# jklebes/MetropolisEngine

Hardware: AMD Instinct MI355X
Metric: MC steps/sec (chains x sweeps) at 2^20 chains, 16 params (higher is better)
Workload: dtype f64

## Files before the change

include/metropolis_engine.h:

```cpp
#ifndef METROPOLIS_ENGINE_H
#define METROPOLIS_ENGINE_H

#include <stddef.h>
#include <stdint.h>

#ifdef __cplusplus
extern "C" {
#endif

#define ME_ABI_VERSION 1

typedef struct me_engine me_engine;

typedef enum me_status {
  ME_OK = 0,
  ME_ERR_INVALID = 1,
  ME_ERR_UNSUPPORTED = 2,
  ME_ERR_HIP = 3,
  ME_ERR_NUMERIC = 4,
  ME_ERR_STATE = 5
} me_status;

typedef enum me_dtype { ME_F32 = 0, ME_F64 = 1 } me_dtype;

// ... 206 lines not shown
int me_mbar_histogram_gram_samples(int32_t device_id, const double *energies, const int32_t *rungs, int64_t n_samples,
                                   const double *ladder_temps, int32_t n_rungs, const double *f, const double *temps, int32_t n,
                                   const double *values, const double *edges, int32_t n_bins, double *slot_gram,
                                   double *ladder_gram, double *column_counts, double *mass, int64_t *counts,
                                   double *neff_fraction, int64_t *n_used);
int me_mbar_histogram_joint(me_engine *engine, const double *f, const double *temps, int32_t n, int32_t column_x,
                        const double *edges_x, int32_t n_bins_x, int32_t column_y, const double *edges_y, int32_t n_bins_y,
                        double *mass, int64_t *counts, double *neff_fraction);
int me_mbar_histogram_joint_samples(int32_t device_id, const double *energies, const int32_t *rungs, int64_t n_samples,
                                const double *ladder_temps, int32_t n_rungs, const double *f, const double *temps, int32_t n,
                                const double *values_x, const double *values_y, const double *edges_x, int32_t n_bins_x,
                                const double *edges_y, int32_t n_bins_y, double *mass, int64_t *counts, double *neff_fraction);
int me_mbar_histogram_joint_gram(me_engine *engine, const double *f, const double *temps, int32_t n, int32_t column_x,
                                 const double *edges_x, int32_t n_bins_x, int32_t column_y, const double *edges_y,
                                 int32_t n_bins_y, double *cell_gram, double *ladder_gram, double *column_counts, double *mass,
                                 int64_t *counts, double *neff_fraction, int64_t *n_used);
int me_mbar_histogram_joint_gram_samples(int32_t device_id, const double *energies, const int32_t *rungs, int64_t n_samples,
                                         const double *ladder_temps, int32_t n_rungs, const double *f, const double *temps,
                                         int32_t n, const double *values_x, const double *values_y, const double *edges_x,
                                         int32_t n_bins_x, const double *edges_y, int32_t n_bins_y, double *cell_gram,
                                         double *ladder_gram, double *column_counts, double *mass, int64_t *counts,
                                         double *neff_fraction, int64_t *n_used);

int me_recorded_inefficiency(me_engine *engine, int32_t mintime, int32_t max_lag, double *g, double *mean, double *var,
                             int32_t *stop_lag, int64_t *chains_used, double *acf);
int me_series_inefficiency_samples(int32_t device_id, const double *series, int64_t n_records, int64_t n_series,
                                   int64_t group_chains, int32_t mintime, int32_t max_lag, double *g, double *mean, double *var,
                                   int32_t *stop_lag, int64_t *chains_used, double *acf);

int me_last_error(me_engine *engine, char *buf, size_t buf_bytes);

int me_supported(int32_t dtype, int32_t n_real, int32_t n_complex, int32_t energy_kind);

int me_detect_equilibration(int32_t device_id, const double *series, int64_t n_series, int64_t length, int32_t fast,
                            int32_t nskip, int64_t *t0, double *g, double *neff_max);

#ifdef __cplusplus
}
#endif
#endif
```

metropolisengine_amd/_capi.py:

```python
import ctypes
import os

PKG_DIR = os.path.dirname(os.path.abspath(__file__))
LIB_PATH = os.environ.get("METROPOLIS_HIP_LIB") or os.path.join(PKG_DIR, "lib", "libmetropolis_hip.so")
ABI_VERSION = 1

ME_OK, ME_ERR_INVALID, ME_ERR_UNSUPPORTED, ME_ERR_HIP, ME_ERR_NUMERIC, ME_ERR_STATE = range(6)
ME_F32, ME_F64 = 0, 1
(ENERGY_ISO_QUAD, ENERGY_DIAG_QUAD, ENERGY_DENSE_QUAD, ENERGY_LANDAU_TOY, ENERGY_CYLINDER, ENERGY_USER,
 ENERGY_USER_INDIRECT, ENERGY_LANDAU_TERMS) = range(8)
FLAG_TRACK_COVARIANCE = 1
FLAG_REFERENCE_ENERGY_LEDGERS = 2
REJECT_NONE, REJECT_ABS_REAL0_GE, REJECT_USER = 0, 1, 2
STEP_ALL, STEP_REAL_GROUP, STEP_COMPLEX_GROUP, STEP_COMPLEX_MAGNITUDE_PHASE = range(4)
COV_REFERENCE, COV_FIXED, COV_POOLED = 0, 1, 2
COMM_ID_BYTES = 128
(FIELD_PARAMS, FIELD_ENERGY, FIELD_WIDTH, FIELD_MEAN, FIELD_COV, FIELD_OBS_MEAN, FIELD_FACTOR, FIELD_ENERGY_TOTAL) = range(8)

_dp = ctypes.POINTER(ctypes.c_double)


def double_ptr(arr):
    return arr.ctypes.data_as(_dp)

# ... 44 lines not shown
                                               ctypes.POINTER(ctypes.c_double)]),
    "me_get": (ctypes.c_int, [_H, ctypes.c_int32, ctypes.c_int64, ctypes.c_int64, _dp]),
    "me_set": (ctypes.c_int, [_H, ctypes.c_int32, ctypes.c_int64, ctypes.c_int64, _dp]),
    "me_recompute_energy": (ctypes.c_int, [_H]),
    "me_constants": (ctypes.c_int, [_H, _dp, ctypes.POINTER(ctypes.c_int32), _dp]),
    "me_counters": (ctypes.c_int, [_H, ctypes.POINTER(ctypes.c_uint64), ctypes.POINTER(ctypes.c_uint64)]),
    "me_set_counters": (ctypes.c_int, [_H, ctypes.c_uint64, ctypes.c_uint64]),
    "me_accept_stats": (ctypes.c_int, [_H, ctypes.POINTER(ctypes.c_uint64), ctypes.POINTER(ctypes.c_uint64)]),
    "me_pooled_moments_size": (ctypes.c_int, [_H, ctypes.POINTER(ctypes.c_int64)]),
    "me_pooled_moments_geometry": (ctypes.c_int, [_H, ctypes.POINTER(ctypes.c_int32), ctypes.POINTER(ctypes.c_int32),
                                                  ctypes.POINTER(ctypes.c_int32)]),
    "me_pooled_moments": (ctypes.c_int, [_H, _dp, ctypes.c_int64]),
    "me_pooled_moments_device": (ctypes.c_int, [_H, ctypes.c_void_p, ctypes.c_int64]),
    "me_comm_unique_id": (ctypes.c_int, [ctypes.c_void_p, ctypes.c_size_t]),
    "me_comm_init_rank": (ctypes.c_int, [_H, ctypes.c_void_p, ctypes.c_size_t, ctypes.c_int32, ctypes.c_int32]),
    "me_comm_destroy": (ctypes.c_int, [_H]),
    "me_comm_info": (ctypes.c_int, [_H, ctypes.POINTER(ctypes.c_int32), ctypes.POINTER(ctypes.c_int32),
                                    ctypes.POINTER(ctypes.c_int32)]),
    "me_pooled_moments_allreduce": (ctypes.c_int, [_H, _dp, ctypes.c_int64]),
    "me_pooled_moments_allreduce_begin": (ctypes.c_int, [_H]),
    "me_set_shared_factor": (ctypes.c_int, [_H, _dp, ctypes.c_int64]),
    "me_get_shared_factor": (ctypes.c_int, [_H, _dp, ctypes.c_int64, ctypes.POINTER(ctypes.c_int32)]),
    "me_set_accept_stats": (ctypes.c_int, [_H, ctypes.c_uint64, ctypes.c_uint64]),
    "me_set_cache_budget": (ctypes.c_int, [ctypes.c_int64]),
    "me_trace_enable": (ctypes.c_int, [_H, ctypes.c_int64, ctypes.c_int64]),
    "me_trace_shape": (ctypes.c_int, [_H, ctypes.POINTER(ctypes.c_int64), ctypes.POINTER(ctypes.c_int64),
                                      ctypes.POINTER(ctypes.c_int64)]),
    "me_trace_get": (ctypes.c_int, [_H, _dp, ctypes.c_int64]),
    "me_sync": (ctypes.c_int, [_H]),
    "me_set_stream": (ctypes.c_int, [_H, ctypes.c_void_p]),
    "me_time_steps": (ctypes.c_int, [_H, ctypes.c_int32, ctypes.c_int32, ctypes.POINTER(ctypes.c_float)]),
    "me_last_error": (ctypes.c_int, [_H, ctypes.c_char_p, ctypes.c_size_t]),
    "me_supported": (ctypes.c_int, [ctypes.c_int32, ctypes.c_int32, ctypes.c_int32, ctypes.c_int32]),
    "me_set_temperature_ladder": (ctypes.c_int, [_H, _dp, ctypes.c_int32]),
    "me_temperature_ladder": (ctypes.c_int, [_H, _dp, ctypes.c_int32, ctypes.POINTER(ctypes.c_int32)]),
    "me_replica_exchange": (ctypes.c_int, [_H, ctypes.c_int32]),
    "me_replica_stats": (ctypes.c_int, [_H, ctypes.POINTER(ctypes.c_uint64), ctypes.POINTER(ctypes.c_uint64),
                                        ctypes.POINTER(ctypes.c_uint64), ctypes.c_int32]),
    "me_set_replica_stats": (ctypes.c_int, [_H, ctypes.c_uint64, ctypes.POINTER(ctypes.c_uint64),
                                            ctypes.POINTER(ctypes.c_uint64), ctypes.c_int32]),
    "me_pooled_moments_range": (ctypes.c_int, [_H, ctypes.c_int64, ctypes.c_int64, _dp, ctypes.c_int64]),
    "me_set_temperature": (ctypes.c_int, [_H, ctypes.c_double]),
    "me_population_resample": (ctypes.c_int, [_H, ctypes.c_double]),
    "me_population_stats": (ctypes.c_int, [_H, ctypes.POINTER(ctypes.c_uint64), _dp, _dp, _dp, ctypes.POINTER(ctypes.c_int64),
                                           ctypes.c_int64]),
    "me_set_population_stats": (ctypes.c_int, [_H, ctypes.c_uint64, _dp, _dp, _dp, ctypes.POINTER(ctypes.c_int64)]),
    "me_population_families": (ctypes.c_int, [_H, ctypes.c_int64, ctypes.c_int64, ctypes.POINTER(ctypes.c_int64)]),
    "me_set_population_families": (ctypes.c_int, [_H, ctypes.c_int64, ctypes.c_int64, ctypes.POINTER(ctypes.c_int64)]),
    "me_energy_samples_enable": (ctypes.c_int, [_H, ctypes.c_int64]),
    "me_energy_samples_record": (ctypes.c_int, [_H]),
    "me_energy_samples_count": (ctypes.c_int, [_H, ctypes.POINTER(ctypes.c_int64), ctypes.POINTER(ctypes.c_int64)]),
    "me_energy_samples_get": (ctypes.c_int, [_H, ctypes.c_int64, ctypes.c_int64, _dp]),
    "me_energy_samples_set": (ctypes.c_int, [_H, ctypes.c_int64, _dp]),
    "me_mbar_solve": (ctypes.c_int, [_H, ctypes.c_double, ctypes.c_int32, _dp, ctypes.POINTER(ctypes.c_int32), _dp,
                                     ctypes.POINTER(ctypes.c_int64)]),
    "me_mbar_solve_newton": (ctypes.c_int, [_H, ctypes.c_double, ctypes.c_int32, _dp, ctypes.POINTER(ctypes.c_int32), _dp, _dp,
                                            ctypes.POINTER(ctypes.c_int32), ctypes.POINTER(ctypes.c_int32),
                                            ctypes.POINTER(ctypes.c_int64)]),
    "me_mbar_solve_newton_samples": (ctypes.c_int, [ctypes.c_int32, _dp, ctypes.POINTER(ctypes.c_int32), ctypes.c_int64, _dp,
                                                    ctypes.c_int32, ctypes.c_double, ctypes.c_int32, _dp,
                                                    ctypes.POINTER(ctypes.c_int32), _dp, _dp, ctypes.POINTER(ctypes.c_int32),
                                                    ctypes.POINTER(ctypes.c_int32), ctypes.POINTER(ctypes.c_int64)]),
    "me_mbar_reweight": (ctypes.c_int, [_H, _dp, _dp, ctypes.c_int32, _dp, _dp, _dp, _dp]),
    "me_mbar_solve_samples": (ctypes.c_int, [ctypes.c_int32, _dp, ctypes.POINTER(ctypes.c_int32), ctypes.c_int64, _dp,
                                             ctypes.c_int32, ctypes.c_double, ctypes.c_int32, _dp,
                                             ctypes.POINTER(ctypes.c_int32), _dp, ctypes.POINTER(ctypes.c_int64)]),
# ... 107 lines not shown
```

metropolisengine_amd/csrc/me_api.hip:

```cpp
#include <algorithm>
#include <cmath>
#include <cstdlib>
#include <cstring>
#include <dlfcn.h>
#include <mutex>
#include <memory>
#include <string>
#include <atomic>
#include <chrono>
#include <vector>

#include "me_engine.h"

namespace me {

static std::vector<const KernelSet *> &registry() {
  static std::vector<const KernelSet *> sets;
  return sets;
}
static std::mutex &registry_mutex() {
  static std::mutex m;
  return m;
}
void register_kernel_set(const KernelSet *set) {
// ... 112 lines not shown
  to_device_type(src, count, dtype, bytes);
  const hipError_t err = dst.resize(bytes.size());
  return err != hipSuccess ? err : hipMemcpy(dst.get(), bytes.data(), bytes.size(), hipMemcpyHostToDevice);
}

int refuse_stale_total(me_engine *e, const char *subject) {
  if (!e->stale_total) return ME_OK;
  return fail(e, ME_ERR_UNSUPPORTED, std::string(subject) + " not available with ME_FLAG_REFERENCE_ENERGY_LEDGERS: its two ledgers "
                                                            "make the energy of a chain ambiguous");
}

static int report_status(me_engine *e, unsigned int bits) {
  if (!bits) return ME_OK;
  ME_HIP(e, hipMemsetAsync(e->status.get(), 0, sizeof(unsigned int), e->stream));
  std::string msg = "numeric failure in at least one chain:";
  if (bits & ST_NONFINITE_ENERGY) msg += " non-finite energy;";
  if (bits & ST_BAD_PIVOT) msg += " non-positive Cholesky pivot (proposal covariance not positive definite);";
  if (bits & ST_BAD_WIDTH) msg += " sampling width <= 0;";
  return fail(e, ME_ERR_NUMERIC, msg);
}
int check_status(me_engine *e) {
  unsigned long long *scratch = e->host_scratch.get<unsigned long long>();
  ME_HIP(e, hipMemcpyAsync(&scratch[0], e->status.get(), sizeof(unsigned int), hipMemcpyDeviceToHost, e->stream));
  ME_HIP(e, hipStreamSynchronize(e->stream));
  return report_status(e, (unsigned int)scratch[0]);
}

}

using namespace me;

namespace {

int broadcast(me_engine *e, DeviceBuffer &dst, const std::vector<double> &row, bool tiled = false) {
  std::vector<unsigned char> bytes;
  to_device_type(row.data(), row.size(), e->dtype, bytes);
  ME_HIP(e, hipMemcpyAsync(e->row_dev.get(), bytes.data(), bytes.size(), hipMemcpyHostToDevice, e->stream));
  if (tiled) ME_HIP(e, launch_broadcast_tiled(dst.get(), e->row_dev.get(), (int)row.size(), e->n, e->dtype, e->stream));
  else ME_HIP(e, launch_broadcast_rows(dst.get(), e->row_dev.get(), (int)row.size(), e->n, e->dtype, e->stream));
  ME_HIP(e, hipStreamSynchronize(e->stream));
  return ME_OK;
}

template <typename T>
void gather_rows(const T *t, int comps, int64_t n_chains, double *dst) {
  for (int r = 0; r < comps; ++r)
    for (int64_t c = 0; c < n_chains; ++c) dst[c * comps + r] = (double)t[(size_t)r * n_chains + c];
}
template <typename T>
void scatter_rows(T *t, int comps, int64_t n_chains, const double *src) {
  for (int r = 0; r < comps; ++r)
    for (int64_t c = 0; c < n_chains; ++c) t[(size_t)r * n_chains + c] = (T)src[c * comps + r];
}
template <typename T>
void transpose_tiled(T *t, int entries, int64_t tile0, int64_t chain_begin, int64_t n_chains, double *dst, const double *src) {
  const size_t tile_values = (size_t)entries * 64;
  auto at = [&](int64_t c, int k) { return (size_t)((c >> 6) - tile0) * tile_values + (size_t)k * 64 + (size_t)(c & 63); };
  for (int64_t i = 0; i < n_chains; ++i)
    for (int k = 0; k < entries; ++k) {
      if (dst) dst[i * entries + k] = (double)t[at(chain_begin + i, k)];
      else t[at(chain_begin + i, k)] = (T)src[i * entries + k];
    }
}

int copy_tiled(me_engine *e, void *field_ptr, int entries, int64_t chain_begin, int64_t n_chains, double *dst, const double *src) {
  const int64_t tile0 = chain_begin >> 6, tile1 = (chain_begin + n_chains - 1) >> 6;
  const size_t tile_values = (size_t)entries * 64, n_values = (size_t)(tile1 - tile0 + 1) * tile_values;
  unsigned char *dev = (unsigned char *)field_ptr + (size_t)tile0 * tile_values * e->esize;
  std::vector<unsigned char> tmp(n_values * e->esize);
  const bool whole = (chain_begin & 63) == 0 && (((chain_begin + n_chains) & 63) == 0 || chain_begin + n_chains == e->n);
  if (dst || !whole) {
    ME_HIP(e, hipMemcpyAsync(tmp.data(), dev, tmp.size(), hipMemcpyDeviceToHost, e->stream));
    ME_HIP(e, hipStreamSynchronize(e->stream));
  }
  if (e->dtype == ME_F32) transpose_tiled(reinterpret_cast<float *>(tmp.data()), entries, tile0, chain_begin, n_chains, dst, src);
  else transpose_tiled(reinterpret_cast<double *>(tmp.data()), entries, tile0, chain_begin, n_chains, dst, src);
  if (src) {
    ME_HIP(e, hipMemcpyAsync(dev, tmp.data(), tmp.size(), hipMemcpyHostToDevice, e->stream));
    ME_HIP(e, hipStreamSynchronize(e->stream));
  }
  return dst ? check_status(e) : ME_OK;
}

int field_info(me_engine *e, int field, void **ptr, int *comps) {
  switch (field) {
    case ME_FIELD_PARAMS: *ptr = e->x.get(); *comps = e->d; return ME_OK;
    case ME_FIELD_ENERGY: *ptr = e->energy.get(); *comps = e->n_terms; return ME_OK;
    case ME_FIELD_WIDTH: *ptr = e->width.get(); *comps = e->width_rows; return ME_OK;
    case ME_FIELD_MEAN: *ptr = e->mean.get(); *comps = e->d; return ME_OK;
    case ME_FIELD_OBS_MEAN: *ptr = e->obs_mean.get(); *comps = e->nobs; return ME_OK;
    case ME_FIELD_COV:
      if (!e->cov)
        return fail(e, ME_ERR_UNSUPPORTED, "this engine keeps no per-chain covariance: for large parameter spaces it is "
                                           "kept on request only (me_config.flags: ME_FLAG_TRACK_COVARIANCE), and not "
                                           "at all where the field would pass 4 GiB");
      *ptr = e->cov.get(); *comps = e->p; return ME_OK;
    case ME_FIELD_ENERGY_TOTAL:
      if (!e->stale_total)
        return fail(e, ME_ERR_UNSUPPORTED, "this engine keeps one coherent energy ledger (sum ME_FIELD_ENERGY); a separate "
                                           "energy_total exists with ME_FLAG_REFERENCE_ENERGY_LEDGERS only");
      *ptr = e->energy.get<unsigned char>() + (size_t)e->n_terms * (size_t)e->n * e->esize; *comps = 1; return ME_OK;
    case ME_FIELD_FACTOR:
      if (!e->factor) return fail(e, ME_ERR_UNSUPPORTED, "this engine keeps no per-chain proposal factors (dimensions "
                                                         "without per-chain kernels, or a field beyond 4 GiB)");
      *ptr = e->factor.get(); *comps = e->p; return ME_OK;
    default: return fail(e, ME_ERR_INVALID, "unknown field id");
  }
}

// ... 56 lines not shown
    return fail(e, ME_ERR_INVALID, "ME_REJECT_ABS_REAL0_GE needs a real parameter");
  return ME_OK;
}
int check_user_reject(me_engine *e, int reject_kind, const KernelSet *ks) {
  if (reject_kind == ME_REJECT_USER && !ks->has_user_reject)
    return fail(e, ME_ERR_UNSUPPORTED,
                "ME_REJECT_USER: this user-energy plugin defines no me_user_reject (#define ME_USER_HAS_REJECT in its source)");
  return ME_OK;
}

}

namespace me {
namespace {
std::atomic<long long> g_cache_budget{224ll << 20};
}
long long cache_budget_bytes() { return g_cache_budget.load(std::memory_order_relaxed); }
void set_cache_budget_bytes(long long bytes) { g_cache_budget.store(bytes, std::memory_order_relaxed); }
}


int me_set_cache_budget(int64_t bytes) {
  if (bytes < 0) return fail(nullptr, ME_ERR_INVALID, "cache budget must be >= 0");
  me::set_cache_budget_bytes(bytes);
  return ME_OK;
}

int me_abi_version(void) { return ME_ABI_VERSION; }

int me_supported(int32_t dtype, int32_t n_real, int32_t n_complex, int32_t energy_kind) {
  return find_kernel_set(dtype, n_real, n_complex, energy_kind, nullptr) ? 1 : 0;
}

namespace {

int validate_config(const me_config *c, const KernelSet **ks_out) {
  if (c->abi_version != ME_ABI_VERSION) return fail(nullptr, ME_ERR_INVALID, "me_config.abi_version mismatch");
  if (c->n_real < 0 || c->n_complex < 0 || c->n_real + c->n_complex == 0)
    return fail(nullptr, ME_ERR_INVALID,
                "must give at least one real or complex parameter (metropolis_engine.py:37-39)");
  if (c->n_chains <= 0) return fail(nullptr, ME_ERR_INVALID, "n_chains must be positive");
  if (!(c->temp >= 0)) return fail(nullptr, ME_ERR_INVALID, "temp must be >= 0 (metropolis_engine.py:92)");
  if (!(c->target_acceptance > 0 && c->target_acceptance < 1))
    return fail(nullptr, ME_ERR_INVALID, "target_acceptance must be in (0, 1)");
  if (!(c->sampling_width > 0)) return fail(nullptr, ME_ERR_INVALID, "sampling_width must be > 0");
  if (c->dtype != ME_F32 && c->dtype != ME_F64) return fail(nullptr, ME_ERR_INVALID, "unknown dtype");
  if (!c->initial_params) return fail(nullptr, ME_ERR_INVALID, "initial_params is required");
  if (c->n_energy_coeffs < 0 || (c->n_energy_coeffs > 0 && !c->energy_coeffs))
    return fail(nullptr, ME_ERR_INVALID, "energy coefficients missing");
  int rc = check_reject_kind(nullptr, c->reject_kind, c->energy_kind, c->n_real);
  if (rc != ME_OK) return rc;
  if (c->cov_mode < ME_COV_REFERENCE || c->cov_mode > ME_COV_POOLED)
    return fail(nullptr, ME_ERR_INVALID, "unknown cov_mode");
  const KernelSet *ks = *ks_out = find_kernel_set(c->dtype, c->n_real, c->n_complex, c->energy_kind, c->user_energy_name);
  if (!ks) {
    if (is_user_kind(c->energy_kind))
      return fail(nullptr, ME_ERR_UNSUPPORTED,
                  std::string("no user-energy plugin named '") + (c->user_energy_name ? c->user_energy_name : "") +
                      "' is loaded for these dimensions (build it with metropolisengine_amd.build.build_user_energy "
                      "and load it with me_load_plugin)");
    if (!has_dims(c->dtype, c->n_real, c->n_complex))
      return fail(nullptr, ME_ERR_UNSUPPORTED,
                  "no kernel set compiled for (dtype, n_real, n_complex) = (" + std::to_string(c->dtype) + ", " +
                      std::to_string(c->n_real) + ", " + std::to_string(c->n_complex) + ")");
    return fail(nullptr, ME_ERR_UNSUPPORTED, "energy kind " + std::to_string(c->energy_kind) +
                                                  " is not compiled for these dimensions");
// ... 8 lines not shown
    const bool starts_shared = !initial_shape_is_identity(c) && c->cov_mode != ME_COV_REFERENCE;
    if (starts_shared && c->n_complex > 0)
      return fail(nullptr, ME_ERR_UNSUPPORTED,
                  "parameter spaces beyond " + std::to_string(kMaxRegisterDof) + " real degrees of freedom with complex "
                  "parameters run with the identity proposal shape only: leave covariance_matrix_real / _complex unset");
    {
      const long long per_block = (long long)(c->n_real + 2 * c->n_complex) * 64 * (c->dtype == ME_F32 ? 4 : 8);
      const bool dense = c->energy_kind == ME_ENERGY_DENSE_QUAD, pooled = c->cov_mode == ME_COV_POOLED || starts_shared;
      const bool per_chain = c->cov_mode == ME_COV_REFERENCE || (c->flags & ME_FLAG_TRACK_COVARIANCE) != 0;
      if ((dense || pooled || per_chain) && per_block * (pooled ? 2 : 1) > 150 * 1024)
        return fail(nullptr, ME_ERR_UNSUPPORTED,
                    "a dense quadratic form, a shared proposal factor or per-chain shapes beyond " + std::to_string(kMaxRegisterDof) +
                        " degrees of freedom are staged in LDS: this many parameters do not fit (float64: about 290, 145 with "
                        "a shared factor or an initial covariance that ME_COV_FIXED keeps; float32 twice that)");
    }
    if (c->flags & ME_FLAG_REFERENCE_ENERGY_LEDGERS)
      return fail(nullptr, ME_ERR_UNSUPPORTED, "ME_FLAG_REFERENCE_ENERGY_LEDGERS is not available beyond " +
                                                   std::to_string(kMaxRegisterDof) + " real degrees of freedom");
    if (c->reject_kind == ME_REJECT_USER) return fail(nullptr, ME_ERR_UNSUPPORTED, "no user plugins at these dimensions");
  }
  if ((c->flags & ME_FLAG_REFERENCE_ENERGY_LEDGERS) && (c->n_real == 0 || c->n_complex == 0))
    return fail(nullptr, ME_ERR_INVALID,
                "ME_FLAG_REFERENCE_ENERGY_LEDGERS applies to mixed engines (real and complex parameters): only their "
                "step_all keeps a separate energy_total (metropolis_engine.py:241-259)");
  if (c->cov_mode == ME_COV_REFERENCE && !ks->per_chain_cov)
    return fail(nullptr, ME_ERR_UNSUPPORTED,
                "per-chain adaptive covariance is not compiled for these dimensions; use ME_COV_FIXED or ME_COV_POOLED");
  return ME_OK;
}

struct Layout {
  bool keep_per_chain;
  bool keep_cov;
  bool x_tiled;
  int width_rows;
};
int decide_layout(const me_config *c, const KernelSet *ks, Layout &l) {
  const long long esz = c->dtype == ME_F32 ? 4 : 8, limit = 1ll << 32, padded = padded_chains(c->n_chains);
  l.keep_per_chain = ks->per_chain_cov && (!ks->streams_packed || c->cov_mode == ME_COV_REFERENCE);
  if (l.keep_per_chain && !ks->streams_packed && (long long)packed_total(c->n_real, c->n_complex) * padded * esz >= limit) {
    if (c->cov_mode == ME_COV_REFERENCE)
      return fail(nullptr, ME_ERR_UNSUPPORTED,
                  "the per-chain covariance field would exceed 4 GiB on this engine; shard the chains over more "
                  "engines or use ME_COV_FIXED / ME_COV_POOLED");
    l.keep_per_chain = false;
  }
  const long long rows = std::max<long long>(c->n_real + 2 * c->n_complex, 2 * c->n_real + c->n_complex);
  if (rows * padded * esz >= limit)
    return fail(nullptr, ME_ERR_UNSUPPORTED,
                "a per-chain field would exceed 4 GiB on this engine; shard the chains over more engines");
  l.keep_cov = l.keep_per_chain ||
               ((!ks->per_chain_cov || ks->streams_packed) && ks->tracks_cov && (c->flags & ME_FLAG_TRACK_COVARIANCE));
  l.x_tiled = ks->tiled_state;
  l.width_rows = (c->n_real > 0 && c->n_complex > 0) ? 3 : 1;
  return ME_OK;
}

std::unique_ptr<me_engine> configure(const me_config *c, const KernelSet *ks, const Layout &l) {
  std::unique_ptr<me_engine> e(new me_engine);
  e->device = c->device_id;
  e->ks = ks;
  e->n_terms = ks->energy_terms(c->energy_kind);
  e->dtype = c->dtype;
  e->esize = c->dtype == ME_F32 ? 4 : 8;
  e->n = c->n_chains;
  e->nr = c->n_real;
  e->nc = c->n_complex;
  e->d = e->nr + 2 * e->nc;
  e->p = packed_total(e->nr, e->nc);
  e->nobs = n_observables(e->nr, e->nc);
  e->chain_offset = c->chain_offset;
  e->seed = c->seed;
  e->temp = c->temp;
  e->target_acceptance = c->target_acceptance;
  e->energy_kind = c->energy_kind;
  e->reject_kind = c->reject_kind;
  e->reject_bound = c->reject_bound;
  e->cov_mode = c->cov_mode;
  e->coef.assign(c->energy_coeffs, c->energy_coeffs + c->n_energy_coeffs);
  e->alpha = -norm_ppf(c->target_acceptance / 2.0);
  e->m = e->nr + e->nc;
  e->ratio = (1.0 - 1.0 / e->m) * std::sqrt(2.0 * M_PI) * std::exp(e->alpha * e->alpha / 2.0) / 2.0 * e->alpha +
             1.0 / (e->m * c->target_acceptance * (1.0 - c->target_acceptance));
  if (const char *g = std::getenv("ME_GRID_BLOCKS")) e->grid_blocks = std::atoi(g);
  e->x_tiled = l.x_tiled;
  e->stale_total = (c->flags & ME_FLAG_REFERENCE_ENERGY_LEDGERS) != 0;
  e->width_rows = l.width_rows;
  e->n_slots = (e->n + 31) / 32 + 8;
  return e;
}

int allocate(me_engine *e, const Layout &l) {
  const KernelSet *ks = e->ks;
  ME_HIP(e, hipSetDevice(e->device));
  ME_HIP(e, e->stream.create());
  const size_t n = (size_t)e->n, tiles = (size_t)padded_chains(e->n), es = e->esize;
  ME_HIP(e, e->x.resize((e->x_tiled ? tiles : n) * e->d * es));
  ME_HIP(e, e->energy.resize(n * (e->n_terms + (e->stale_total ? 1 : 0)) * es));
  ME_HIP(e, e->width.resize(n * e->width_rows * es));
  ME_HIP(e, e->mean.resize(n * e->d * es));
  ME_HIP(e, e->obs_mean.resize(n * e->nobs * es));
  if (l.keep_cov) ME_HIP(e, e->cov.resize(tiles * e->p * es));
  if (l.keep_per_chain) ME_HIP(e, e->factor.resize(tiles * e->p * es));
  ME_HIP(e, e->shared_factor.resize((size_t)e->p * es));
  if (e->nc == 0) ME_HIP(e, e->shared_full.resize((size_t)e->nr * e->nr * es));
  if (e->shared_full && ks->prepare_matrix) ME_HIP(e, e->shared_image.resize(ks->matrix_image_bytes));
  ME_HIP(e, e->row_dev.resize((size_t)std::max(std::max(e->d, e->p), e->nobs) * es));
  ME_HIP(e, e->accept_slots.resize((size_t)e->n_slots * sizeof(unsigned long long)));
  ME_HIP(e, e->accept_total.resize(sizeof(unsigned long long)));
  ME_HIP(e, e->status.resize(sizeof(unsigned int)));
  const size_t moments_bytes = sizeof(double) * (size_t)moments_size(e->nr, e->nc);
  ME_HIP(e, e->pool.dev.resize(moments_bytes));
  ME_HIP(e, e->host_scratch.allocate(64));
  e->host_scratch.get<unsigned long long>()[0] = e->host_scratch.get<unsigned long long>()[1] = 0;
  ME_HIP(e, e->pool.host.allocate(moments_bytes));
  if (pool_reduce_supported(e->nr, e->nc, e->dtype))
    ME_HIP(e, e->pool.partials.resize(sizeof(double) * (size_t)pool_reduce_blocks(e->n, e->nr, e->nc) *
                                      (size_t)(1 + e->d + e->nr + e->nc + e->d * (e->d + 1) / 2)));
  ME_HIP(e, hipMemsetAsync(e->accept_slots.get(), 0, e->accept_slots.bytes(), e->stream));
  ME_HIP(e, hipMemsetAsync(e->status.get(), 0, sizeof(unsigned int), e->stream));
  return ME_OK;
}

int upload_coefficients(me_engine *e) {
  const std::vector<double> &coef = e->coef;
  const bool runtime_dims = e->ks->n_real < 0;
  std::vector<double> form;
  if (runtime_dims && e->energy_kind == ME_ENERGY_DIAG_QUAD) {
    if ((int)coef.size() != e->nr + e->nc) return fail(e, ME_ERR_INVALID, "wrong number of energy coefficients for this energy kind");
    form.assign(coef.begin(), coef.end());
// ... 23 lines not shown
  for (int i = 0; i < e->nr; ++i) {
    obs[i] = std::fabs(init[i]);
    obs[e->nr + e->nc + i] = init[i] * init[i];
  }
  for (int j = 0; j < e->nc; ++j) obs[e->nr + j] = std::hypot(init[e->nr + j], init[e->nr + e->nc + j]);
  const int pr = packed_real(e->nr);
  std::vector<double> c0(e->p, 0.0);
  bool identity = true;
  for (int i = 0; i < e->nr; ++i)
    for (int j = 0; j <= i; ++j) {
      const double v = c->covariance_real ? c->covariance_real[i * e->nr + j] : (i == j ? 1.0 : 0.0);
      c0[i * (i + 1) / 2 + j] = v;
      identity = identity && v == (i == j ? 1.0 : 0.0);
    }
  for (int i = 0; i < e->nc; ++i) {
    for (int j = 0; j < i; ++j) {
      const double re = c->covariance_complex ? c->covariance_complex[2 * (i * e->nc + j)] : 0.0;
      const double im = c->covariance_complex ? c->covariance_complex[2 * (i * e->nc + j) + 1] : 0.0;
      c0[pr + i * i + 2 * j] = re;
      c0[pr + i * i + 2 * j + 1] = im;
      identity = identity && re == 0.0 && im == 0.0;
    }
    const double dg = c->covariance_complex ? c->covariance_complex[2 * (i * e->nc + i)] : 1.0;
    c0[pr + i * i + 2 * i] = dg;
    identity = identity && dg == 1.0;
  }
  std::vector<double> f0 = c0;
  for (int i = 0; i < e->nc; ++i)
    for (int j = 0; j < i; ++j) f0[pr + i * i + 2 * j + 1] = -f0[pr + i * i + 2 * j + 1];
  if (!host_factor(f0, e->nr, e->nc))
    return fail(e, ME_ERR_INVALID, "initial covariance matrix is not positive definite (metropolis_engine.py:270)");
  int rc = ME_OK;
  std::vector<double> width_row((size_t)e->width_rows, c->sampling_width);
  if ((rc = broadcast(e, e->x, init, e->x_tiled)) || (rc = broadcast(e, e->mean, init)) || (rc = broadcast(e, e->obs_mean, obs)) ||
      (rc = broadcast(e, e->width, width_row)) || (e->cov && (rc = broadcast(e, e->cov, c0, true))) ||
      (e->factor && (rc = broadcast(e, e->factor, f0, true))) || (rc = upload_shared_factor(e, f0.data())))
    return rc;
  e->cov_kind = identity ? CK_IDENTITY : (e->ks->n_real < 0 && e->factor) ? CK_PER_CHAIN : CK_SHARED;
  return ME_OK;
}

int initial_energy(me_engine *e) {
  const int rc = me_recompute_energy(e);
  if (rc != ME_OK) return rc;
  const hipError_t herr = hipStreamSynchronize(e->stream);
  if (herr != hipSuccess) return fail(e, ME_ERR_HIP, std::string("initial energy evaluation: ") + hipGetErrorString(herr));
  return ME_OK;
}

}

int me_create(const me_config *c, me_engine **out) {
  if (!c || !out) return fail(nullptr, ME_ERR_INVALID, "null config or output pointer");
  *out = nullptr;
  const KernelSet *ks = nullptr;
  Layout layout;
  int rc;
  if ((rc = validate_config(c, &ks)) || (rc = decide_layout(c, ks, layout))) return rc;
  int n_dev = 0;
  if (hipGetDeviceCount(&n_dev) != hipSuccess || n_dev <= 0)
    return fail(nullptr, ME_ERR_HIP, "no HIP device available (this library has no CPU fallback)");
  if (c->device_id < 0 || c->device_id >= n_dev) return fail(nullptr, ME_ERR_INVALID, "device_id out of range");

  std::unique_ptr<me_engine> e = configure(c, ks, layout);
  if ((rc = allocate(e.get(), layout)) || (rc = upload_coefficients(e.get())) || (rc = initial_state(e.get(), c)) ||
      (rc = initial_energy(e.get())))
    return fail(nullptr, rc, e->err);
  *out = e.release();
  return ME_OK;
}

int me_set_reject_condition(me_engine *e, int32_t reject_kind, double reject_bound) {
  if (!e) return ME_ERR_INVALID;
  int rc;
  if ((rc = check_reject_kind(e, reject_kind, e->energy_kind, e->nr)) || (rc = check_user_reject(e, reject_kind, e->ks))) return rc;
  e->reject_kind = reject_kind;
  e->reject_bound = reject_bound;
  return ME_OK;
}

int me_set_energy(me_engine *e, int32_t energy_kind, const double *coeffs, int32_t n_coeffs, const char *user_name) {
  if (!e) return ME_ERR_INVALID;
  if (n_coeffs < 0 || (n_coeffs > 0 && !coeffs)) return fail(e, ME_ERR_INVALID, "energy coefficients missing");
  if (e->ks->n_real < 0) return fail(e, ME_ERR_UNSUPPORTED, "me_set_energy: not available on the runtime-dimension kernel set");
  if (energy_kind == ME_ENERGY_DENSE_QUAD)
    return fail(e, ME_ERR_UNSUPPORTED, "me_set_energy: the dense quadratic form keeps device images of its matrix; create a new engine");
  const KernelSet *ks = find_kernel_set(e->dtype, e->nr, e->nc, energy_kind, user_name);
  if (!ks || ks->n_real < 0)
    return fail(e, ME_ERR_UNSUPPORTED, is_user_kind(energy_kind)
                    ? std::string("no user-energy plugin named '") + (user_name ? user_name : "") + "' is loaded for these dimensions"
                    : "energy kind " + std::to_string(energy_kind) + " is not compiled for these dimensions");
  if (ks->tiled_state != e->ks->tiled_state || ks->per_chain_cov != e->ks->per_chain_cov || ks->streams_packed != e->ks->streams_packed ||
      ks->tracks_cov != e->ks->tracks_cov)
    return fail(e, ME_ERR_UNSUPPORTED, "me_set_energy: the plugin was built with other per-chain covariance options than this engine's kernel set");
  if (e->reject_kind == ME_REJECT_USER && !ks->has_user_reject)
    return fail(e, ME_ERR_UNSUPPORTED, "me_set_energy: the engine's wall is the plugin's me_user_reject, which the new energy does not define");
  const int n_terms = ks->energy_terms(energy_kind);
  ME_HIP(e, hipSetDevice(e->device));
  ME_HIP(e, hipStreamSynchronize(e->stream));
  DeviceBuffer ledger, coef_dev;
  if (n_terms != e->n_terms)
    ME_HIP(e, ledger.resize((size_t)e->n * (size_t)(n_terms + (e->stale_total ? 1 : 0)) * e->esize));
  if (is_user_kind(energy_kind) && n_coeffs > 0) ME_HIP(e, upload(coef_dev, coeffs, (size_t)n_coeffs, e->dtype));
  if (n_terms != e->n_terms) {
    e->energy = std::move(ledger);
    e->n_terms = n_terms;
    if (e->trace.chains > 0) e->trace.restart();
  }
  e->coef.assign(coeffs, coeffs + n_coeffs);
  e->coef_dev = std::move(coef_dev);
  e->ks = ks;
  e->energy_kind = energy_kind;
  const int rc = me_recompute_energy(e);
  if (rc != ME_OK) return rc;
  ME_HIP(e, hipStreamSynchronize(e->stream));
  return check_status(e);
}

int me_load_plugin(const char *path) {
  if (!path) return fail(nullptr, ME_ERR_INVALID, "null plugin path");
  void *handle = dlopen(path, RTLD_NOW | RTLD_GLOBAL);
  if (!handle) return fail(nullptr, ME_ERR_INVALID, std::string("dlopen failed: ") + dlerror());
  return ME_OK;
}

// ... 128 lines not shown
  l.mean = e->mean.get();
  l.cov = e->cov.get();
  l.obs_mean = e->obs_mean.get();
  l.factor = e->factor.get();
  l.status = e->status.get<unsigned int>();
  l.n = e->n;
  l.measure_count = count;
  l.update_cov = (count > 50 && e->cov) ? 1 : 0;
  l.split_widths = (e->width_rows == 3 && !e->widths_synced) ? 1 : 0;
  l.write_factor = (l.update_cov && e->cov_mode == ME_COV_REFERENCE) ? 1 : 0;
  l.grid_blocks = e->grid_blocks;
}

int commit_measure(me_engine *e, const MeasureLaunch &l) {
  e->measure_count = l.measure_count;
  if (l.write_factor) e->cov_kind = CK_PER_CHAIN;
  if (e->trace.chains > 0) {
    const long long cols = e->d + e->n_terms + e->width_rows;
    if (e->trace.rows == e->trace.capacity) {
      const long long cap = e->trace.capacity ? 2 * e->trace.capacity : 1024;
      DeviceBuffer bigger;
      ME_HIP(e, bigger.resize(sizeof(double) * (size_t)(cap * cols * e->trace.chains)));
      if (e->trace.dev) {
        ME_HIP(e, hipMemcpyAsync(bigger.get(), e->trace.dev.get(), sizeof(double) * (size_t)(e->trace.rows * cols * e->trace.chains),
                                 hipMemcpyDeviceToDevice, e->stream));
        ME_HIP(e, hipStreamSynchronize(e->stream));
      }
      e->trace.dev = std::move(bigger);
      e->trace.capacity = cap;
    }
    const int rows_valid = (e->width_rows == 3 && e->widths_synced) ? 1 : e->width_rows;
    double *row = e->trace.dev.get<double>() + e->trace.rows * cols * e->trace.chains;
    ME_HIP(e, launch_trace(e->x.get(), e->energy.get(), e->width.get(), e->n, e->d, e->n_terms, rows_valid, e->dtype, e->trace.chains,
                           e->trace.stride, row, e->stream, e->x_tiled));
    if (rows_valid != e->width_rows) {
      double *widths = row + (size_t)(e->d + e->n_terms) * e->trace.chains;
      for (int r = 1; r < 3; ++r)
        ME_HIP(e, hipMemcpyAsync(widths + (size_t)r * e->trace.chains, widths, sizeof(double) * (size_t)e->trace.chains,
                                 hipMemcpyDeviceToDevice, e->stream));
    }
    e->trace.rows += 1;
  }
  return ME_OK;
}
}

int me_measure(me_engine *e) {
  if (!e) return ME_ERR_INVALID;
  ME_HIP(e, hipSetDevice(e->device));
  MeasureLaunch l;
  fill_measure_launch(e, l, e->measure_count + 1);
  ME_HIP(e, e->ks->measure(l, e->stream));
  return commit_measure(e, l);
}

int me_cycle(me_engine *e, int32_t n_sweeps) {
  if (!e) return ME_ERR_INVALID;
  if (n_sweeps <= 0) return fail(e, ME_ERR_INVALID, "n_sweeps must be positive");
  ME_HIP(e, hipSetDevice(e->device));
  if (e->ks->cycle) {
    StepLaunch sl;
    fill_step_launch(e, sl, n_sweeps);
    MeasureLaunch ml;
    fill_measure_launch(e, ml, e->measure_count + 1);
    ml.split_widths = 0;
    const hipError_t err = e->ks->cycle(sl, ml, e->stream);
    if (err == hipSuccess) {
// ... 39 lines not shown
  const long long want = e->trace.rows * (e->d + e->n_terms + e->width_rows) * e->trace.chains;
  if (n_doubles != want) return fail(e, ME_ERR_INVALID, "wrong trace buffer length");
  if (want == 0) return ME_OK;
  ME_HIP(e, hipSetDevice(e->device));
  ME_HIP(e, hipStreamSynchronize(e->stream));
  ME_HIP(e, hipMemcpy(dst, e->trace.dev.get(), sizeof(double) * (size_t)want, hipMemcpyDeviceToHost));
  return ME_OK;
}

int me_field_components(me_engine *e, int32_t field, int32_t *n_components) {
  if (!e || !n_components) return ME_ERR_INVALID;
  void *ptr;
  int comps;
  int rc = field_info(e, field, &ptr, &comps);
  if (rc == ME_OK) *n_components = comps;
  return rc;
}

int me_energy_terms(me_engine *e, int32_t *n_terms) {
  if (!e || !n_terms) return ME_ERR_INVALID;
  *n_terms = e->n_terms;
  return ME_OK;
}

int me_get(me_engine *e, int32_t field, int64_t chain_begin, int64_t n_chains, double *dst) {
  if (!e || !dst) return ME_ERR_INVALID;
  if (chain_begin < 0 || n_chains < 0 || chain_begin + n_chains > e->n) return fail(e, ME_ERR_INVALID, "chain range out of bounds");
  ME_HIP(e, hipSetDevice(e->device));
  void *ptr;
  int comps;
  int rc = field_info(e, field, &ptr, &comps);
  if (rc != ME_OK) return rc;
  if (n_chains == 0) return ME_OK;
  if (field == ME_FIELD_COV || field == ME_FIELD_FACTOR || (field == ME_FIELD_PARAMS && e->x_tiled))
    return copy_tiled(e, ptr, comps, chain_begin, n_chains, dst, nullptr);
  std::vector<unsigned char> tmp((size_t)comps * n_chains * e->esize);
  for (int r = 0; r < comps; ++r)
    ME_HIP(e, hipMemcpyAsync(tmp.data() + (size_t)r * n_chains * e->esize,
                             (const unsigned char *)ptr + ((size_t)r * e->n + chain_begin) * e->esize,
                             (size_t)n_chains * e->esize, hipMemcpyDeviceToHost, e->stream));
  ME_HIP(e, hipStreamSynchronize(e->stream));
  if (e->dtype == ME_F32) gather_rows(reinterpret_cast<const float *>(tmp.data()), comps, n_chains, dst);
  else gather_rows(reinterpret_cast<const double *>(tmp.data()), comps, n_chains, dst);
  if (field == ME_FIELD_WIDTH && e->width_rows == 3 && e->widths_synced)
    for (int64_t c = 0; c < n_chains; ++c) dst[c * 3 + 1] = dst[c * 3 + 2] = dst[c * 3];
  return check_status(e);
}

int me_set(me_engine *e, int32_t field, int64_t chain_begin, int64_t n_chains, const double *src) {
  if (!e || !src) return ME_ERR_INVALID;
  if (chain_begin < 0 || n_chains < 0 || chain_begin + n_chains > e->n) return fail(e, ME_ERR_INVALID, "chain range out of bounds");
  ME_HIP(e, hipSetDevice(e->device));
  void *ptr;
  int comps;
  int rc = field_info(e, field, &ptr, &comps);
  if (rc != ME_OK) return rc;
  if (field == ME_FIELD_WIDTH && e->width_rows == 3 && (chain_begin != 0 || n_chains != e->n))
    return fail(e, ME_ERR_INVALID, "widths of a mixed engine must be set for all chains at once");
  if (n_chains == 0) return ME_OK;
  if (field == ME_FIELD_COV || field == ME_FIELD_FACTOR || (field == ME_FIELD_PARAMS && e->x_tiled)) {
    rc = copy_tiled(e, ptr, comps, chain_begin, n_chains, nullptr, src);
    if (rc != ME_OK) return rc;
    if (field == ME_FIELD_FACTOR) e->cov_kind = CK_PER_CHAIN;
    return ME_OK;
  }
  std::vector<unsigned char> tmp((size_t)comps * n_chains * e->esize);
  if (e->dtype == ME_F32) scatter_rows(reinterpret_cast<float *>(tmp.data()), comps, n_chains, src);
  else scatter_rows(reinterpret_cast<double *>(tmp.data()), comps, n_chains, src);
  for (int r = 0; r < comps; ++r)
    ME_HIP(e, hipMemcpyAsync((unsigned char *)ptr + ((size_t)r * e->n + chain_begin) * e->esize,
                             tmp.data() + (size_t)r * n_chains * e->esize, (size_t)n_chains * e->esize,
                             hipMemcpyHostToDevice, e->stream));
  ME_HIP(e, hipStreamSynchronize(e->stream));
  if (field == ME_FIELD_FACTOR) e->cov_kind = CK_PER_CHAIN;
  if (field == ME_FIELD_WIDTH && e->width_rows == 3) e->widths_synced = false;
  return ME_OK;
}

int me_constants(me_engine *e, double *alpha, int32_t *m, double *ratio) {
  if (!e) return ME_ERR_INVALID;
  if (alpha) *alpha = e->alpha;
  if (m) *m = e->m;
  if (ratio) *ratio = e->ratio;
  return ME_OK;
}

int me_counters(me_engine *e, uint64_t *step_index, uint64_t *measure_step_counter) {
  if (!e) return ME_ERR_INVALID;
  if (step_index) *step_index = e->step_index;
  if (measure_step_counter) *measure_step_counter = e->measure_count;
  return ME_OK;
}

int me_set_counters(me_engine *e, uint64_t step_index, uint64_t measure_step_counter) {
// ... 41 lines not shown
  *matrix_core = e->ks->pool_stage1 ? 1 : 0;
  *tile_chains = e->ks->pool_stage1 ? 64 : pool_tile_chains(e->nr, e->nc, e->dtype);
  *partial_rows = pool_reduce_blocks(e->n, e->nr, e->nc);
  return ME_OK;
}

namespace {
hipError_t wait_polling(hipEvent_t ev) {
  const auto t0 = std::chrono::steady_clock::now();
  for (;;) {
    const hipError_t rc = hipEventQuery(ev);
    if (rc != hipErrorNotReady) return rc;
    if (std::chrono::steady_clock::now() - t0 > std::chrono::milliseconds(2)) return hipEventSynchronize(ev);
  }
}
hipError_t wait_polling(hipStream_t stream) {
  const auto t0 = std::chrono::steady_clock::now();
  for (;;) {
    const hipError_t rc = hipStreamQuery(stream);
    if (rc != hipErrorNotReady) return rc;
    if (std::chrono::steady_clock::now() - t0 > std::chrono::milliseconds(2)) return hipStreamSynchronize(stream);
  }
}

int check_pooled(me_engine *e, int64_t n_doubles) {
  if (n_doubles != moments_size(e->nr, e->nc)) return fail(e, ME_ERR_INVALID, "wrong pooled-moment buffer length");
  if (e->pool.pending) return fail(e, ME_ERR_STATE, "a pooled-moment reduction is in flight (me_pooled_moments_end first)");
  if (!e->pool.partials) return fail(e, ME_ERR_UNSUPPORTED, "pooled moments: dimension too large for the reduction kernel");
  ME_HIP(e, hipSetDevice(e->device));
  return ME_OK;
}
int enqueue_pool_reduce(me_engine *e, const void *x, long long n_chains, long long n_slots, double proposed, double *device_out) {
  hipError_t err = launch_pool_reduce(x, n_chains, e->nr, e->nc, e->dtype, e->accept_slots.get<unsigned long long>(), n_slots, proposed,
                                      e->pool.partials.get<double>(), device_out, e->stream, e->ks->pool_stage1, e->x_tiled);
  if (err == hipErrorInvalidValue) return fail(e, ME_ERR_UNSUPPORTED, "pooled moments: dimension too large for the reduction kernel");
  ME_HIP(e, err);
  return ME_OK;
}
int enqueue_pooled_moments(me_engine *e, double *device_out, int64_t n_doubles) {
  const int rc = check_pooled(e, n_doubles);
  return rc != ME_OK ? rc : enqueue_pool_reduce(e, e->x.get(), e->n, e->n_slots, (double)e->proposed, device_out);
}
int fetch_pooled_moments(me_engine *e, double *host_out, int64_t n_doubles) {
  const size_t bytes = sizeof(double) * (size_t)n_doubles;
  ME_HIP(e, hipMemcpyAsync(e->pool.host.get<double>(), e->pool.dev.get(), bytes, hipMemcpyDeviceToHost, e->stream));
  ME_HIP(e, wait_polling(e->stream));
  std::memcpy(host_out, e->pool.host.get<double>(), bytes);
  return ME_OK;
}
}

int me_pooled_moments_device(me_engine *e, void *device_out, int64_t n_doubles) {
  if (!e || !device_out) return ME_ERR_INVALID;
  int rc = enqueue_pooled_moments(e, (double *)device_out, n_doubles);
  if (rc != ME_OK) return rc;
  ME_HIP(e, wait_polling(e->stream));
  return ME_OK;
}

int me_pooled_moments(me_engine *e, double *host_out, int64_t n_doubles) {
  if (!e || !host_out) return ME_ERR_INVALID;
  const int rc = enqueue_pooled_moments(e, e->pool.dev.get<double>(), n_doubles);
  return rc != ME_OK ? rc : fetch_pooled_moments(e, host_out, n_doubles);
}

int me_pooled_moments_range(me_engine *e, int64_t chain_begin, int64_t n_chains, double *host_out, int64_t n_doubles) {
  if (!e || !host_out) return ME_ERR_INVALID;
  if (chain_begin < 0 || n_chains <= 0 || chain_begin + n_chains > e->n || chain_begin % 64 != 0 || n_chains % 64 != 0)
    return fail(e, ME_ERR_INVALID, "the chain range must be whole 64-chain tiles inside the engine");
  int rc = check_pooled(e, n_doubles);
  if (rc != ME_OK) return rc;
  const unsigned char *x = e->x.get<unsigned char>();
  if (e->x_tiled) {
    x += (size_t)chain_begin * e->d * e->esize;
  } else {
    const size_t row = (size_t)n_chains * e->esize;
    if (row * e->d > e->pool.range_x.bytes()) {
      ME_HIP(e, hipStreamSynchronize(e->stream));
      ME_HIP(e, e->pool.range_x.reserve(row * e->d));
    }
    ME_HIP(e, hipMemcpy2DAsync(e->pool.range_x.get(), row, x + (size_t)chain_begin * e->esize, (size_t)e->n * e->esize, row, (size_t)e->d,
                               hipMemcpyDeviceToDevice, e->stream));
    x = e->pool.range_x.get<unsigned char>();
  }
  if ((rc = enqueue_pool_reduce(e, x, n_chains, 0, 0.0, e->pool.dev.get<double>())) != ME_OK) return rc;
  return fetch_pooled_moments(e, host_out, n_doubles);
}

namespace {
int begin_pooled(me_engine *e, bool allreduce) {
  if (e->pool.pending) return fail(e, ME_ERR_STATE, "a pooled-moment reduction is already in flight: call me_pooled_moments_end first");
  if (allreduce && !e->comm)
    return fail(e, ME_ERR_STATE, "this engine has no communicator: call me_comm_init_rank first (single-GPU engines use me_pooled_moments)");
  ME_HIP(e, hipSetDevice(e->device));
  if (!e->pool.copy_stream) {
    ME_HIP(e, e->pool.copy_stream.create());
    ME_HIP(e, e->pool.reduced.create(hipEventDisableTiming));
    ME_HIP(e, e->pool.copied.create(hipEventDisableTiming));
  }
  const int64_t n_doubles = moments_size(e->nr, e->nc);
  int rc = enqueue_pooled_moments(e, e->pool.dev.get<double>(), n_doubles);
  if (rc != ME_OK) return rc;
  ME_HIP(e, hipEventRecord(e->pool.reduced, e->stream));
  ME_HIP(e, hipStreamWaitEvent(e->pool.copy_stream, e->pool.reduced, 0));
  if (allreduce) {
    const ncclResult_t nrc = e->rccl->all_reduce(e->pool.dev.get<double>(), e->pool.dev.get<double>(), (size_t)n_doubles, ncclDouble, ncclSum, e->comm, e->pool.copy_stream);
    if (nrc != ncclSuccess) return fail(e, ME_ERR_HIP, std::string("ncclAllReduce: ") + e->rccl->error_string(nrc));
// ... 167 lines not shown
```

metropolisengine_amd/csrc/me_device.h:

```cpp
#pragma once

#include <type_traits>
#include <utility>

#include <hip/hip_runtime.h>
#include <stdint.h>

#include "me_internal.h"
#include "me_math64.h"

namespace me {

struct U4 {
  uint32_t x, y, z, w;
};

__device__ __forceinline__ uint32_t xor3(uint32_t a, uint32_t b, uint32_t c) {
  return __builtin_amdgcn_bitop3_b32(a, b, c, 0x96);
}
__device__ __forceinline__ U4 philox4x32_10(U4 c, uint32_t k0, uint32_t k1) {
#pragma unroll
  for (int r = 0; r < 10; ++r) {
    const uint64_t p0 = (uint64_t)0xD2511F53u * c.x;
    const uint64_t p1 = (uint64_t)0xCD9E8D57u * c.z;
// ... 179 lines not shown
  __device__ __forceinline__ R load_nt(int k, unsigned int tile_off) const { return load_aux<ME_NT_AUX>(k, tile_off); }
  __device__ __forceinline__ void store(int k, unsigned int tile_off, R value) const { store_aux<0>(k, tile_off, value); }
  __device__ __forceinline__ void store_nt(int k, unsigned int tile_off, R value) const { store_aux<ME_NT_AUX>(k, tile_off, value); }
};

template <bool NT, class F>
__device__ __forceinline__ auto packed_load(const F &f, int row, unsigned int chain_off) {
  if constexpr (NT) return f.load_nt(row, chain_off);
  else return f.load(row, chain_off);
}
template <bool NT, class F, typename R>
__device__ __forceinline__ void packed_store(const F &f, int row, unsigned int chain_off, R value) {
  if constexpr (NT) f.store_nt(row, chain_off, value);
  else f.store(row, chain_off, value);
}

template <typename R, bool NTS>
struct StateField : Field<R> {
  using Field<R>::Field;
  __device__ __forceinline__ R load(int row, unsigned int chain_off) const {
    if constexpr (NTS) return Field<R>::load_nt(row, chain_off);
    else return Field<R>::load(row, chain_off);
  }
  __device__ __forceinline__ void store(int row, unsigned int chain_off, R value) const {
    if constexpr (NTS) Field<R>::store_nt(row, chain_off, value);
    else Field<R>::store(row, chain_off, value);
  }
};

#ifndef ME_TILED_STATE_DOF
#define ME_TILED_STATE_DOF 16
#endif
constexpr int kTiledStateDof = ME_TILED_STATE_DOF;
template <typename R, int D, bool NTS = false>
struct XField {
  static constexpr bool kTiled = D >= kTiledStateDof;
  std::conditional_t<kTiled, TiledField<R>, StateField<R, NTS>> f;
  __device__ __forceinline__ XField(const R *base, long long n) : f(base, n, D) {}
  static __device__ __forceinline__ unsigned int offset(long long c) {
    if constexpr (kTiled) return tiled_offset<R>(c, D);
    else return (unsigned int)c * (unsigned int)sizeof(R);
  }
  __device__ __forceinline__ R load(int row, unsigned int off) const {
    if constexpr (kTiled && NTS) return f.load_nt(row, off);
    else return f.load(row, off);
  }
  __device__ __forceinline__ void store(int row, unsigned int off, R value) const {
    if constexpr (kTiled && NTS) f.store_nt(row, off, value);
    else f.store(row, off, value);
  }
};
template <typename R, int D>
__device__ __forceinline__ long long state_index(long long c, int row, long long n) {
  if constexpr (D >= kTiledStateDof) return ((c >> 6) * (long long)D + row) * 64 + (c & 63);
  else return (long long)row * n + c;
}

constexpr int kMaxPackedInRegisters = 160;
#ifndef ME_STREAM_F64_ENTRIES
#define ME_STREAM_F64_ENTRIES 96
#endif
constexpr int kStreamF64Entries = ME_STREAM_F64_ENTRIES;

template <typename R, int NR, int NC>
struct EnergyIso {
  static constexpr int D = NR + 2 * NC;
  R a;
  __device__ __forceinline__ R operator()(const R (&x)[D]) const {
    R s0 = 0, s1 = 0;
#pragma unroll
    for (int d = 0; d + 1 < D; d += 2) {
      s0 += x[d] * x[d];
      s1 += x[d + 1] * x[d + 1];
    }
    if constexpr (D % 2 == 1) s0 += x[D - 1] * x[D - 1];
    return a * (s0 + s1);
  }
};

template <typename R, int NR, int NC>
struct EnergyDiag {
  static constexpr int D = NR + 2 * NC;
  R w[D];
  __device__ __forceinline__ R operator()(const R (&x)[D]) const {
    R s0 = 0, s1 = 0;
#pragma unroll
    for (int d = 0; d + 1 < D; d += 2) {
      s0 += w[d] * x[d] * x[d];
// ... 337 lines not shown
        R acc = 0;
#pragma unroll
        for (int j = 0; j <= i; ++j) acc += fac(tri(i, j)) * g[j];
        xp[i] = x[i] + w_r * acc;
      }
    }
    if constexpr (MOVE_COMPLEX) {
#pragma unroll
      for (int i = 0; i < NC; ++i) {
        R are = 0, aim = 0;
#pragma unroll
        for (int j = 0; j < i; ++j) {
          const R lre = fac(cre(PR, i, j));
          const R lim = fac(cim(PR, i, j));
          const R wre = g[NR + j] * R(0.70710678118654752440), wim = g[NR + NC + j] * R(0.70710678118654752440);
          are += lre * wre - lim * wim;
          aim += lre * wim + lim * wre;
        }
        const R ld = fac(cdiag(PR, i));
        are += ld * (g[NR + i] * R(0.70710678118654752440));
        aim += ld * (g[NR + NC + i] * R(0.70710678118654752440));
        xp[NR + i] = x[NR + i] + w_c * are;
        xp[NR + NC + i] = x[NR + NC + i] + w_c * aim;
      }
    }
  }

}

template <typename R, int NR, int NC, class Energy, int CK, int GROUP, bool LADDER, class Ledger>
__device__ __forceinline__ void decide_step(const StepArgs<R> &a, long long c, const Energy &en, bool stale_total, R u,
                                            const R (&g)[2 * ((NR + 2 * NC + 1) / 2)], R (&x)[NR + 2 * NC], const R (&xp)[NR + 2 * NC],
                                            Ledger &ledger, R &total_q5, R &w, R &w_r, R &w_c, unsigned int &wave_accepted,
                                            bool &bad_energy) {
  [[maybe_unused]] constexpr int D = NR + 2 * NC;
  constexpr bool MOVE_REAL = NR > 0 && GROUP != GROUP_COMPLEX;
  constexpr bool MOVE_COMPLEX = NC > 0 && GROUP != GROUP_REAL;
  using N_ = Num<R>;
  bool rejected = false;
  if (a.reject_kind == ME_REJECT_ABS_REAL0_GE) rejected = !(N_::abs_(xp[0]) < a.reject_bound);
  else if (a.reject_kind == ME_REJECT_USER) rejected = energy_reject(en, xp, 0);
  R terms_new[Ledger::T];
  const R e_new = ledger.propose(en, xp, terms_new);
  const R diff = e_new - (stale_total ? total_q5 : ledger.partial());
  bool accept = diff <= R(0);
  if constexpr (LADDER) accept = accept || uphill_at<true>(a, c, u, diff);
  else if (a.temp > R(0)) accept = accept || N_::uphill(u, diff, a.inv_temp, a.inv_temp_log2e);
  accept = accept && !rejected;
  bad_energy |= (!rejected && !N_::finite(e_new));
  if constexpr (CK == CK_IDENTITY) {
    const R wa_r = accept ? w_r : R(0), wa_c = accept ? w_c : R(0);
    if constexpr (MOVE_REAL) {
#pragma unroll
      for (int i = 0; i < NR; ++i) x[i] = x[i] + wa_r * g[i];
    }
    if constexpr (MOVE_COMPLEX) {
#pragma unroll
      for (int j = 0; j < NC; ++j) {
        x[NR + j] = x[NR + j] + wa_c * (g[NR + j] * R(0.70710678118654752440));
        x[NR + NC + j] = x[NR + NC + j] + wa_c * (g[NR + NC + j] * R(0.70710678118654752440));
      }
    }
  } else {
#pragma unroll
    for (int d = 0; d < D; ++d) x[d] = accept ? xp[d] : x[d];
  }
  if (stale_total) total_q5 = accept ? e_new : total_q5;
  else ledger.commit(accept, terms_new);
  w = N_::adapt(w, accept, a.ratio, a.p, a.damping, a.up, a.down);
  if constexpr (GROUP == GROUP_ALL) w_r = w_c = w;
  else if constexpr (GROUP == GROUP_REAL) w_r = w;
  else w_c = w;
  wave_accepted += (unsigned int)__popcll(__ballot(accept));
}

template <typename R, int NR, int NC, class Energy, int CK, bool INJECT, int GROUP, bool LADDER, class Ledger, class Fac>
__device__ __forceinline__ void run_sweeps(const StepArgs<R> &a, const Energy &en, long long c, unsigned long long gid,
                                           bool stale_total, R (&x)[NR + 2 * NC], Ledger &ledger, R &total_q5, R &w, R &w_r,
                                           R &w_c, Fac &&fac, unsigned int &wave_accepted, bool &bad_energy) {
  constexpr int D = NR + 2 * NC;
  constexpr int NW = 2 * ((D + 1) / 2);
  for (int s = 0; s < a.n_sweeps; ++s) {
    R g[NW], u, xp[D];
    draw_step<R, NR, NC, INJECT>(a, c, gid, s, g, u);
    propose_registers<R, NR, NC, CK, GROUP>(x, g, w_r, w_c, fac, xp);
    decide_step<R, NR, NC, Energy, CK, GROUP, LADDER>(a, c, en, stale_total, u, g, x, xp, ledger, total_q5, w, w_r, w_c, wave_accepted, bad_energy);
  }
}

#ifndef ME_STEP_WAVES_PER_EU
#define ME_STEP_WAVES_PER_EU 0
#endif
#if ME_STEP_WAVES_PER_EU > 0
#define ME_STEP_BOUNDS __launch_bounds__(kFusedStepThreads, ME_STEP_WAVES_PER_EU)
#else
#define ME_STEP_BOUNDS __launch_bounds__(kFusedStepThreads)
#endif

#ifndef ME_STEP_PRIO_SHIFT
#define ME_STEP_PRIO_SHIFT 8
#endif
__device__ __forceinline__ void stagger_priority() {
#if ME_STEP_PRIO_SHIFT >= 0
  switch ((blockIdx.x >> ME_STEP_PRIO_SHIFT) & 3u) {
    case 0: __builtin_amdgcn_s_setprio(3); break;
    case 1: __builtin_amdgcn_s_setprio(2); break;
    case 2: __builtin_amdgcn_s_setprio(1); break;
    default: break;
  }
#endif
}

template <typename R, int NR, int NC, class Energy, int CK, bool INJECT = false, int GROUP = GROUP_ALL, bool NTS = false,
          bool LADDER = false>
__global__ void ME_STEP_BOUNDS k_step(StepArgs<R> a, Energy en) {
  constexpr int D = NR + 2 * NC;
  constexpr bool MIXED = NR > 0 && NC > 0;
  static_assert(GROUP == GROUP_ALL || MIXED, "group-wise kernels exist for mixed engines only");
  using N_ = Num<R>;

  stagger_priority();
  if constexpr (!INJECT) N_::prepare();
  energy_prepare(en, 0);
  unsigned int wave_accepted = 0;
  bool bad_energy = false, bad_width = false;
  const long long stride = (long long)gridDim.x * blockDim.x;
  using Ledger = EnergyLedger<R, Energy, GROUP>;
  const XField<R, D, NTS> fx(a.x, a.n);
  const StateField<R, NTS> fe(a.energy, a.n, Ledger::T + (MIXED ? 1 : 0)), fw(a.width, a.n, MIXED ? 3 : 1);
  const bool stale_total = MIXED && GROUP == GROUP_ALL && a.stale_total != 0;
  constexpr bool PER_CHAIN = CK == CK_PER_CHAIN || CK == CK_PER_CHAIN_NT;
  constexpr int PF = PER_CHAIN ? NR * (NR + 1) / 2 + NC * NC : 0;
  constexpr bool STREAM_FACTOR = PER_CHAIN && (PF > kMaxPackedInRegisters ||
                                               (!INJECT && sizeof(R) == 8 && NC == 0 && PF > kStreamF64Entries));
  const TiledField<R> ffac(a.factor, a.n, STREAM_FACTOR ? 0 : PF);
  for (long long c = (long long)blockIdx.x * blockDim.x + threadIdx.x; c < a.n; c += stride) {
    const unsigned int coff = (unsigned int)c * (unsigned int)sizeof(R);
    const unsigned int xoff = fx.offset(c);
    R x[D];
#pragma unroll
    for (int d = 0; d < D; ++d) x[d] = fx.load(d, xoff);
    Ledger ledger;
    R total_q5 = R(0);
    if (stale_total) total_q5 = fe.load(Ledger::T, coff);
    else ledger.load(fe, coff);
    R w = fw.load(MIXED ? GROUP : 0, coff);
    R w_r = w, w_c = w;
    if constexpr (MIXED && GROUP == GROUP_ALL) {
      if (a.split_widths) {
        w_r = fw.load(GROUP_REAL, coff);
        w_c = fw.load(GROUP_COMPLEX, coff);
      }
    }
    const unsigned long long gid = a.chain_offset + (unsigned long long)c;
    [[maybe_unused]] const unsigned int toff = tiled_offset<R>(c, PF);
    auto fac = [&](int k) -> R {
      if constexpr (CK == CK_PER_CHAIN_NT) return ffac.load_nt(k, toff);
      else if constexpr (CK == CK_PER_CHAIN) return ffac.load(k, toff);
      else return a.factor[k];
    };

    if constexpr (STREAM_FACTOR) {
      constexpr int NW = 2 * ((D + 1) / 2);
      for (int s = 0; s < a.n_sweeps; ++s) {
        static_assert(!INJECT, "the streamed-factor form has no replay hook");
        constexpr int NBLK = (NW + 1 + 3) / 4;
        const unsigned long long step = a.step_index + (unsigned long long)s;
        R g[NW];
        R u_accept;
        {
          uint32_t words[4 * NBLK];
#pragma unroll
          for (int b = 0; b < NBLK; ++b) {
            const U4 o = philox_block(gid, step, b, a.seed_lo, a.seed_hi);
// ... 59 lines not shown
            const R lim = use(std::integral_constant<int, cim(NR * (NR + 1) / 2, i, j)>{});
            const R wre = g[NR + j] * R(0.70710678118654752440), wim = g[NR + NC + j] * R(0.70710678118654752440);
            are += lre * wre - lim * wim;
            aim += lre * wim + lim * wre;
          });
          const R ld = use(std::integral_constant<int, cdiag(NR * (NR + 1) / 2, i)>{});
          are += ld * (g[NR + i] * R(0.70710678118654752440));
          aim += ld * (g[NR + NC + i] * R(0.70710678118654752440));
          if constexpr (GROUP != GROUP_REAL) {
            xp[NR + i] = x[NR + i] + w_c * are;
            xp[NR + NC + i] = x[NR + NC + i] + w_c * aim;
          }
        });
        bool rejected = false;
        if (a.reject_kind == ME_REJECT_ABS_REAL0_GE) rejected = !(N_::abs_(xp[0]) < a.reject_bound);
        else if (a.reject_kind == ME_REJECT_USER) rejected = energy_reject(en, xp, 0);
        R terms_new[Ledger::T];
        const R e_new = ledger.propose(en, xp, terms_new);
        const R diff = e_new - (stale_total ? total_q5 : ledger.partial());
        bool accept = diff <= R(0);
        if constexpr (LADDER) accept = accept || uphill_at<true>(a, c, u_accept, diff);
        else if (a.temp > R(0)) accept = accept || N_::uphill(u_accept, diff, a.inv_temp, a.inv_temp_log2e);
        accept = accept && !rejected;
        bad_energy |= (!rejected && !N_::finite(e_new));
#pragma unroll
        for (int d = 0; d < D; ++d) x[d] = accept ? xp[d] : x[d];
        if (stale_total) total_q5 = accept ? e_new : total_q5;
        else ledger.commit(accept, terms_new);
        w = N_::adapt(w, accept, a.ratio, a.p, a.damping, a.up, a.down);
        if constexpr (GROUP == GROUP_ALL) w_r = w_c = w;
        else if constexpr (GROUP == GROUP_REAL) w_r = w;
        else w_c = w;
        wave_accepted += (unsigned int)__popcll(__ballot(accept));
      }
    } else {
      run_sweeps<R, NR, NC, Energy, CK, INJECT, GROUP, LADDER>(a, en, c, gid, stale_total, x, ledger, total_q5, w, w_r, w_c, fac, wave_accepted, bad_energy);
    }
    bad_width |= !(w > R(0));
#pragma unroll
    for (int d = 0; d < D; ++d) fx.store(d, xoff, x[d]);
    if (stale_total) fe.store(Ledger::T, coff, total_q5);
    else ledger.store(fe, coff);
    fw.store(MIXED ? GROUP : 0, coff, w);
  }
  publish_step(a, blockDim.x >> 6, wave_accepted, bad_energy, bad_width);
}

template <typename R, int NR, int NC, class Energy>
__global__ void __launch_bounds__(kStepThreads) k_init_energy(const R *xs, R *energy, long long n, unsigned int *status,
                                                                Energy en, int total_row) {
  constexpr int D = NR + 2 * NC;
  energy_prepare(en, 0);
  const long long stride = (long long)gridDim.x * kStepThreads;
  for (long long c = (long long)blockIdx.x * kStepThreads + threadIdx.x; c < n; c += stride) {
    R x[D];
#pragma unroll
    for (int d = 0; d < D; ++d) x[d] = xs[state_index<R, D>(c, d, n)];
    constexpr int T = term_count<Energy>::value;
    bool finite = true;
    R total = R(0);
#pragma unroll
    for (int t = 0; t < T; ++t) {
      R e;
      if constexpr (T == 1) e = en(x);
      else e = en.term(t, x);
      energy[(long long)t * n + c] = e;
      total = t == 0 ? e : total + e;
      finite = finite && Num<R>::finite(e);
    }
    if (total_row >= 0) energy[(long long)total_row * n + c] = total;
    if (!finite) atomicOr(status, (unsigned int)ST_NONFINITE_ENERGY);
  }
}

}
#include "me_packed_walk.h"
// ... 198 lines not shown
    R x[D];
#pragma unroll
    for (int d = 0; d < D; ++d) x[d] = fx.load(d, xoff);
    measure_chain<R, NR, NC, PER_CHAIN_COV, FUSED, NT, NTM>(a, c, x, fmean, fobs, fcov, ffac, s_delta, [&](R &w_real, R &w_cplx) {
      constexpr bool MIXED = NR > 0 && NC > 0;
      w_real = fw.load((MIXED && a.split_widths) ? 1 : 0, coff);
      w_cplx = fw.load((MIXED && a.split_widths) ? 2 : 0, coff);
    }, bad_pivot);
  }
  if (bad_pivot) atomicOr(a.status, (unsigned int)ST_BAD_PIVOT);
}

template <typename R, int NR, int NC, class Energy, int CK, bool NT, bool NTM, bool LADDER = false>
__global__ void ME_STEP_BOUNDS k_cycle(StepArgs<R> a, MeasureArgs<R> ma, Energy en) {
  constexpr int D = NR + 2 * NC;
  constexpr int P = NR * (NR + 1) / 2 + NC * NC;
  constexpr int NOBS = 2 * NR + NC;
  constexpr bool MIXED = NR > 0 && NC > 0;
  static_assert(P <= kMaxPackedInRegisters, "k_cycle keeps the packed matrix in registers");
  static_assert(CK == CK_IDENTITY || CK == CK_SHARED || CK == CK_PER_CHAIN, "NT selects the non-temporal factor read");
  constexpr int CKX = CK == CK_PER_CHAIN ? (NT ? CK_PER_CHAIN_NT : CK_PER_CHAIN) : CK;
  using N_ = Num<R>;
  N_::prepare();
  energy_prepare(en, 0);
  unsigned int wave_accepted = 0;
  bool bad_energy = false, bad_width = false, bad_pivot = false;
  const long long stride = (long long)gridDim.x * blockDim.x;
  using Ledger = EnergyLedger<R, Energy, GROUP_ALL>;
  const XField<R, D> fx(a.x, a.n);
  const Field<R> fe(a.energy, a.n, Ledger::T + (MIXED ? 1 : 0)), fw(a.width, a.n, MIXED ? 3 : 1);
  const Field<R> fmean(ma.mean, a.n, D), fobs(ma.obs_mean, a.n, NOBS);
  const TiledField<R> fcov(ma.cov, a.n, P), ffac(ma.factor, a.n, P);
  const bool stale_total = MIXED && a.stale_total != 0;
  for (long long c = (long long)blockIdx.x * blockDim.x + threadIdx.x; c < a.n; c += stride) {
    const unsigned int coff = (unsigned int)c * (unsigned int)sizeof(R);
    const unsigned int xoff = fx.offset(c);
    R x[D];
#pragma unroll
    for (int d = 0; d < D; ++d) x[d] = fx.load(d, xoff);
    Ledger ledger;
    R total_q5 = R(0);
    if (stale_total) total_q5 = fe.load(Ledger::T, coff);
    else ledger.load(fe, coff);
    R w = fw.load(0, coff);
    R w_r = w, w_c = w;
    if constexpr (MIXED) {
      if (a.split_widths) {
        w_r = fw.load(GROUP_REAL, coff);
        w_c = fw.load(GROUP_COMPLEX, coff);
      }
    }
    const unsigned long long gid = a.chain_offset + (unsigned long long)c;
    [[maybe_unused]] const unsigned int toff = tiled_offset<R>(c, P);
    auto fac = [&](int k) -> R {
      if constexpr (CK == CK_PER_CHAIN) return packed_load<NT>(ffac, k, toff);
      else return a.factor[k];
    };
    run_sweeps<R, NR, NC, Energy, CKX, false, GROUP_ALL, LADDER>(a, en, c, gid, stale_total, x, ledger, total_q5, w, w_r, w_c, fac,
                                                         wave_accepted, bad_energy);
    bad_width |= !(w > R(0));
#pragma unroll
    for (int d = 0; d < D; ++d) fx.store(d, xoff, x[d]);
    if (stale_total) fe.store(Ledger::T, coff, total_q5);
    else ledger.store(fe, coff);
    fw.store(0, coff, w);
    measure_chain<R, NR, NC, true, true, NT, NTM>(ma, c, x, fmean, fobs, fcov, ffac, nullptr,
                                                  [&](R &w_real, R &w_cplx) { w_real = w_cplx = w; }, bad_pivot);
  }
  publish_step(a, blockDim.x >> 6, wave_accepted, bad_energy, bad_width, bad_pivot);
}

template <typename R, int NR, bool NT>
__global__ void __launch_bounds__(kStepThreads) k_factor_stream(const R *cov, R *factor, unsigned int *status, long long n) {
  constexpr int P = NR * (NR + 1) / 2;
  constexpr int ROWS = sizeof(R) == 4 ? 4 : 2;
  __shared__ R rows[ROWS * NR][kStepThreads];
  bool bad_pivot = false;
  const long long stride = (long long)gridDim.x * kStepThreads;
  for (long long c = (long long)blockIdx.x * kStepThreads + threadIdx.x; c < n; c += stride) {
    const long long base = (c >> 6) * (long long)P * 64 + (c & 63);
    factor_real_rows<R, ROWS, NT>(cov + base, factor + base, NR, rows, (int)threadIdx.x, bad_pivot);
  }
  if (bad_pivot) atomicOr(status, (unsigned int)ST_BAD_PIVOT);
}

template <typename R, int NR, int NC, bool NT>
__global__ void __launch_bounds__(kStepThreads) k_factor_mixed(const R *cov, R *factor, unsigned int *status, long long n) {
  constexpr int PR = NR * (NR + 1) / 2, P = PR + NC * NC;
  using N_ = Num<R>;
  bool bad_pivot = false;
  const long long stride = (long long)gridDim.x * kStepThreads;
  for (long long c = (long long)blockIdx.x * kStepThreads + threadIdx.x; c < n; c += stride) {
    const long long base = (c >> 6) * (long long)P * 64 + (c & 63);
    const R *cv = cov + base;
    R *fc = factor + base;
    auto in = [&](int k) -> R { return NT ? __builtin_nontemporal_load(cv + (long long)k * 64) : cv[(long long)k * 64]; };
    for (int i = 0; i < NR; ++i)
      for (int j = 0; j <= i; ++j) {
        R s = in(tri(i, j));
        for (int k = 0; k < j; ++k) s = fma_(-fc[(long long)tri(i, k) * 64], fc[(long long)tri(j, k) * 64], s);
// ... 14 lines not shown
```

metropolisengine_amd/csrc/me_engine.h:

```cpp
#pragma once

#include <string>
#include <utility>
#include <vector>

#include "me_comm.h"
#include "me_internal.h"

#pragma GCC visibility push(hidden)

namespace me {


class DeviceBuffer {
 public:
  DeviceBuffer() = default;
  DeviceBuffer(DeviceBuffer &&o) noexcept : ptr_(std::exchange(o.ptr_, nullptr)), bytes_(std::exchange(o.bytes_, 0)) {}
  DeviceBuffer &operator=(DeviceBuffer &&o) noexcept {
    if (this != &o) {
      reset();
      ptr_ = std::exchange(o.ptr_, nullptr);
      bytes_ = std::exchange(o.bytes_, 0);
    }
    return *this;
// ... 86 lines not shown
  operator hipEvent_t() const { return event_; }

 private:
  hipEvent_t event_ = nullptr;
};

}

struct me_engine {
  int device = 0;
  me::Stream stream;
  const me::KernelSet *ks = nullptr;
  int dtype = ME_F32;
  size_t esize = 4;
  long long n = 0;
  int nr = 0, nc = 0, d = 0, p = 0, nobs = 0;
  unsigned long long chain_offset = 0, seed = 0;
  double temp = 0, target_acceptance = 0.3, alpha = 0, ratio = 0, reject_bound = 0;
  int m = 0, energy_kind = 0, reject_kind = 0, cov_mode = 0;
  bool stale_total = false;
  me::Event time_start, time_stop;
  std::vector<double> shared_host;
  int cov_kind = me::CK_IDENTITY;
  int grid_blocks = 0;
  int n_terms = 1;
  std::vector<double> coef;
  unsigned long long step_index = 0, measure_count = 1;
  unsigned long long fused_cycles = 0;
  me::DeviceBuffer x, energy, width, mean, cov, obs_mean;
  me::DeviceBuffer factor, shared_factor, shared_full, shared_image, energy_image, coef_dev, row_dev;
  me::DeviceBuffer accept_slots, accept_total;
  long long n_slots = 0;
  unsigned long long proposed = 0;
  bool x_tiled = false;
  int width_rows = 1;
  bool widths_synced = true;
  me::DeviceBuffer status;
  me::PinnedBuffer host_scratch;
  struct Pool {
    me::DeviceBuffer dev, partials;
    me::PinnedBuffer host;
    me::DeviceBuffer range_x;
    me::Stream copy_stream;
    me::Event reduced, copied;
    bool pending = false;
  } pool;
  const me::RcclApi *rccl = nullptr;
  ncclComm_t comm = nullptr;
  int comm_rank = 0, comm_world = 1;
  struct Trace {
    me::DeviceBuffer dev;
    long long chains = 0, stride = 1, rows = 0, capacity = 0;
    void restart() {
      dev.reset();
      rows = capacity = 0;
    }
  } trace;
  struct Ladder {
    int n_rungs = 0;
    std::vector<double> temps;
    me::DeviceBuffer table;
    me::DeviceBuffer pair_counts;
    unsigned long long round = 0;
  } ladder;
  struct Population {
    me::DeviceBuffer fam, fam_out;
    me::DeviceBuffer x, energy;
// ... 44 lines not shown
```

metropolisengine_amd/csrc/me_generic.hip:

```cpp
#include "me_internal.h"
#include "me_launch.h"

namespace me {
namespace {

template <typename R>
__global__ void __launch_bounds__(kBlockThreads) k_broadcast_rows(R *dst, const R *row_values, int rows, long long n) {
  const long long stride = (long long)gridDim.x * kBlockThreads;
  for (long long c = (long long)blockIdx.x * kBlockThreads + threadIdx.x; c < n; c += stride)
    for (int r = 0; r < rows; ++r) dst[(long long)r * n + c] = row_values[r];
}

template <typename R>
__global__ void __launch_bounds__(kBlockThreads) k_broadcast_tiled(R *dst, const R *entry_values, int entries, long long n_padded) {
  const long long total = n_padded * entries, stride = (long long)gridDim.x * kBlockThreads;
  for (long long i = (long long)blockIdx.x * kBlockThreads + threadIdx.x; i < total; i += stride)
    dst[i] = entry_values[(i >> 6) % entries];
}

__device__ __forceinline__ void pair_of(int p, int &i, int &j) {
  i = (int)((sqrtf(8.0f * (float)p + 1.0f) - 1.0f) * 0.5f);
  while (i * (i + 1) / 2 > p) --i;
  while ((i + 1) * (i + 2) / 2 <= p) ++i;
  j = p - i * (i + 1) / 2;
}

constexpr int kMaxEntries = 12;

template <typename R, int TILE>
__global__ void __launch_bounds__(kBlockThreads) k_pool_reduce(const R *x, long long n, int nr, int nc, int entry_base, int tiled, double *partials) {
  extern __shared__ __attribute__((aligned(16))) unsigned char smem_raw[];
  R *tile = reinterpret_cast<R *>(smem_raw);
  constexpr int kTilePitch = TILE + 1;
  const int d = nr + 2 * nc;
  const int n_aug = d + nr + nc;
  const int n_pair = d * (d + 1) / 2;
  const int n_entries = 1 + n_aug + n_pair;
  const int tid = threadIdx.x;
  auto at = [&](int r, long long c) -> long long { return tiled ? ((c >> 6) * (long long)d + r) * 64 + (c & 63) : (long long)r * n + c; };

  int row_i[kMaxEntries], row_j[kMaxEntries];
  bool active[kMaxEntries];
  double acc[kMaxEntries];
#pragma unroll
  for (int k = 0; k < kMaxEntries; ++k) {
    const int e = entry_base + tid + k * kBlockThreads;
    acc[k] = 0.0;
    row_i[k] = row_j[k] = -1;
    active[k] = e < n_entries;
    if (!active[k] || e == 0) continue;
    if (e <= n_aug) {
      row_i[k] = e - 1;
    } else {
      pair_of(e - 1 - n_aug, row_i[k], row_j[k]);
    }
  }

  const long long n_tiles = (n + TILE - 1) / TILE;
  for (long long t = blockIdx.x; t < n_tiles; t += gridDim.x) {
    const long long base = t * TILE;
    const int valid = (int)((n - base) < TILE ? (n - base) : TILE);
    for (int r = tid / TILE; r < n_aug; r += kBlockThreads / TILE) {
      const int col = tid % TILE;
      R v = 0;
      if (col < valid) {
        const long long c = base + col;
        if (r < d) v = x[at(r, c)];
        else if (r < d + nr) {
          const R xv = x[at(r - d, c)];
          v = xv < 0 ? -xv : xv;
        } else {
          const int j = r - d - nr;
// ... 78 lines not shown
#pragma unroll
  for (int w = 0; w < kFinishSlices; ++w) s += part[w][lane];
  if (e == 0) {
    out[0] = s;
  } else if (e <= n_aug) {
    const int r = e - 1;
    out[r < d ? 1 + r : 1 + d + n_pair + (r - d)] = s;
  } else if (e < n_entries) {
    const int p = e - 1 - n_aug;
    int i, j;
    pair_of(p, i, j);
    out[1 + d + p] = s;
    if (i == j && i < nr) out[1 + d + n_pair + nr + nc + i] = s;
  }
}

}

hipError_t launch_broadcast_rows(void *dst, const void *row_values, int rows, long long n, int dtype,
                                 hipStream_t stream) {
  long long blocks = (n + kBlockThreads - 1) / kBlockThreads;
  if (blocks > 4096) blocks = 4096;
  if (blocks < 1) blocks = 1;
  if (dtype == ME_F32)
    hipLaunchKernelGGL(k_broadcast_rows<float>, dim3((unsigned)blocks), dim3(kBlockThreads), 0, stream, (float *)dst,
                       (const float *)row_values, rows, n);
  else
    hipLaunchKernelGGL(k_broadcast_rows<double>, dim3((unsigned)blocks), dim3(kBlockThreads), 0, stream, (double *)dst,
                       (const double *)row_values, rows, n);
  return hipGetLastError();
}

hipError_t launch_broadcast_tiled(void *dst, const void *entry_values, int entries, long long n, int dtype,
                                  hipStream_t stream) {
  const long long n_padded = (n + 63) / 64 * 64;
  long long blocks = (n_padded * entries + kBlockThreads - 1) / kBlockThreads;
  if (blocks > 8192) blocks = 8192;
  if (blocks < 1) blocks = 1;
  if (dtype == ME_F32)
    hipLaunchKernelGGL(k_broadcast_tiled<float>, dim3((unsigned)blocks), dim3(kBlockThreads), 0, stream, (float *)dst,
                       (const float *)entry_values, entries, n_padded);
  else
    hipLaunchKernelGGL(k_broadcast_tiled<double>, dim3((unsigned)blocks), dim3(kBlockThreads), 0, stream, (double *)dst,
                       (const double *)entry_values, entries, n_padded);
  return hipGetLastError();
}

constexpr int kSumThreads = 1024;
__global__ void __launch_bounds__(kSumThreads) k_sum_slots(const unsigned long long *slots, long long n_slots,
                                                           unsigned long long *total) {
  __shared__ unsigned long long part[kSumThreads / 64];
  unsigned long long s = 0;
  long long i = threadIdx.x;
  for (; i + 7 * kSumThreads < n_slots; i += 8 * kSumThreads) {
    unsigned long long v[8];
#pragma unroll
    for (int u = 0; u < 8; ++u) v[u] = slots[i + u * kSumThreads];
#pragma unroll
    for (int u = 0; u < 8; ++u) s += v[u];
  }
  for (; i < n_slots; i += kSumThreads) s += slots[i];
#pragma unroll
  for (int w = 32; w > 0; w >>= 1) s += __shfl_xor(s, w, 64);
  if ((threadIdx.x & 63) == 0) part[threadIdx.x >> 6] = s;
  __syncthreads();
  if (threadIdx.x == 0) {
    unsigned long long t = 0;
#pragma unroll
    for (int w = 0; w < kSumThreads / 64; ++w) t += part[w];
    total[0] = t;
  }
}

template <typename R>
__global__ void __launch_bounds__(kBlockThreads) k_trace(const R *x, const R *energy, const R *width, long long n, int d,
                                                         int n_terms, int width_rows, long long n_traced, long long stride,
                                                         int tiled, double *out) {
  const long long t = (long long)blockIdx.x * kBlockThreads + threadIdx.x;
  if (t >= n_traced) return;
  const long long c = t * stride;
  for (int k = 0; k < d; ++k)
    out[(long long)k * n_traced + t] = (double)x[tiled ? ((c >> 6) * (long long)d + k) * 64 + (c & 63) : (long long)k * n + c];
  for (int k = 0; k < n_terms; ++k) out[(long long)(d + k) * n_traced + t] = (double)energy[(long long)k * n + c];
  for (int r = 0; r < width_rows; ++r)
    out[(long long)(d + n_terms + r) * n_traced + t] = (double)width[(long long)r * n + c];
}

hipError_t launch_trace(const void *x, const void *energy, const void *width, long long n, int d, int n_terms,
                        int width_rows, int dtype, long long n_traced, long long stride, double *out, hipStream_t stream,
                        bool tiled_state) {
  const dim3 grid((unsigned)((n_traced + kBlockThreads - 1) / kBlockThreads)), block(kBlockThreads);
  if (dtype == ME_F32)
    hipLaunchKernelGGL(k_trace<float>, grid, block, 0, stream, (const float *)x, (const float *)energy, (const float *)width,
                       n, d, n_terms, width_rows, n_traced, stride, tiled_state ? 1 : 0, out);
  else
    hipLaunchKernelGGL(k_trace<double>, grid, block, 0, stream, (const double *)x, (const double *)energy,
                       (const double *)width, n, d, n_terms, width_rows, n_traced, stride, tiled_state ? 1 : 0, out);
  return hipGetLastError();
}

hipError_t launch_sum_slots(const unsigned long long *slots, long long n_slots, unsigned long long *total,
                            hipStream_t stream) {
  hipLaunchKernelGGL(k_sum_slots, dim3(1), dim3(kSumThreads), 0, stream, slots, n_slots, total);
  return hipGetLastError();
}

constexpr size_t kPoolLdsLimit = 160 * 1024;
int pool_tile_chains(int nr, int nc, int dtype) {
  const int n_aug = nr + 2 * nc + nr + nc;
  const size_t elem = dtype == ME_F32 ? sizeof(float) : sizeof(double);
  for (int tile : {64, 32, 16})
    if ((size_t)n_aug * (size_t)(tile + 1) * elem <= kPoolLdsLimit) return tile;
  return 0;
}

bool pool_reduce_supported(int nr, int nc, int dtype) { return pool_tile_chains(nr, nc, dtype) != 0; }

int pool_reduce_blocks(long long n, int nr, int nc) {
  const int d = nr + 2 * nc;
  const long long n_entries = 1 + d + nr + nc + (long long)d * (d + 1) / 2;
  long long cap = (32ll << 20) / (8 * n_entries);
  if (cap > 1024) cap = 1024;
  if (cap < 64) cap = 64;
  if (d + nr + nc <= 32) cap = 256;
  const long long tiles = (n + 63) / 64;
  return (int)(tiles < cap ? (tiles < 1 ? 1 : tiles) : cap);
}

namespace {
template <typename R, int TILE>
hipError_t launch_pool_stage1(const void *x, long long n, int nr, int nc, int n_entries, int blocks, double *partials, hipStream_t stream, bool tiled) {
  const size_t lds = (size_t)(nr + 2 * nc + nr + nc) * (size_t)(TILE + 1) * sizeof(R);
  if (lds > 64 * 1024)
    if (hipError_t rc = raise_lds_limit<k_pool_reduce<R, TILE>>(kPoolLdsLimit); rc != hipSuccess) return rc;
  for (int base = 0; base < n_entries; base += kMaxEntries * kBlockThreads)
    hipLaunchKernelGGL((k_pool_reduce<R, TILE>), dim3((unsigned)blocks), dim3(kBlockThreads), lds, stream, (const R *)x, n, nr, nc, base,
                       tiled ? 1 : 0, partials);
  return hipGetLastError();
}
template <typename R>
hipError_t launch_pool_stage1_tile(int tile, const void *x, long long n, int nr, int nc, int n_entries, int blocks, double *partials, hipStream_t stream, bool tiled) {
  switch (tile) {
    case 64: return launch_pool_stage1<R, 64>(x, n, nr, nc, n_entries, blocks, partials, stream, tiled);
    case 32: return launch_pool_stage1<R, 32>(x, n, nr, nc, n_entries, blocks, partials, stream, tiled);
    case 16: return launch_pool_stage1<R, 16>(x, n, nr, nc, n_entries, blocks, partials, stream, tiled);
    default: return hipErrorInvalidValue;
  }
}
}

hipError_t launch_pool_reduce(const void *x, long long n, int nr, int nc, int dtype, const unsigned long long *slots,
                              long long n_slots, double proposed, double *partials, double *out_device,
                              hipStream_t stream,
                              hipError_t (*stage1)(const void *, long long, double *, int, hipStream_t), bool tiled_state) {
  const int d = nr + 2 * nc;
  const int n_aug = d + nr + nc;
  const int n_entries = 1 + n_aug + d * (d + 1) / 2;
  const int tile = pool_tile_chains(nr, nc, dtype);
  if (!stage1 && tile == 0) return hipErrorInvalidValue;
  const int blocks = pool_reduce_blocks(n, nr, nc);
  hipError_t err;
  if (stage1) err = stage1(x, n, partials, blocks, stream);
  else if (dtype == ME_F32) err = launch_pool_stage1_tile<float>(tile, x, n, nr, nc, n_entries, blocks, partials, stream, tiled_state);
  else err = launch_pool_stage1_tile<double>(tile, x, n, nr, nc, n_entries, blocks, partials, stream, tiled_state);
  if (err != hipSuccess) return err;
  hipLaunchKernelGGL(k_pool_finish, dim3((unsigned)((n_entries + 63) / 64 + 1)), dim3(kFinishThreads), 0, stream,
                     (const double *)partials, blocks, nr, nc, slots, n_slots, proposed, out_device);
  return hipGetLastError();
}

}
```

metropolisengine_amd/csrc/me_internal.h:

```cpp
#pragma once

#include <hip/hip_runtime.h>
#include <stdint.h>

#include "../../include/metropolis_engine.h"

namespace me {

enum CovKind { CK_IDENTITY = 0, CK_SHARED = 1, CK_PER_CHAIN = 2, CK_PER_CHAIN_NT = 3 };

enum StepGroup { GROUP_ALL = 0, GROUP_REAL = 1, GROUP_COMPLEX = 2 };

enum StatusBits : uint32_t {
  ST_NONFINITE_ENERGY = 1u,
  ST_BAD_PIVOT = 2u,
  ST_BAD_WIDTH = 4u
};

long long cache_budget_bytes();
void set_cache_budget_bytes(long long bytes);

constexpr int kBlockThreads = 256;
#ifndef ME_STEP_THREADS
#define ME_STEP_THREADS 64
// ... 24 lines not shown
  int stale_total;
  const void *cov;
  double reject_bound, temp, ratio, target_acceptance, damping;
  const void *ladder;
  int tiles_per_rung;
};

struct MeasureLaunch {
  int n_real, n_complex;
  void *x, *width, *mean, *cov, *obs_mean, *factor;
  unsigned int *status;
  long long n;
  unsigned long long measure_count;
  int update_cov;
  int split_widths;
  int write_factor;
  int grid_blocks;
};

struct EnergyLaunch {
  int n_real, n_complex;
  int total_row;
  void *x, *energy;
  const void *coef_device;
  const double *coef_host;
  int n_coef;
  unsigned int *status;
  long long n;
  int energy_kind, grid_blocks;
};

constexpr int kMaxRegisterDof = 96;

struct KernelSet {
  const char *user_name;
  int dtype, n_real, n_complex;
  bool per_chain_cov;
  bool tracks_cov;
  bool (*has_energy)(int energy_kind);
  int (*energy_terms)(int energy_kind);
  hipError_t (*step)(const StepLaunch &, hipStream_t);
  hipError_t (*magphase)(const StepLaunch &, hipStream_t);
  hipError_t (*measure)(const MeasureLaunch &, hipStream_t);
  hipError_t (*init_energy)(const EnergyLaunch &, hipStream_t);
  size_t matrix_image_bytes;
  hipError_t (*prepare_matrix)(const void *matrix, void *image, hipStream_t);
  hipError_t (*pool_stage1)(const void *x, long long n, double *partials, int n_rows, hipStream_t);
  bool has_user_reject;
  bool streams_packed;
  hipError_t (*cycle)(const StepLaunch &, const MeasureLaunch &, hipStream_t);
  bool tiled_state;
};

void register_kernel_set(const KernelSet *set);
const KernelSet *find_kernel_set(int dtype, int n_real, int n_complex, int energy_kind, const char *user_name);
bool has_dims(int dtype, int n_real, int n_complex);

hipError_t launch_broadcast_rows(void *dst, const void *row_values, int rows, long long n, int dtype,
                                 hipStream_t stream);
hipError_t launch_broadcast_tiled(void *dst, const void *entry_values, int entries, long long n, int dtype,
                                  hipStream_t stream);
hipError_t launch_pool_reduce(const void *x, long long n, int n_real, int n_complex, int dtype,
                              const unsigned long long *slots, long long n_slots, double proposed, double *partials,
                              double *out_device, hipStream_t stream,
                              hipError_t (*stage1)(const void *, long long, double *, int, hipStream_t) = nullptr,
                              bool tiled_state = false);
int pool_reduce_blocks(long long n, int n_real, int n_complex);
bool pool_reduce_supported(int n_real, int n_complex, int dtype);
int pool_tile_chains(int n_real, int n_complex, int dtype);
hipError_t launch_trace(const void *x, const void *energy, const void *width, long long n, int d, int n_terms,
                        int width_rows, int dtype, long long n_traced, long long stride, double *out, hipStream_t stream,
                        bool tiled_state = false);
hipError_t launch_sum_slots(const unsigned long long *slots, long long n_slots, unsigned long long *total,
                            hipStream_t stream);

inline int grid_for(long long n, int requested, int threads = kStepThreads) {
  long long blocks = (n + threads - 1) / threads;
  if (requested > 0 && blocks > requested) blocks = requested;
  if (blocks < 1) blocks = 1;
  return (int)blocks;
}

__host__ __device__ inline int packed_real(int nr) { return nr * (nr + 1) / 2; }
__host__ __device__ inline int packed_total(int nr, int nc) { return nr * (nr + 1) / 2 + nc * nc; }
__host__ __device__ inline int n_observables(int nr, int nc) { return 2 * nr + nc; }
__host__ __device__ inline long long moments_size(int nr, int nc) {
  const int d = nr + 2 * nc;
  return 1 + d + (long long)d * (d + 1) / 2 + n_observables(nr, nc) + 2;
}

}
```

metropolisengine_amd/csrc/me_kernels.hip:

```cpp
#include <type_traits>

#include "me_device.h"
#include "me_dense_mfma.h"
#include "me_dense_bf16x3.h"
#include "me_dense_f64.h"
#include "me_factor_tile.h"
#include "me_per_device.h"
#include "me_pool_gram.h"
#include "me_magphase.h"

#ifdef ME_USER_SOURCE
#include ME_USER_SOURCE
#endif

#ifndef ME_NR
#error "compile with -DME_NR=<n_real> -DME_NC=<n_complex>"
#endif
#ifndef ME_DENSE
#define ME_DENSE 0
#endif
#ifndef ME_PER_CHAIN
#define ME_PER_CHAIN 1
#endif
#ifndef ME_TRACK_COV
// ... 61 lines not shown
  return fn;
}
#endif

int energy_terms(int kind) {
#ifdef ME_USER_SOURCE
#ifdef ME_USER_N_TERMS
  if (kind == ME_ENERGY_USER) return ME_USER_N_TERMS;
#else
  if (kind == ME_ENERGY_USER) return 1;
#endif
  return kind == ME_ENERGY_USER_INDIRECT ? 1 : 0;
#endif
  switch (kind) {
    case ME_ENERGY_ISO_QUAD:
    case ME_ENERGY_DIAG_QUAD: return 1;
    case ME_ENERGY_DENSE_QUAD: return ME_DENSE != 0 ? 1 : 0;
    case ME_ENERGY_LANDAU_TOY: return kLandau ? 1 : 0;
    case ME_ENERGY_LANDAU_TERMS: return kLandau ? 2 : 0;
    case ME_ENERGY_CYLINDER: return kCylinder ? 1 : 0;
    default: return 0;
  }
}
bool has_energy(int kind) { return energy_terms(kind) > 0; }

template <typename R, class Energy, bool INJECT, int GROUP, bool LADDER>
hipError_t launch_step_cov(const StepLaunch &l, const StepArgs<R> &a, const Energy &en, dim3 grid, dim3 block,
                           hipStream_t stream) {
  switch (l.cov_kind) {
    case CK_IDENTITY: {
      constexpr long long state_bytes = (long long)sizeof(R) * (D + 2);
      if constexpr (!INJECT && GROUP == GROUP_ALL && !LADDER) {
        if (state_bytes * l.n > 2 * cache_budget_bytes()) {
          hipLaunchKernelGGL((k_step<R, NR, NC, Energy, CK_IDENTITY, INJECT, GROUP, true>), grid, block, 0, stream, a, en);
          break;
        }
      }
      hipLaunchKernelGGL((k_step<R, NR, NC, Energy, CK_IDENTITY, INJECT, GROUP, false, LADDER>), grid, block, 0, stream, a, en);
      break;
    }
    case CK_SHARED: hipLaunchKernelGGL((k_step<R, NR, NC, Energy, CK_SHARED, INJECT, GROUP, false, LADDER>), grid, block, 0, stream, a, en); break;
#if ME_PER_CHAIN == 2
    case CK_PER_CHAIN: {
      if constexpr (INJECT) return hipErrorInvalidValue;
      else hipLaunchKernelGGL((k_step<R, NR, NC, Energy, CK_PER_CHAIN_NT, INJECT, GROUP, false, LADDER>), grid, block, 0, stream, a, en);
      break;
    }
#elif ME_PER_CHAIN
    case CK_PER_CHAIN: {
      constexpr long long per_chain_bytes = (long long)sizeof(R) * (D + 2 + NR * (NR + 1) / 2 + NC * NC);
      if constexpr (!INJECT) {
        if (per_chain_bytes * l.n > cache_budget_bytes()) {
          hipLaunchKernelGGL((k_step<R, NR, NC, Energy, CK_PER_CHAIN_NT, INJECT, GROUP, false, LADDER>), grid, block, 0, stream, a, en);
          break;
        }
      }
      hipLaunchKernelGGL((k_step<R, NR, NC, Energy, CK_PER_CHAIN, INJECT, GROUP, false, LADDER>), grid, block, 0, stream, a, en);
      break;
    }
#endif
    default: return hipErrorInvalidValue;
  }
  return hipGetLastError();
}

template <typename R, class Energy, bool INJECT, bool LADDER = false>
hipError_t launch_step_group(const StepLaunch &l, const StepArgs<R> &a, const Energy &en, dim3 grid, dim3 block,
                             hipStream_t stream) {
  if (l.group == GROUP_ALL) return launch_step_cov<R, Energy, INJECT, GROUP_ALL, LADDER>(l, a, en, grid, block, stream);
  if constexpr (NR > 0 && NC > 0) {
    if (l.group == GROUP_REAL) return launch_step_cov<R, Energy, INJECT, GROUP_REAL, LADDER>(l, a, en, grid, block, stream);
    if (l.group == GROUP_COMPLEX) return launch_step_cov<R, Energy, INJECT, GROUP_COMPLEX, LADDER>(l, a, en, grid, block, stream);
  }
  return hipErrorInvalidValue;
}

template <typename R, class Energy>
hipError_t step_with(const StepLaunch &l, const Energy &en, hipStream_t stream) {
  const StepArgs<R> a = typed<R>(l);
  const bool per_chain = l.cov_kind == CK_PER_CHAIN;
  const int threads = (l.n_sweeps >= kFusedSweepsThreshold || (ME_PER_CHAIN == 2 && per_chain)) ? kFusedStepThreads : kStepThreads;
  const dim3 grid(grid_for(l.n, l.grid_blocks, threads)), block(threads);
  if (l.ladder) {
    if (l.inj_normals) {
      if constexpr (std::is_same<R, double>::value) {
        if (l.group != GROUP_ALL || l.cov_kind != CK_IDENTITY) return hipErrorNotSupported;
        hipLaunchKernelGGL((k_step<R, NR, NC, Energy, CK_IDENTITY, true, GROUP_ALL, false, true>), grid, block, 0, stream, a, en);
        return hipGetLastError();
      } else return hipErrorNotSupported;
    }
#if ME_DENSE && !defined(ME_USER_SOURCE)
    if constexpr (NR == 64 && NC == 0 && std::is_same<Energy, EnergyDense<R, 64, 0>>::value) return hipErrorNotSupported;
    else
#endif
      return launch_step_group<R, Energy, false, true>(l, a, en, grid, block, stream);
  }
  if (l.inj_normals) {
    if constexpr (std::is_same<R, double>::value) return launch_step_group<R, Energy, true>(l, a, en, grid, block, stream);
    else return hipErrorNotSupported;
  }
#if ME_DENSE && !defined(ME_USER_SOURCE)
  if constexpr (std::is_same<R, float>::value && NR == 64 && NC == 0 &&
                std::is_same<Energy, EnergyDense<float, 64, 0>>::value) {
    if (per_chain) return launch_step_group<R, Energy, false>(l, a, en, grid, block, stream);
    if (dense64_exact_fp32_mfma()) {
      if (l.cov_kind == CK_IDENTITY)
        return launch_step_dense64_mfma<CK_IDENTITY>(a, en.a, nullptr, l.grid_blocks, stream);
      if (l.cov_kind == CK_SHARED && l.factor_full)
        return launch_step_dense64_mfma<CK_SHARED>(a, en.a, (const float *)l.factor_full, l.grid_blocks, stream);
      return hipErrorInvalidValue;
    }
    if (!l.energy_image) return hipErrorInvalidValue;
    if (l.cov_kind == CK_IDENTITY)
      return launch_step_dense64_bf16x3<CK_IDENTITY>(a, (const unsigned int *)l.energy_image, nullptr, l.grid_blocks, stream);
    if (l.cov_kind == CK_SHARED && l.factor_image)
      return launch_step_dense64_bf16x3<CK_SHARED>(a, (const unsigned int *)l.energy_image,
                                                   (const unsigned int *)l.factor_image, l.grid_blocks, stream);
    return hipErrorInvalidValue;
  } else if constexpr (std::is_same<R, double>::value && NR == 64 && NC == 0 &&
                       std::is_same<Energy, EnergyDense<double, 64, 0>>::value) {
// ... 120 lines not shown
    hipLaunchKernelGGL((k_init_energy<R, NR, NC, Energy>), dim3(grid_for(l.n, l.grid_blocks)), dim3(kStepThreads), 0,
                       stream, (const R *)l.x, (R *)l.energy, l.n, l.status, en, l.total_row);
    return hipGetLastError();
  });
}

#ifndef ME_FACTOR_TILE
#define ME_FACTOR_TILE 1
#endif
#ifndef ME_CYCLE
#define ME_CYCLE (ME_PER_CHAIN == 1)
#endif
template <typename R>
hipError_t cycle(const StepLaunch &l, const MeasureLaunch &ml, hipStream_t stream) {
#if ME_CYCLE
  constexpr int P = NR * (NR + 1) / 2 + NC * NC;
  if constexpr (P <= kMaxPackedInRegisters) {
    if (l.group != GROUP_ALL || l.inj_normals || !ml.cov || !ml.factor) return hipErrorNotSupported;
    if (l.cov_kind != CK_IDENTITY && l.cov_kind != CK_PER_CHAIN) return hipErrorNotSupported;
    return with_energy<R>(l.energy_kind, l.coef_host, l.n_coef, l.coef_device, [&](const auto &en) -> hipError_t {
      using Energy = std::decay_t<decltype(en)>;
#if ME_DENSE && !defined(ME_USER_SOURCE)
      if constexpr (NR == 64 && NC == 0 && std::is_same<Energy, EnergyDense<R, 64, 0>>::value) return hipErrorNotSupported;
#endif
      const StepArgs<R> a = typed<R>(l);
      const MeasureArgs<R> ma = typed_measure<R>(ml);
      constexpr long long mean_bytes = (long long)sizeof(R) * (2 * D + (2 * NR + NC));
      constexpr long long all_bytes = mean_bytes + (long long)sizeof(R) * (2 + 2 * P);
      const bool nt = all_bytes * l.n > cache_budget_bytes(), ntm = mean_bytes * l.n > cache_budget_bytes();
      const int threads = l.n_sweeps >= kFusedSweepsThreshold ? kFusedStepThreads : kStepThreads;
      const dim3 grid(grid_for(l.n, l.grid_blocks, threads)), block(threads);
      auto launch = [&](auto ck) {
        constexpr int CK = decltype(ck)::value;
        if (l.ladder && nt) hipLaunchKernelGGL((k_cycle<R, NR, NC, Energy, CK, true, true, true>), grid, block, 0, stream, a, ma, en);
        else if (l.ladder) hipLaunchKernelGGL((k_cycle<R, NR, NC, Energy, CK, false, false, true>), grid, block, 0, stream, a, ma, en);
        else if (ntm) hipLaunchKernelGGL((k_cycle<R, NR, NC, Energy, CK, true, true>), grid, block, 0, stream, a, ma, en);
        else if (nt) hipLaunchKernelGGL((k_cycle<R, NR, NC, Energy, CK, true, false>), grid, block, 0, stream, a, ma, en);
        else hipLaunchKernelGGL((k_cycle<R, NR, NC, Energy, CK, false, false>), grid, block, 0, stream, a, ma, en);
      };
      if (l.cov_kind == CK_PER_CHAIN) launch(std::integral_constant<int, CK_PER_CHAIN>{});
      else launch(std::integral_constant<int, CK_IDENTITY>{});
      return hipGetLastError();
    });
  }
#endif
  return hipErrorNotSupported;
}

template <typename R>
hipError_t measure(const MeasureLaunch &l, hipStream_t stream) {
  const MeasureArgs<R> a = typed_measure<R>(l);
  constexpr int P = NR * (NR + 1) / 2 + NC * NC;
  constexpr bool kFused = ME_PER_CHAIN == 1;
  static_assert(ME_PER_CHAIN != 1 || P <= kMaxPackedInRegisters, "ME_PER_CHAIN=1 keeps the packed matrix in registers");
  const dim3 grid(grid_for(l.n, l.grid_blocks)), block(kStepThreads);
  constexpr long long mean_bytes = (long long)sizeof(R) * (2 * D + (2 * NR + NC));
  constexpr long long all_bytes = mean_bytes + (long long)sizeof(R) * 2 * P;
  const bool nt = all_bytes * l.n > cache_budget_bytes(), ntm = mean_bytes * l.n > cache_budget_bytes();
  constexpr bool kCov = (ME_PER_CHAIN != 0 || ME_TRACK_COV != 0);
  if (l.cov) {
    if (ntm) hipLaunchKernelGGL((k_measure<R, NR, NC, kCov, kFused, true, true>), grid, block, 0, stream, a);
    else if (nt) hipLaunchKernelGGL((k_measure<R, NR, NC, kCov, kFused, true, false>), grid, block, 0, stream, a);
    else hipLaunchKernelGGL((k_measure<R, NR, NC, kCov, kFused, false, false>), grid, block, 0, stream, a);
  } else {
    if (ntm) hipLaunchKernelGGL((k_measure<R, NR, NC, false, false, false, true>), grid, block, 0, stream, a);
    else hipLaunchKernelGGL((k_measure<R, NR, NC, false, false, false, false>), grid, block, 0, stream, a);
  }
#if ME_PER_CHAIN == 2
  static_assert(P > kMaxPackedInRegisters, "ME_PER_CHAIN=2 is for spaces with more than 160 packed entries");
  if (l.cov && l.update_cov && l.write_factor) {
    if constexpr (NC > 0) {
// ... 32 lines not shown
  if constexpr (NR == 64 && NC == 0) {
    hipLaunchKernelGGL(k_dense64_bf16_fragments<0>, dim3(1), dim3(256), 0, stream, (const float *)factor_full,
                       (unsigned int *)image);
    return hipGetLastError();
  }
  return hipSuccess;
}
[[maybe_unused]] constexpr size_t kMatrixImageBytes = (NR == 64 && NC == 0) ? sizeof(unsigned int) * kBf16FragWords : 0;
#define ME_PREPARE_MATRIX_F32 kMatrixImageBytes, (kMatrixImageBytes ? prepare_matrix_f32 : nullptr), pool_stage1_f32()
hipError_t prepare_matrix_f64(const void *matrix, void *image, hipStream_t stream) {
  if constexpr (NR == 64 && NC == 0) {
    hipLaunchKernelGGL(k_dense64_f64_fragments<0>, dim3(1), dim3(256), 0, stream, (const double *)matrix, (double *)image);
    return hipGetLastError();
  }
  return hipSuccess;
}
[[maybe_unused]] constexpr size_t kMatrixImageBytesF64 = (NR == 64 && NC == 0) ? sizeof(double) * kDense64F64ImageDoubles : 0;
#define ME_PREPARE_MATRIX_F64 kMatrixImageBytesF64, (kMatrixImageBytesF64 ? prepare_matrix_f64 : nullptr), pool_stage1_f64()
#else
#define ME_PREPARE_MATRIX_F32 0, nullptr, pool_stage1_f32()
#define ME_PREPARE_MATRIX_F64 0, nullptr, pool_stage1_f64()
#endif
#ifdef ME_USER_HAS_REJECT
constexpr bool kHasUserReject = true;
#else
constexpr bool kHasUserReject = false;
#endif
#ifndef ME_ONLY_DTYPE
#define ME_ONLY_DTYPE 0
#endif
#if ME_ONLY_DTYPE != 64
const KernelSet kSetF32 = {ME_SET_NAME, ME_F32, NR, NC, ME_PER_CHAIN != 0, (ME_PER_CHAIN != 0 || ME_TRACK_COV != 0), has_energy, energy_terms, step<float>,
                           (NC > 0 && ME_PER_CHAIN == 1) ? magphase<float> : nullptr, measure<float>, init_energy<float>,
                           ME_PREPARE_MATRIX_F32, kHasUserReject, ME_PER_CHAIN == 2, cycle<float>, D >= kTiledStateDof};
#endif
#if ME_ONLY_DTYPE != 32
const KernelSet kSetF64 = {ME_SET_NAME, ME_F64, NR, NC, ME_PER_CHAIN != 0, (ME_PER_CHAIN != 0 || ME_TRACK_COV != 0), has_energy, energy_terms, step<double>,
                           (NC > 0 && ME_PER_CHAIN == 1) ? magphase<double> : nullptr, measure<double>, init_energy<double>,
                           ME_PREPARE_MATRIX_F64, kHasUserReject, ME_PER_CHAIN == 2, cycle<double>, D >= kTiledStateDof};
#endif

struct Registrar {
  Registrar() {
#if ME_ONLY_DTYPE != 64
    register_kernel_set(&kSetF32);
#endif
#if ME_ONLY_DTYPE != 32
    register_kernel_set(&kSetF64);
#endif
  }
} registrar;

}
}
```

metropolisengine_amd/csrc/me_mbar_obs.hip:

```cpp
#include "me_mbar.h"

#pragma clang fp contract(off)

namespace me {
namespace mbar {
namespace {

constexpr int kObsTargets = 4;
constexpr int kObsCols = 4;

struct ObsSelection {
  int q[ME_MAX_RECORDED_OBSERVABLES];
};

template <typename R>
__global__ void __launch_bounds__(kThreads) k_observable_record(const R *__restrict__ x, const R *__restrict__ energy, long long n,
                                                                 int nr, int nc, int n_terms, int tiled, ObsSelection sel,
                                                                 int n_sel, double *dst) {
  const long long c = (long long)blockIdx.x * kThreads + threadIdx.x;
  if (c >= n) return;
  const int d = nr + 2 * nc, nobs = 2 * nr + nc;
  const long long x0 = tiled ? (c >> 6) * (long long)d * 64 + (c & 63) : c;
  const long long xs = tiled ? 64 : n;
  for (int j = 0; j < n_sel; ++j) {
    const int q = sel.q[j];
    double v;
    if (q < d) {
      v = (double)x[x0 + (long long)q * xs];
    } else if (q < d + nobs) {
      const int o = q - d;
      if (o < nr) {
        v = fabs((double)x[x0 + (long long)o * xs]);
      } else if (o < nr + nc) {
        const double re = (double)x[x0 + (long long)o * xs], im = (double)x[x0 + (long long)(o + nc) * xs];
        v = __builtin_sqrt(__builtin_fma(re, re, im * im));
      } else {
        const double xr = (double)x[x0 + (long long)(o - nr - nc) * xs];
        v = xr * xr;
      }
    } else {
      v = (double)energy[(long long)(q - d - nobs) * n + c];
    }
    dst[(long long)j * n + c] = v;
  }
}

struct TargetState {
  double M, W, Q2, mean_e;
  double mean[kObsCols], M2[kObsCols], C[kObsCols];
};
static_assert(sizeof(TargetState) == 16 * sizeof(double), "partials are addressed as 16 doubles per state");

__device__ __forceinline__ void clear(TargetState &s) {
  s.M = -INFINITY;
  s.W = s.Q2 = s.mean_e = 0.0;
#pragma unroll
// ... 223 lines not shown

hipError_t reweight_observables_enqueue(Problem &p, const MbarSamples &sm, const ObsColumns &oc, const double *inv_temps, int n_temps,
                                        ObsScratch &scratch, double *out) {
  hipStream_t stream = p.stream;
  const int n_blocks = blocks_of(sm.n_samples), nq_all = oc.n_columns;
  const long long n_tiles = tiles_of(sm.n_samples);
  const size_t cells = (size_t)n_temps * nq_all;
  ME_MBAR_HIP(log_denominator_enqueue(p, sm, scratch.d));
  ME_MBAR_HIP(scratch.partials.resize((size_t)n_blocks * kObsTargets * sizeof(TargetState)));
  double *o_mean = out, *o_var = o_mean + cells, *o_cov = o_var + cells, *o_neff = o_cov + cells;
  for (int t0 = 0; t0 < n_temps; t0 += kObsTargets) {
    const int nt = std::min(kObsTargets, n_temps - t0);
    for (int q0 = 0; q0 < nq_all; q0 += kObsCols) {
      const int nq = std::min(kObsCols, nq_all - q0);
      const size_t cell = (size_t)t0 * nq_all + q0;
      hipLaunchKernelGGL(k_mbar_reweight_obs, dim3(n_blocks), dim3(kThreads), 0, stream, sm.energies, scratch.d.get<const double>(),
                         oc.data + (size_t)q0 * oc.column_stride, sm.n_samples, oc.n_chains, oc.record_stride, oc.column_stride, nq,
                         inv_temps + t0, nt, n_tiles, scratch.partials.get<TargetState>());
      hipLaunchKernelGGL(k_mbar_reweight_obs_finish, dim3(nt), dim3(kThreads), 0, stream, scratch.partials.get<const TargetState>(),
                         n_blocks, nq, nq_all, p.n_used, q0 == 0 ? 1 : 0, o_mean + cell, o_var + cell, o_cov + cell, o_neff + t0);
    }
  }
  return hipGetLastError();
}

hipError_t observable_record_enqueue(me_engine *e, long long row) {
  me_engine::Samples &s = e->samples;
  ObsSelection sel;
  for (int j = 0; j < ME_MAX_RECORDED_OBSERVABLES; ++j) sel.q[j] = j < s.n_obs ? s.obs_index[j] : 0;
  double *dst = s.obs.get<double>() + (size_t)row * (size_t)s.n_obs * (size_t)e->n;
  const dim3 grid((unsigned)((e->n + kThreads - 1) / kThreads));
  if (e->dtype == ME_F32)
    hipLaunchKernelGGL(k_observable_record<float>, grid, dim3(kThreads), 0, e->stream, e->x.get<const float>(), e->energy.get<const float>(),
                       e->n, e->nr, e->nc, e->n_terms, e->x_tiled ? 1 : 0, sel, s.n_obs, dst);
  else
    hipLaunchKernelGGL(k_observable_record<double>, grid, dim3(kThreads), 0, e->stream, e->x.get<const double>(),
                       e->energy.get<const double>(), e->n, e->nr, e->nc, e->n_terms, e->x_tiled ? 1 : 0, sel, s.n_obs, dst);
  return hipGetLastError();
}

}
}

using namespace me;
using namespace me::mbar;

extern "C" {

int me_observable_samples_enable(me_engine *e, const int32_t *indices, int32_t n_observables) {
  if (!e) return ME_ERR_INVALID;
  const int rc = refuse_stale_total(e, "observable samples are");
  if (rc != ME_OK) return rc;
  if (n_observables < 0 || n_observables > ME_MAX_RECORDED_OBSERVABLES)
    return fail(e, ME_ERR_INVALID, "n_observables must lie in [0, " + std::to_string(ME_MAX_RECORDED_OBSERVABLES) + "]");
  me_engine::Samples &s = e->samples;
  ME_HIP(e, hipSetDevice(e->device));
  if (n_observables == 0) {
    ME_HIP(e, hipStreamSynchronize(e->stream));
    s.obs.reset();
    s.n_obs = 0;
    return ME_OK;
  }
  if (!s.data) return fail(e, ME_ERR_STATE, "observable samples need the energy store: call me_energy_samples_enable first");
  if (!indices) return fail(e, ME_ERR_INVALID, "indices missing");
  for (int j = 0; j < n_observables; ++j)
    if (indices[j] < 0 || indices[j] >= catalogue_size(e))
      return fail(e, ME_ERR_INVALID, "observable index " + std::to_string(indices[j]) + " outside the catalogue of " +
                                         std::to_string(catalogue_size(e)) + " quantities");
  ME_HIP(e, hipStreamSynchronize(e->stream));
  s.obs.reset();
// ... 72 lines not shown
```

metropolisengine_amd/csrc/me_population.hip:

```cpp
#include <algorithm>
#include <cmath>
#include <vector>

#include "me_device.h"
#include "me_engine.h"

namespace me {
namespace {

constexpr int kPopThreads = 256;
constexpr int kPopWaves = kPopThreads / 64;
constexpr int kPopItems = 8;
constexpr int kPopChunk = kPopThreads * kPopItems;
constexpr int kFinalThreads = 256;
constexpr long long kSerialSlots = 8;

struct PopParams {
  double M, W, u;
  long long hi;
  long long n_finite;
};

template <typename R>
__device__ __forceinline__ double chain_log_weight(const Field<R> &fe, long long c, long long n, int n_terms, double neg_dbeta,
// ... 224 lines not shown
      up = slot_bound(o + f * q, N, p.W, p.u, p.hi);
    }
    const bool long_run = up - lo > kSerialSlots;
    if (!long_run)
      for (long long j = lo; j < up; ++j) ancestors[j] = (unsigned int)c;
    unsigned long long runs = __ballot(long_run);
    while (runs) {
      const int src = __ffsll((long long)runs) - 1;
      runs &= runs - 1;
      const long long run_lo = __shfl(lo, src), run_up = __shfl(up, src);
      const unsigned int run_c = (unsigned int)__shfl(c, src);
      for (long long j = run_lo + (threadIdx.x & 63); j < run_up; j += 64) ancestors[j] = run_c;
    }
  }
}

template <class F>
__device__ __forceinline__ void copy_rows(const F &src, const F &dst, unsigned int src_off, unsigned int dst_off, int rows) {
  constexpr int B = 8;
  for (int r0 = 0; r0 < rows; r0 += B) {
    decltype(src.load(0, 0u)) v[B];
#pragma unroll
    for (int k = 0; k < B; ++k)
      if (r0 + k < rows) v[k] = src.load(r0 + k, src_off);
#pragma unroll
    for (int k = 0; k < B; ++k)
      if (r0 + k < rows) dst.store(r0 + k, dst_off, v[k]);
  }
}

template <typename R>
__global__ void __launch_bounds__(kPopThreads) k_pop_gather(const R *x, const R *energy, const long long *fam, R *x_out,
                                                           R *energy_out, long long *fam_out, long long n, int d, int n_terms,
                                                           int tiled, const unsigned int *ancestors, const PopParams *params) {
  const long long j = (long long)blockIdx.x * kPopThreads + threadIdx.x;
  if (j >= n) return;
  const long long hi = params->hi;
  const long long a = (long long)ancestors[j < hi ? j : hi - 1];
  const unsigned int a_off = (unsigned int)a * (unsigned int)sizeof(R), j_off = (unsigned int)j * (unsigned int)sizeof(R);
  if (tiled) copy_rows(TiledField<R>(x, n, d), TiledField<R>(x_out, n, d), tiled_offset<R>(a, d), tiled_offset<R>(j, d), d);
  else copy_rows(Field<R>(x, n, d), Field<R>(x_out, n, d), a_off, j_off, d);
  copy_rows(Field<R>(energy, n, n_terms), Field<R>(energy_out, n, n_terms), a_off, j_off, n_terms);
  fam_out[j] = fam[a];
}

__global__ void __launch_bounds__(kPopThreads) k_pop_init_families(long long *fam, long long n, unsigned long long chain_offset) {
  const long long j = (long long)blockIdx.x * kPopThreads + threadIdx.x;
  if (j < n) fam[j] = (long long)(chain_offset + (unsigned long long)j);
}

template <typename R>
hipError_t launch(me_engine *e, double neg_dbeta) {
  me_engine::Population &pop = e->population;
  const long long n = e->n;
  hipStream_t stream = e->stream;
  const int n_blocks = (int)((n + kPopChunk - 1) / kPopChunk);
  const unsigned slot_blocks = (unsigned)((n + kPopThreads - 1) / kPopThreads);
  double *partials = pop.scratch.get<double>(), *factors = partials + 4 * (size_t)n_blocks, *offsets = factors + n_blocks;
  PopParams *params = (PopParams *)(offsets + n_blocks + 1);
  double *record = pop.records.get<double>() + 3 * (size_t)pop.stages;
  hipLaunchKernelGGL(k_pop_weights<R>, dim3(n_blocks), dim3(kPopThreads), 0, stream, e->energy.get<const R>(), n, e->n_terms,
                     neg_dbeta, partials);
  hipLaunchKernelGGL(k_pop_finalize, dim3(1), dim3(kFinalThreads), 0, stream, (const double *)partials, n_blocks, n,
                     e->chain_offset, pop.stages, (uint32_t)e->seed, (uint32_t)(e->seed >> 32), factors, offsets, params, record);
  hipLaunchKernelGGL(k_pop_scan_ancestors<R>, dim3(n_blocks), dim3(kPopThreads), 0, stream, e->energy.get<const R>(), n,
                     e->n_terms, neg_dbeta, (const double *)partials, (const double *)factors, (const double *)offsets,
                     (const PopParams *)params, pop.anc.get<unsigned int>());
  hipLaunchKernelGGL(k_pop_gather<R>, dim3(slot_blocks), dim3(kPopThreads), 0, stream, e->x.get<const R>(), e->energy.get<const R>(),
                     pop.fam.get<const long long>(), pop.x.get<R>(), pop.energy.get<R>(), pop.fam_out.get<long long>(), n, e->d,
                     e->n_terms, e->x_tiled ? 1 : 0, pop.anc.get<const unsigned int>(), (const PopParams *)params);
  return hipGetLastError();
}

size_t population_scratch_doubles(long long n) {
  const long long n_blocks = (n + kPopChunk - 1) / kPopChunk;
  return (size_t)(4 * n_blocks + n_blocks + n_blocks + 1) + (sizeof(PopParams) + sizeof(double) - 1) / sizeof(double);
}

int ensure_families(me_engine *e) {
  me_engine::Population &pop = e->population;
  if (pop.fam) return ME_OK;
  ME_HIP(e, pop.fam.resize((size_t)e->n * sizeof(long long)));
  hipLaunchKernelGGL(k_pop_init_families, dim3((unsigned)((e->n + kPopThreads - 1) / kPopThreads)), dim3(kPopThreads), 0, e->stream,
                     pop.fam.get<long long>(), e->n, e->chain_offset);
  ME_HIP(e, hipGetLastError());
  return ME_OK;
}
int ensure_population_scratch(me_engine *e) {
  me_engine::Population &pop = e->population;
  const size_t energy_bytes = (size_t)e->n * (size_t)e->n_terms * e->esize;
  if (pop.energy.bytes() < energy_bytes) {
    if (pop.energy) ME_HIP(e, hipStreamSynchronize(e->stream));
    ME_HIP(e, pop.energy.reserve(energy_bytes));
  }
  if (!pop.x) {
    ME_HIP(e, pop.x.resize(e->x.bytes()));
    ME_HIP(e, hipMemcpyAsync(pop.x.get(), e->x.get(), pop.x.bytes(), hipMemcpyDeviceToDevice, e->stream));
  }
  ME_HIP(e, pop.fam_out.resize((size_t)e->n * sizeof(long long)));
  ME_HIP(e, pop.anc.resize((size_t)e->n * sizeof(unsigned int)));
  ME_HIP(e, pop.scratch.resize(population_scratch_doubles(e->n) * sizeof(double)));
  return ME_OK;
}
// ... 129 lines not shown
```

metropolisengine_amd/csrc/me_replica.hip:

```cpp
#include <algorithm>
#include <cmath>
#include <string>
#include <vector>

#include "me_device.h"
#include "me_engine.h"

namespace me {
namespace {

constexpr int kSwapThreads = 256;
constexpr int kSwapBlocks = 2048;

template <typename R>
struct SwapArgs {
  R *x, *energy;
  const R *ladder;
  unsigned long long *pair_counts;
  long long n, rung_chains;
  unsigned long long chain_offset, round;
  uint32_t seed_lo, seed_hi;
  int d, n_terms, first_rung, tiled;
};

template <class F>
__device__ __forceinline__ void swap_rows(const F &f, unsigned int off_a, unsigned int off_b, int rows) {
  constexpr int B = 8;
  for (int r0 = 0; r0 < rows; r0 += B) {
    decltype(f.load(0, 0u)) va[B], vb[B];
#pragma unroll
    for (int u = 0; u < B; ++u)
      if (r0 + u < rows) {
        va[u] = f.load(r0 + u, off_a);
        vb[u] = f.load(r0 + u, off_b);
      }
#pragma unroll
    for (int u = 0; u < B; ++u)
      if (r0 + u < rows) {
        f.store(r0 + u, off_a, vb[u]);
        f.store(r0 + u, off_b, va[u]);
      }
  }
}

template <typename R>
__device__ __forceinline__ bool swap_pair(const SwapArgs<R> &s, const Field<R> &fe, int k, long long j, R dbeta, R dbeta_log2e) {
  using N_ = Num<R>;
  const long long a = (long long)k * s.rung_chains + j, b = a + s.rung_chains;
  const unsigned int ea_off = (unsigned int)a * (unsigned int)sizeof(R), eb_off = (unsigned int)b * (unsigned int)sizeof(R);
  const R ea = chain_energy(fe, ea_off, s.n_terms), eb = chain_energy(fe, eb_off, s.n_terms);
  const unsigned long long gid = s.chain_offset + (unsigned long long)a;
  U4 ctr;
  ctr.x = (uint32_t)gid;
  ctr.y = (uint32_t)(gid >> 32);
  ctr.z = (uint32_t)s.round;
  ctr.w = ((uint32_t)(s.round >> 32) << 16) | 0xffffu;
  const R u = N_::unit(philox4x32_10(ctr, s.seed_lo, s.seed_hi).x);
  const R delta = dbeta * (ea - eb);
  const bool accept = N_::finite(ea) && N_::finite(eb) && (delta >= R(0) || N_::uphill(u, eb - ea, dbeta, dbeta_log2e));
  if (accept) {
    if (s.tiled) swap_rows(TiledField<R>(s.x, s.n, s.d), tiled_offset<R>(a, s.d), tiled_offset<R>(b, s.d), s.d);
    else swap_rows(Field<R>(s.x, s.n, s.d), ea_off, eb_off, s.d);
    swap_rows(fe, ea_off, eb_off, s.n_terms);
  }
  return accept;
}

template <typename R>
__global__ void __launch_bounds__(kSwapThreads) k_replica_swap(SwapArgs<R> s) {
  const int k = s.first_rung + 2 * (int)blockIdx.y;
  const Field<R> fe(s.energy, s.n, s.n_terms);
  const R dbeta = s.ladder[2 * k] - s.ladder[2 * k + 2], dbeta_log2e = s.ladder[2 * k + 1] - s.ladder[2 * k + 3];
  unsigned int attempted = 0, accepted = 0;
  for (long long j = (long long)blockIdx.x * kSwapThreads + threadIdx.x; j < s.rung_chains; j += (long long)gridDim.x * kSwapThreads) {
    const bool acc = swap_pair(s, fe, k, j, dbeta, dbeta_log2e);
    attempted += (unsigned int)__popcll(__ballot(true));
    accepted += (unsigned int)__popcll(__ballot(acc));
  }
  __shared__ unsigned int wave_counts[kSwapThreads / 64][2];
  if ((threadIdx.x & 63) == 0) {
    wave_counts[threadIdx.x >> 6][0] = attempted;
    wave_counts[threadIdx.x >> 6][1] = accepted;
  }
  __syncthreads();
  if (threadIdx.x < 2) {
    unsigned long long total = 0;
#pragma unroll
    for (int w = 0; w < kSwapThreads / 64; ++w) total += wave_counts[w][threadIdx.x];
    if (total) atomicAdd(&s.pair_counts[2 * k + threadIdx.x], total);
  }
}

template <typename R>
hipError_t launch(void *x, void *energy, long long n, int d, int n_terms, bool tiled_state, const void *ladder, int n_rungs,
                  unsigned long long round, unsigned long long chain_offset, unsigned long long seed,
                  unsigned long long *pair_counts, hipStream_t stream) {
  SwapArgs<R> s;
  s.x = (R *)x;
  s.energy = (R *)energy;
  s.ladder = (const R *)ladder;
  s.pair_counts = pair_counts;
  s.n = n;
  s.rung_chains = n / n_rungs;
  s.first_rung = (int)(round & 1ull);
  const int n_pairs = (n_rungs - s.first_rung) / 2;
  s.chain_offset = chain_offset;
  s.round = round;
  s.seed_lo = (uint32_t)seed;
  s.seed_hi = (uint32_t)(seed >> 32);
  s.d = d;
  s.n_terms = n_terms;
  s.tiled = tiled_state ? 1 : 0;
  if (n_pairs == 0) return hipSuccess;
  const long long per_pair = std::min<long long>((s.rung_chains + kSwapThreads - 1) / kSwapThreads, std::max(kSwapBlocks / n_pairs, 1));
  hipLaunchKernelGGL(k_replica_swap<R>, dim3((unsigned)per_pair, (unsigned)n_pairs), dim3(kSwapThreads), 0, stream, s);
  return hipGetLastError();
}

int check_ladder_capable(me_engine *e) {
  if (e->ks->n_real < 0)
    return fail(e, ME_ERR_UNSUPPORTED, "temperature ladders are not available on the runtime-dimension kernel set (beyond " +
                                           std::to_string(kMaxRegisterDof) + " real degrees of freedom)");
  if (e->energy_kind == ME_ENERGY_DENSE_QUAD && e->nr == 64 && e->nc == 0)
    return fail(e, ME_ERR_UNSUPPORTED, "temperature ladders are not available on the matrix-core kernels of the dense 64-parameter form");
  return refuse_stale_total(e, "temperature ladders are");
}
int free_ladder(me_engine *e) {
  ME_HIP(e, hipStreamSynchronize(e->stream));
  e->ladder = me_engine::Ladder();
  e->samples.rows = 0;
  return ME_OK;
}
}
}

using namespace me;

extern "C" {

int me_set_temperature_ladder(me_engine *e, const double *temps, int32_t n_rungs) {
  if (!e) return ME_ERR_INVALID;
  if (n_rungs < 0 || (n_rungs > 0 && !temps)) return fail(e, ME_ERR_INVALID, "n_rungs must be >= 0 and temps given");
  ME_HIP(e, hipSetDevice(e->device));
  if (n_rungs == 0) return free_ladder(e);
  int rc = check_ladder_capable(e);
// ... 6 lines not shown
  }
  if (e->n % (64ll * n_rungs) != 0)
    return fail(e, ME_ERR_INVALID, "n_chains must be a multiple of 64 * n_rungs: every rung is a run of whole 64-chain tiles");
  std::vector<double> table(2 * (size_t)n_rungs);
  for (int k = 0; k < n_rungs; ++k) {
    table[2 * k] = 1.0 / temps[k];
    table[2 * k + 1] = 1.4426950408889634 / temps[k];
  }
  if ((rc = free_ladder(e)) != ME_OK) return rc;
  ME_HIP(e, upload(e->ladder.table, table.data(), table.size(), e->dtype));
  ME_HIP(e, e->ladder.pair_counts.resize(2 * (size_t)std::max(n_rungs - 1, 1) * sizeof(unsigned long long)));
  ME_HIP(e, hipMemset(e->ladder.pair_counts.get(), 0, e->ladder.pair_counts.bytes()));
  e->ladder.temps.assign(temps, temps + n_rungs);
  e->ladder.n_rungs = n_rungs;
  return ME_OK;
}

int me_temperature_ladder(me_engine *e, double *temps, int32_t capacity, int32_t *n_rungs) {
  if (!e || !n_rungs) return ME_ERR_INVALID;
  *n_rungs = e->ladder.n_rungs;
  if (e->ladder.n_rungs == 0 || !temps) return ME_OK;
  if (capacity < e->ladder.n_rungs) return fail(e, ME_ERR_INVALID, "temps must hold n_rungs doubles");
  std::copy(e->ladder.temps.begin(), e->ladder.temps.end(), temps);
  return ME_OK;
}

int me_replica_exchange(me_engine *e, int32_t n_rounds) {
  if (!e) return ME_ERR_INVALID;
  if (n_rounds < 0) return fail(e, ME_ERR_INVALID, "n_rounds must be >= 0");
  if (e->ladder.n_rungs == 0) return fail(e, ME_ERR_STATE, "no temperature ladder: call me_set_temperature_ladder first");
  ME_HIP(e, hipSetDevice(e->device));
  const auto swap = e->dtype == ME_F32 ? launch<float> : launch<double>;
  for (int i = 0; i < n_rounds; ++i) {
    ME_HIP(e, swap(e->x.get(), e->energy.get(), e->n, e->d, e->n_terms, e->x_tiled, e->ladder.table.get(), e->ladder.n_rungs, e->ladder.round,
                   e->chain_offset, e->seed, e->ladder.pair_counts.get<unsigned long long>(), e->stream));
    e->ladder.round += 1;
  }
  return ME_OK;
}

int me_replica_stats(me_engine *e, uint64_t *round, uint64_t *attempted, uint64_t *accepted, int32_t n_pairs) {
  if (!e) return ME_ERR_INVALID;
  if (e->ladder.n_rungs == 0) return fail(e, ME_ERR_STATE, "no temperature ladder");
  if (n_pairs != e->ladder.n_rungs - 1) return fail(e, ME_ERR_INVALID, "n_pairs must be n_rungs - 1");
  if (round) *round = e->ladder.round;
  if (n_pairs == 0) return ME_OK;
  ME_HIP(e, hipSetDevice(e->device));
  std::vector<unsigned long long> counts(2 * (size_t)n_pairs);
  ME_HIP(e, hipMemcpyAsync(counts.data(), e->ladder.pair_counts.get(), counts.size() * sizeof(unsigned long long), hipMemcpyDeviceToHost,
                           e->stream));
  ME_HIP(e, hipStreamSynchronize(e->stream));
  for (int k = 0; k < n_pairs; ++k) {
    if (attempted) attempted[k] = counts[2 * k];
    if (accepted) accepted[k] = counts[2 * k + 1];
  }
  return ME_OK;
}

int me_set_replica_stats(me_engine *e, uint64_t round, const uint64_t *attempted, const uint64_t *accepted, int32_t n_pairs) {
  if (!e) return ME_ERR_INVALID;
  if (e->ladder.n_rungs == 0) return fail(e, ME_ERR_STATE, "no temperature ladder");
  if (n_pairs != e->ladder.n_rungs - 1) return fail(e, ME_ERR_INVALID, "n_pairs must be n_rungs - 1");
  if (n_pairs > 0 && (!attempted || !accepted)) return fail(e, ME_ERR_INVALID, "attempted / accepted missing");
  std::vector<unsigned long long> counts(2 * (size_t)n_pairs);
  for (int k = 0; k < n_pairs; ++k) {
    if (accepted[k] > attempted[k]) return fail(e, ME_ERR_INVALID, "accepted swaps exceed attempted ones");
    counts[2 * k] = attempted[k];
// ... 14 lines not shown
```

Before: 18.71 billion.

## Add per-chain line state layout and generalize tiled state indexing

Adds a third state layout (per-chain contiguous "line" rows) alongside the component-major and 64-chain tiled layouts, selected per dtype and dimension through state_layout_of. Device loads and stores, host copies, replica swaps, population gather, observable recording and pooled reductions all now go through a generic state_index or layout field. The aim is to make each chain's parameters contiguous for some dtype/dimension combinations, such as f64 at 16 parameters, which may improve cache-line use in the step kernel. In exchange, per-thread accesses stop being coalesced across chains, and runtime layout dispatch is added to the auxiliary kernels.

```diff
diff --git a/include/metropolis_engine.h b/include/metropolis_engine.h
--- a/include/metropolis_engine.h
+++ b/include/metropolis_engine.h
@@ -262,6 +262,9 @@
 
 int me_supported(int32_t dtype, int32_t n_real, int32_t n_complex, int32_t energy_kind);
 
+int me_state_layout(int32_t dtype, int32_t n_real, int32_t n_complex, int32_t *layout);
+int me_state_index(int32_t layout, int64_t chain, int32_t row, int32_t d, int64_t n, int64_t *index);
+
 int me_detect_equilibration(int32_t device_id, const double *series, int64_t n_series, int64_t length, int32_t fast,
                             int32_t nskip, int64_t *t0, double *g, double *neff_max);
 
diff --git a/metropolisengine_amd/_capi.py b/metropolisengine_amd/_capi.py
--- a/metropolisengine_amd/_capi.py
+++ b/metropolisengine_amd/_capi.py
@@ -100,6 +100,9 @@
     "me_time_steps": (ctypes.c_int, [_H, ctypes.c_int32, ctypes.c_int32, ctypes.POINTER(ctypes.c_float)]),
     "me_last_error": (ctypes.c_int, [_H, ctypes.c_char_p, ctypes.c_size_t]),
     "me_supported": (ctypes.c_int, [ctypes.c_int32, ctypes.c_int32, ctypes.c_int32, ctypes.c_int32]),
+    "me_state_layout": (ctypes.c_int, [ctypes.c_int32, ctypes.c_int32, ctypes.c_int32, ctypes.POINTER(ctypes.c_int32)]),
+    "me_state_index": (ctypes.c_int, [ctypes.c_int32, ctypes.c_int64, ctypes.c_int32, ctypes.c_int32, ctypes.c_int64,
+                                      ctypes.POINTER(ctypes.c_int64)]),
     "me_set_temperature_ladder": (ctypes.c_int, [_H, _dp, ctypes.c_int32]),
     "me_temperature_ladder": (ctypes.c_int, [_H, _dp, ctypes.c_int32, ctypes.POINTER(ctypes.c_int32)]),
     "me_replica_exchange": (ctypes.c_int, [_H, ctypes.c_int32]),
diff --git a/metropolisengine_amd/csrc/me_api.hip b/metropolisengine_amd/csrc/me_api.hip
--- a/metropolisengine_amd/csrc/me_api.hip
+++ b/metropolisengine_amd/csrc/me_api.hip
@@ -168,11 +168,12 @@
 
 namespace {
 
-int broadcast(me_engine *e, DeviceBuffer &dst, const std::vector<double> &row, bool tiled = false) {
+int broadcast(me_engine *e, DeviceBuffer &dst, const std::vector<double> &row, int layout = ME_STATE_COMPONENT_MAJOR) {
   std::vector<unsigned char> bytes;
   to_device_type(row.data(), row.size(), e->dtype, bytes);
   ME_HIP(e, hipMemcpyAsync(e->row_dev.get(), bytes.data(), bytes.size(), hipMemcpyHostToDevice, e->stream));
-  if (tiled) ME_HIP(e, launch_broadcast_tiled(dst.get(), e->row_dev.get(), (int)row.size(), e->n, e->dtype, e->stream));
+  if (layout != ME_STATE_COMPONENT_MAJOR)
+    ME_HIP(e, launch_broadcast_tiled(dst.get(), e->row_dev.get(), (int)row.size(), e->n, e->dtype, e->stream, layout));
   else ME_HIP(e, launch_broadcast_rows(dst.get(), e->row_dev.get(), (int)row.size(), e->n, e->dtype, e->stream));
   ME_HIP(e, hipStreamSynchronize(e->stream));
   return ME_OK;
@@ -189,9 +190,8 @@
     for (int64_t c = 0; c < n_chains; ++c) t[(size_t)r * n_chains + c] = (T)src[c * comps + r];
 }
 template <typename T>
-void transpose_tiled(T *t, int entries, int64_t tile0, int64_t chain_begin, int64_t n_chains, double *dst, const double *src) {
-  const size_t tile_values = (size_t)entries * 64;
-  auto at = [&](int64_t c, int k) { return (size_t)((c >> 6) - tile0) * tile_values + (size_t)k * 64 + (size_t)(c & 63); };
+void transpose_tiled(T *t, int layout, int entries, int64_t chain0, int64_t chain_begin, int64_t n_chains, double *dst, const double *src) {
+  auto at = [&](int64_t c, int k) { return (size_t)state_index(layout, c - chain0, k, entries, 0); };
   for (int64_t i = 0; i < n_chains; ++i)
     for (int k = 0; k < entries; ++k) {
       if (dst) dst[i * entries + k] = (double)t[at(chain_begin + i, k)];
@@ -199,18 +199,20 @@
     }
 }
 
-int copy_tiled(me_engine *e, void *field_ptr, int entries, int64_t chain_begin, int64_t n_chains, double *dst, const double *src) {
-  const int64_t tile0 = chain_begin >> 6, tile1 = (chain_begin + n_chains - 1) >> 6;
-  const size_t tile_values = (size_t)entries * 64, n_values = (size_t)(tile1 - tile0 + 1) * tile_values;
-  unsigned char *dev = (unsigned char *)field_ptr + (size_t)tile0 * tile_values * e->esize;
+int copy_tiled(me_engine *e, void *field_ptr, int entries, int64_t chain_begin, int64_t n_chains, double *dst, const double *src,
+               int layout = ME_STATE_TILE_MAJOR) {
+  const bool line = layout == ME_STATE_LINE;
+  const int64_t tile0 = chain_begin >> 6, tile1 = (chain_begin + n_chains - 1) >> 6, chain0 = line ? chain_begin : tile0 * 64;
+  const size_t n_values = (size_t)(line ? n_chains : (tile1 - tile0 + 1) * 64) * (size_t)entries;
+  unsigned char *dev = (unsigned char *)field_ptr + (size_t)state_index(layout, chain0, 0, entries, 0) * e->esize;
   std::vector<unsigned char> tmp(n_values * e->esize);
-  const bool whole = (chain_begin & 63) == 0 && (((chain_begin + n_chains) & 63) == 0 || chain_begin + n_chains == e->n);
+  const bool whole = line || ((chain_begin & 63) == 0 && (((chain_begin + n_chains) & 63) == 0 || chain_begin + n_chains == e->n));
   if (dst || !whole) {
     ME_HIP(e, hipMemcpyAsync(tmp.data(), dev, tmp.size(), hipMemcpyDeviceToHost, e->stream));
     ME_HIP(e, hipStreamSynchronize(e->stream));
   }
-  if (e->dtype == ME_F32) transpose_tiled(reinterpret_cast<float *>(tmp.data()), entries, tile0, chain_begin, n_chains, dst, src);
-  else transpose_tiled(reinterpret_cast<double *>(tmp.data()), entries, tile0, chain_begin, n_chains, dst, src);
+  if (e->dtype == ME_F32) transpose_tiled(reinterpret_cast<float *>(tmp.data()), layout, entries, chain0, chain_begin, n_chains, dst, src);
+  else transpose_tiled(reinterpret_cast<double *>(tmp.data()), layout, entries, chain0, chain_begin, n_chains, dst, src);
   if (src) {
     ME_HIP(e, hipMemcpyAsync(dev, tmp.data(), tmp.size(), hipMemcpyHostToDevice, e->stream));
     ME_HIP(e, hipStreamSynchronize(e->stream));
@@ -333,6 +335,21 @@
   return find_kernel_set(dtype, n_real, n_complex, energy_kind, nullptr) ? 1 : 0;
 }
 
+int me_state_layout(int32_t dtype, int32_t n_real, int32_t n_complex, int32_t *layout) {
+  if (!layout) return ME_ERR_INVALID;
+  const KernelSet *ks = find_kernel_set(dtype, n_real, n_complex, ME_ENERGY_ISO_QUAD, nullptr);
+  if (!ks) return ME_ERR_UNSUPPORTED;
+  *layout = ks->state_layout;
+  return ME_OK;
+}
+
+int me_state_index(int32_t layout, int64_t chain, int32_t row, int32_t d, int64_t n, int64_t *index) {
+  if (!index || layout < ME_STATE_COMPONENT_MAJOR || layout > ME_STATE_LINE || chain < 0 || chain >= n || row < 0 || row >= d)
+    return ME_ERR_INVALID;
+  *index = state_index(layout, chain, row, d, n);
+  return ME_OK;
+}
+
 namespace {
 
 int validate_config(const me_config *c, const KernelSet **ks_out) {
@@ -407,7 +424,7 @@
 struct Layout {
   bool keep_per_chain;
   bool keep_cov;
-  bool x_tiled;
+  int x_layout;
   int width_rows;
 };
 int decide_layout(const me_config *c, const KernelSet *ks, Layout &l) {
@@ -426,7 +443,7 @@
                 "a per-chain field would exceed 4 GiB on this engine; shard the chains over more engines");
   l.keep_cov = l.keep_per_chain ||
                ((!ks->per_chain_cov || ks->streams_packed) && ks->tracks_cov && (c->flags & ME_FLAG_TRACK_COVARIANCE));
-  l.x_tiled = ks->tiled_state;
+  l.x_layout = ks->state_layout;
   l.width_rows = (c->n_real > 0 && c->n_complex > 0) ? 3 : 1;
   return ME_OK;
 }
@@ -458,7 +475,7 @@
   e->ratio = (1.0 - 1.0 / e->m) * std::sqrt(2.0 * M_PI) * std::exp(e->alpha * e->alpha / 2.0) / 2.0 * e->alpha +
              1.0 / (e->m * c->target_acceptance * (1.0 - c->target_acceptance));
   if (const char *g = std::getenv("ME_GRID_BLOCKS")) e->grid_blocks = std::atoi(g);
-  e->x_tiled = l.x_tiled;
+  e->x_layout = l.x_layout;
   e->stale_total = (c->flags & ME_FLAG_REFERENCE_ENERGY_LEDGERS) != 0;
   e->width_rows = l.width_rows;
   e->n_slots = (e->n + 31) / 32 + 8;
@@ -470,7 +487,7 @@
   ME_HIP(e, hipSetDevice(e->device));
   ME_HIP(e, e->stream.create());
   const size_t n = (size_t)e->n, tiles = (size_t)padded_chains(e->n), es = e->esize;
-  ME_HIP(e, e->x.resize((e->x_tiled ? tiles : n) * e->d * es));
+  ME_HIP(e, e->x.resize((size_t)state_field_values(e->x_layout, e->d, e->n) * es));
   ME_HIP(e, e->energy.resize(n * (e->n_terms + (e->stale_total ? 1 : 0)) * es));
   ME_HIP(e, e->width.resize(n * e->width_rows * es));
   ME_HIP(e, e->mean.resize(n * e->d * es));
@@ -560,9 +577,9 @@
     return fail(e, ME_ERR_INVALID, "initial covariance matrix is not positive definite (metropolis_engine.py:270)");
   int rc = ME_OK;
   std::vector<double> width_row((size_t)e->width_rows, c->sampling_width);
-  if ((rc = broadcast(e, e->x, init, e->x_tiled)) || (rc = broadcast(e, e->mean, init)) || (rc = broadcast(e, e->obs_mean, obs)) ||
-      (rc = broadcast(e, e->width, width_row)) || (e->cov && (rc = broadcast(e, e->cov, c0, true))) ||
-      (e->factor && (rc = broadcast(e, e->factor, f0, true))) || (rc = upload_shared_factor(e, f0.data())))
+  if ((rc = broadcast(e, e->x, init, e->x_layout)) || (rc = broadcast(e, e->mean, init)) || (rc = broadcast(e, e->obs_mean, obs)) ||
+      (rc = broadcast(e, e->width, width_row)) || (e->cov && (rc = broadcast(e, e->cov, c0, ME_STATE_TILE_MAJOR))) ||
+      (e->factor && (rc = broadcast(e, e->factor, f0, ME_STATE_TILE_MAJOR))) || (rc = upload_shared_factor(e, f0.data())))
     return rc;
   e->cov_kind = identity ? CK_IDENTITY : (e->ks->n_real < 0 && e->factor) ? CK_PER_CHAIN : CK_SHARED;
   return ME_OK;
@@ -618,7 +635,7 @@
     return fail(e, ME_ERR_UNSUPPORTED, is_user_kind(energy_kind)
                     ? std::string("no user-energy plugin named '") + (user_name ? user_name : "") + "' is loaded for these dimensions"
                     : "energy kind " + std::to_string(energy_kind) + " is not compiled for these dimensions");
-  if (ks->tiled_state != e->ks->tiled_state || ks->per_chain_cov != e->ks->per_chain_cov || ks->streams_packed != e->ks->streams_packed ||
+  if (ks->state_layout != e->ks->state_layout || ks->per_chain_cov != e->ks->per_chain_cov || ks->streams_packed != e->ks->streams_packed ||
       ks->tracks_cov != e->ks->tracks_cov)
     return fail(e, ME_ERR_UNSUPPORTED, "me_set_energy: the plugin was built with other per-chain covariance options than this engine's kernel set");
   if (e->reject_kind == ME_REJECT_USER && !ks->has_user_reject)
@@ -813,7 +830,7 @@
     const int rows_valid = (e->width_rows == 3 && e->widths_synced) ? 1 : e->width_rows;
     double *row = e->trace.dev.get<double>() + e->trace.rows * cols * e->trace.chains;
     ME_HIP(e, launch_trace(e->x.get(), e->energy.get(), e->width.get(), e->n, e->d, e->n_terms, rows_valid, e->dtype, e->trace.chains,
-                           e->trace.stride, row, e->stream, e->x_tiled));
+                           e->trace.stride, row, e->stream, e->x_layout));
     if (rows_valid != e->width_rows) {
       double *widths = row + (size_t)(e->d + e->n_terms) * e->trace.chains;
       for (int r = 1; r < 3; ++r)
@@ -919,8 +936,8 @@
   int rc = field_info(e, field, &ptr, &comps);
   if (rc != ME_OK) return rc;
   if (n_chains == 0) return ME_OK;
-  if (field == ME_FIELD_COV || field == ME_FIELD_FACTOR || (field == ME_FIELD_PARAMS && e->x_tiled))
-    return copy_tiled(e, ptr, comps, chain_begin, n_chains, dst, nullptr);
+  if (field == ME_FIELD_COV || field == ME_FIELD_FACTOR || (field == ME_FIELD_PARAMS && e->x_layout != ME_STATE_COMPONENT_MAJOR))
+    return copy_tiled(e, ptr, comps, chain_begin, n_chains, dst, nullptr, field == ME_FIELD_PARAMS ? e->x_layout : ME_STATE_TILE_MAJOR);
   std::vector<unsigned char> tmp((size_t)comps * n_chains * e->esize);
   for (int r = 0; r < comps; ++r)
     ME_HIP(e, hipMemcpyAsync(tmp.data() + (size_t)r * n_chains * e->esize,
@@ -945,8 +962,8 @@
   if (field == ME_FIELD_WIDTH && e->width_rows == 3 && (chain_begin != 0 || n_chains != e->n))
     return fail(e, ME_ERR_INVALID, "widths of a mixed engine must be set for all chains at once");
   if (n_chains == 0) return ME_OK;
-  if (field == ME_FIELD_COV || field == ME_FIELD_FACTOR || (field == ME_FIELD_PARAMS && e->x_tiled)) {
-    rc = copy_tiled(e, ptr, comps, chain_begin, n_chains, nullptr, src);
+  if (field == ME_FIELD_COV || field == ME_FIELD_FACTOR || (field == ME_FIELD_PARAMS && e->x_layout != ME_STATE_COMPONENT_MAJOR)) {
+    rc = copy_tiled(e, ptr, comps, chain_begin, n_chains, nullptr, src, field == ME_FIELD_PARAMS ? e->x_layout : ME_STATE_TILE_MAJOR);
     if (rc != ME_OK) return rc;
     if (field == ME_FIELD_FACTOR) e->cov_kind = CK_PER_CHAIN;
     return ME_OK;
@@ -1054,7 +1071,7 @@
 }
 int enqueue_pool_reduce(me_engine *e, const void *x, long long n_chains, long long n_slots, double proposed, double *device_out) {
   hipError_t err = launch_pool_reduce(x, n_chains, e->nr, e->nc, e->dtype, e->accept_slots.get<unsigned long long>(), n_slots, proposed,
-                                      e->pool.partials.get<double>(), device_out, e->stream, e->ks->pool_stage1, e->x_tiled);
+                                      e->pool.partials.get<double>(), device_out, e->stream, e->ks->pool_stage1, e->x_layout);
   if (err == hipErrorInvalidValue) return fail(e, ME_ERR_UNSUPPORTED, "pooled moments: dimension too large for the reduction kernel");
   ME_HIP(e, err);
   return ME_OK;
@@ -1093,8 +1110,8 @@
   int rc = check_pooled(e, n_doubles);
   if (rc != ME_OK) return rc;
   const unsigned char *x = e->x.get<unsigned char>();
-  if (e->x_tiled) {
-    x += (size_t)chain_begin * e->d * e->esize;
+  if (e->x_layout != ME_STATE_COMPONENT_MAJOR) {
+    x += (size_t)state_index(e->x_layout, chain_begin, 0, e->d, e->n) * e->esize;
   } else {
     const size_t row = (size_t)n_chains * e->esize;
     if (row * e->d > e->pool.range_x.bytes()) {
diff --git a/metropolisengine_amd/csrc/me_device.h b/metropolisengine_amd/csrc/me_device.h
--- a/metropolisengine_amd/csrc/me_device.h
+++ b/metropolisengine_amd/csrc/me_device.h
@@ -235,28 +235,134 @@
 #define ME_TILED_STATE_DOF 16
 #endif
 constexpr int kTiledStateDof = ME_TILED_STATE_DOF;
+template <typename R, int D>
+constexpr int kStateLayout = state_layout_of((int)sizeof(R), D, kTiledStateDof);
 template <typename R, int D, bool NTS = false>
 struct XField {
-  static constexpr bool kTiled = D >= kTiledStateDof;
+  static constexpr int kLayout = kStateLayout<R, D>;
+  static constexpr bool kLine = kLayout == ME_STATE_LINE;
+  static constexpr bool kTiled = kLayout != ME_STATE_COMPONENT_MAJOR;
   std::conditional_t<kTiled, TiledField<R>, StateField<R, NTS>> f;
   __device__ __forceinline__ XField(const R *base, long long n) : f(base, n, D) {}
   static __device__ __forceinline__ unsigned int offset(long long c) {
-    if constexpr (kTiled) return tiled_offset<R>(c, D);
-    else return (unsigned int)c * (unsigned int)sizeof(R);
-  }
+    return (unsigned int)(state_index(kLayout, c, 0, D, 0) * (long long)sizeof(R));
+  }
+  static constexpr unsigned int kRowBytes = (unsigned int)((state_index(kLayout, 0, 1, D, 0) - state_index(kLayout, 0, 0, D, 0)) * (long long)sizeof(R));
   __device__ __forceinline__ R load(int row, unsigned int off) const {
-    if constexpr (kTiled && NTS) return f.load_nt(row, off);
+    if constexpr (kLine) return bit_load<NTS ? ME_NT_AUX : 0>(f.rsrc, off, (unsigned int)row * kRowBytes);
+    else if constexpr (kTiled && NTS) return f.load_nt(row, off);
     else return f.load(row, off);
   }
   __device__ __forceinline__ void store(int row, unsigned int off, R value) const {
-    if constexpr (kTiled && NTS) f.store_nt(row, off, value);
+    if constexpr (kLine) bit_store<NTS ? ME_NT_AUX : 0>(f.rsrc, off, (unsigned int)row * kRowBytes, value);
+    else if constexpr (kTiled && NTS) f.store_nt(row, off, value);
     else f.store(row, off, value);
+  }
+  template <int AUX>
+  static __device__ __forceinline__ R bit_load(__amdgpu_buffer_rsrc_t rsrc, unsigned int voff, unsigned int soff) {
+    if constexpr (sizeof(R) == 4) return __builtin_bit_cast(R, __builtin_amdgcn_raw_buffer_load_b32(rsrc, voff, soff, AUX));
+    else return __builtin_bit_cast(R, __builtin_amdgcn_raw_buffer_load_b64(rsrc, voff, soff, AUX));
+  }
+  template <int AUX>
+  static __device__ __forceinline__ void bit_store(__amdgpu_buffer_rsrc_t rsrc, unsigned int voff, unsigned int soff, R value) {
+    if constexpr (sizeof(R) == 4) {
+      __builtin_amdgcn_raw_buffer_store_b32(__builtin_bit_cast(unsigned int, value), rsrc, voff, soff, AUX);
+    } else {
+      using v2 = decltype(__builtin_amdgcn_raw_buffer_load_b64(rsrc, 0u, 0u, 0));
+      __builtin_amdgcn_raw_buffer_store_b64(__builtin_bit_cast(v2, value), rsrc, voff, soff, AUX);
+    }
   }
 };
 template <typename R, int D>
 __device__ __forceinline__ long long state_index(long long c, int row, long long n) {
-  if constexpr (D >= kTiledStateDof) return ((c >> 6) * (long long)D + row) * 64 + (c & 63);
-  else return (long long)row * n + c;
+  return state_index(kStateLayout<R, D>, c, row, D, n);
+}
+
+template <typename R>
+struct LayoutField : Field<R> {
+  int layout, d;
+  long long n;
+  __device__ __forceinline__ LayoutField(const R *base, long long n_, int d_, int layout_) : Field<R>(base, n_, d_), layout(layout_), d(d_), n(n_) {
+    this->rsrc = __builtin_amdgcn_make_buffer_rsrc(const_cast<R *>(base), 0,
+                                                   (unsigned int)(state_field_values(layout, d, n) * (long long)sizeof(R)), 0x00020000);
+    this->row_bytes = (unsigned int)((state_index(layout, 0, 1, d, n) - state_index(layout, 0, 0, d, n)) * (long long)sizeof(R));
+  }
+  __device__ __forceinline__ unsigned int offset(long long c) const {
+    return (unsigned int)(state_index(layout, c, 0, d, n) * (long long)sizeof(R));
+  }
+};
+
+constexpr int kLineSlabBytes = 8192;
+template <typename R, int D, int AUX>
+struct LineTile {
+  static_assert(sizeof(R) * D == 128, "a chain is one 128-byte line");
+  static constexpr int VPP = 16 / (int)sizeof(R);
+  typedef unsigned int Piece __attribute__((ext_vector_type(4)));
+  struct Values { R v[VPP]; };
+  static __device__ __forceinline__ int swizzle(int c) { return ((c >> 1) & 3) | ((((c >> 3) ^ c) & 1) << 2); }
+  static __device__ __forceinline__ Piece *slab() {
+    extern __shared__ __attribute__((aligned(16))) unsigned char line_slabs[];
+    return reinterpret_cast<Piece *>(line_slabs + (threadIdx.x >> 6) * kLineSlabBytes);
+  }
+  static __device__ __forceinline__ int lane() {
+    int l = (int)(threadIdx.x & 63u);
+    asm volatile("" : "+v"(l));
+    return l;
+  }
+  static __device__ __forceinline__ void wave_sync() {
+    __builtin_amdgcn_fence(__ATOMIC_RELEASE, "wavefront");
+    __builtin_amdgcn_wave_barrier();
+    __builtin_amdgcn_fence(__ATOMIC_ACQUIRE, "wavefront");
+  }
+  static __device__ __forceinline__ void load(__amdgpu_buffer_rsrc_t rsrc, unsigned int tile_bytes, R (&x)[D]) {
+    Piece *s = slab();
+    const int l = lane();
+    const unsigned int voff = tile_bytes + (unsigned int)l * 16u;
+    Piece in[8];
+#pragma unroll
+    for (int i = 0; i < 8; ++i) in[i] = __builtin_amdgcn_raw_buffer_load_b128(rsrc, voff, i * 1024, AUX);
+    wave_sync();
+#pragma unroll
+    for (int i = 0; i < 8; ++i) {
+      const int chain = 8 * i + (l >> 3);
+      s[chain * 8 + ((l & 7) ^ swizzle(chain))] = in[i];
+    }
+    wave_sync();
+#pragma unroll
+    for (int p = 0; p < 8; ++p) {
+      const Values v = __builtin_bit_cast(Values, s[l * 8 + (p ^ swizzle(l))]);
+#pragma unroll
+      for (int k = 0; k < VPP; ++k) x[p * VPP + k] = v.v[k];
+    }
+  }
+  static __device__ __forceinline__ void store(__amdgpu_buffer_rsrc_t rsrc, unsigned int tile_bytes, const R (&x)[D], unsigned long long moved) {
+    if (moved == 0ull) return;
+    Piece *s = slab();
+    const int l = lane();
+    const unsigned int voff = tile_bytes + (unsigned int)l * 16u;
+    wave_sync();
+#pragma unroll
+    for (int p = 0; p < 8; ++p) {
+      Values v;
+#pragma unroll
+      for (int k = 0; k < VPP; ++k) v.v[k] = x[p * VPP + k];
+      s[l * 8 + (p ^ swizzle(l))] = __builtin_bit_cast(Piece, v);
+    }
+    wave_sync();
+    Piece out[8];
+#pragma unroll
+    for (int i = 0; i < 8; ++i) {
+      const int chain = 8 * i + (l >> 3);
+      out[i] = s[chain * 8 + ((l & 7) ^ swizzle(chain))];
+    }
+#pragma unroll
+    for (int i = 0; i < 8; ++i)
+      if ((moved >> (8 * i + (l >> 3))) & 1ull) __builtin_amdgcn_raw_buffer_store_b128(out[i], rsrc, voff, i * 1024, AUX);
+  }
+};
+template <typename R, int D>
+constexpr unsigned int step_lds_bytes(int threads) {
+  return kStateLayout<R, D> == ME_STATE_LINE ? (unsigned int)(threads / 64 * kLineSlabBytes) : 0u;
 }
 
 constexpr int kMaxPackedInRegisters = 160;
@@ -660,7 +766,7 @@
 __device__ __forceinline__ void decide_step(const StepArgs<R> &a, long long c, const Energy &en, bool stale_total, R u,
                                             const R (&g)[2 * ((NR + 2 * NC + 1) / 2)], R (&x)[NR + 2 * NC], const R (&xp)[NR + 2 * NC],
                                             Ledger &ledger, R &total_q5, R &w, R &w_r, R &w_c, unsigned int &wave_accepted,
-                                            bool &bad_energy) {
+                                            bool &moved, bool &bad_energy) {
   [[maybe_unused]] constexpr int D = NR + 2 * NC;
   constexpr bool MOVE_REAL = NR > 0 && GROUP != GROUP_COMPLEX;
   constexpr bool MOVE_COMPLEX = NC > 0 && GROUP != GROUP_REAL;
@@ -700,19 +806,20 @@
   else if constexpr (GROUP == GROUP_REAL) w_r = w;
   else w_c = w;
   wave_accepted += (unsigned int)__popcll(__ballot(accept));
+  moved |= accept;
 }
 
 template <typename R, int NR, int NC, class Energy, int CK, bool INJECT, int GROUP, bool LADDER, class Ledger, class Fac>
 __device__ __forceinline__ void run_sweeps(const StepArgs<R> &a, const Energy &en, long long c, unsigned long long gid,
                                            bool stale_total, R (&x)[NR + 2 * NC], Ledger &ledger, R &total_q5, R &w, R &w_r,
-                                           R &w_c, Fac &&fac, unsigned int &wave_accepted, bool &bad_energy) {
+                                           R &w_c, Fac &&fac, unsigned int &wave_accepted, bool &moved, bool &bad_energy) {
   constexpr int D = NR + 2 * NC;
   constexpr int NW = 2 * ((D + 1) / 2);
   for (int s = 0; s < a.n_sweeps; ++s) {
     R g[NW], u, xp[D];
     draw_step<R, NR, NC, INJECT>(a, c, gid, s, g, u);
     propose_registers<R, NR, NC, CK, GROUP>(x, g, w_r, w_c, fac, xp);
-    decide_step<R, NR, NC, Energy, CK, GROUP, LADDER>(a, c, en, stale_total, u, g, x, xp, ledger, total_q5, w, w_r, w_c, wave_accepted, bad_energy);
+    decide_step<R, NR, NC, Energy, CK, GROUP, LADDER>(a, c, en, stale_total, u, g, x, xp, ledger, total_q5, w, w_r, w_c, wave_accepted, moved, bad_energy);
   }
 }
 
@@ -762,12 +869,19 @@
   constexpr bool STREAM_FACTOR = PER_CHAIN && (PF > kMaxPackedInRegisters ||
                                                (!INJECT && sizeof(R) == 8 && NC == 0 && PF > kStreamF64Entries));
   const TiledField<R> ffac(a.factor, a.n, STREAM_FACTOR ? 0 : PF);
-  for (long long c = (long long)blockIdx.x * blockDim.x + threadIdx.x; c < a.n; c += stride) {
+  constexpr bool LINE = XField<R, D, NTS>::kLine;
+  for (long long c = (long long)blockIdx.x * blockDim.x + threadIdx.x; (LINE ? (c & ~63ll) : c) < a.n; c += stride) {
     const unsigned int coff = (unsigned int)c * (unsigned int)sizeof(R);
     const unsigned int xoff = fx.offset(c);
     R x[D];
-#pragma unroll
-    for (int d = 0; d < D; ++d) x[d] = fx.load(d, xoff);
+    if constexpr (LINE) {
+      LineTile<R, D, NTS ? ME_NT_AUX : 0>::load(fx.f.rsrc, fx.offset(c & ~63ll), x);
+    } else {
+#pragma unroll
+      for (int d = 0; d < D; ++d) x[d] = fx.load(d, xoff);
+    }
+    bool moved = false;
+    if (!LINE || c < a.n) {
     Ledger ledger;
     R total_q5 = R(0);
     if (stale_total) total_q5 = fe.load(Ledger::T, coff);
@@ -893,16 +1007,21 @@
         else if constexpr (GROUP == GROUP_REAL) w_r = w;
         else w_c = w;
         wave_accepted += (unsigned int)__popcll(__ballot(accept));
+        moved |= accept;
       }
     } else {
-      run_sweeps<R, NR, NC, Energy, CK, INJECT, GROUP, LADDER>(a, en, c, gid, stale_total, x, ledger, total_q5, w, w_r, w_c, fac, wave_accepted, bad_energy);
+      run_sweeps<R, NR, NC, Energy, CK, INJECT, GROUP, LADDER>(a, en, c, gid, stale_total, x, ledger, total_q5, w, w_r, w_c, fac, wave_accepted, moved, bad_energy);
     }
     bad_width |= !(w > R(0));
-#pragma unroll
-    for (int d = 0; d < D; ++d) fx.store(d, xoff, x[d]);
+    if constexpr (!LINE) {
+#pragma unroll
+      for (int d = 0; d < D; ++d) fx.store(d, xoff, x[d]);
+    }
     if (stale_total) fe.store(Ledger::T, coff, total_q5);
     else ledger.store(fe, coff);
     fw.store(MIXED ? GROUP : 0, coff, w);
+    }
+    if constexpr (LINE) LineTile<R, D, NTS ? ME_NT_AUX : 0>::store(fx.f.rsrc, fx.offset(c & ~63ll), x, __ballot(moved));
   }
   publish_step(a, blockDim.x >> 6, wave_accepted, bad_energy, bad_width);
 }
@@ -1167,17 +1286,26 @@
   const Field<R> fmean(ma.mean, a.n, D), fobs(ma.obs_mean, a.n, NOBS);
   const TiledField<R> fcov(ma.cov, a.n, P), ffac(ma.factor, a.n, P);
   const bool stale_total = MIXED && a.stale_total != 0;
-  for (long long c = (long long)blockIdx.x * blockDim.x + threadIdx.x; c < a.n; c += stride) {
+  constexpr bool LINE = XField<R, D>::kLine;
+  for (long long c = (long long)blockIdx.x * blockDim.x + threadIdx.x; (LINE ? (c & ~63ll) : c) < a.n; c += stride) {
     const unsigned int coff = (unsigned int)c * (unsigned int)sizeof(R);
     const unsigned int xoff = fx.offset(c);
     R x[D];
-#pragma unroll
-    for (int d = 0; d < D; ++d) x[d] = fx.load(d, xoff);
+    if constexpr (LINE) {
+      LineTile<R, D, 0>::load(fx.f.rsrc, fx.offset(c & ~63ll), x);
+    } else {
+#pragma unroll
+      for (int d = 0; d < D; ++d) x[d] = fx.load(d, xoff);
+    }
+    bool moved = false;
+    const bool live = !LINE || c < a.n;
+    R w = R(0);
+    if (live) {
     Ledger ledger;
     R total_q5 = R(0);
     if (stale_total) total_q5 = fe.load(Ledger::T, coff);
     else ledger.load(fe, coff);
-    R w = fw.load(0, coff);
+    w = fw.load(0, coff);
     R w_r = w, w_c = w;
     if constexpr (MIXED) {
       if (a.split_widths) {
@@ -1192,15 +1320,20 @@
       else return a.factor[k];
     };
     run_sweeps<R, NR, NC, Energy, CKX, false, GROUP_ALL, LADDER>(a, en, c, gid, stale_total, x, ledger, total_q5, w, w_r, w_c, fac,
-                                                         wave_accepted, bad_energy);
+                                                         wave_accepted, moved, bad_energy);
     bad_width |= !(w > R(0));
-#pragma unroll
-    for (int d = 0; d < D; ++d) fx.store(d, xoff, x[d]);
+    if constexpr (!LINE) {
+#pragma unroll
+      for (int d = 0; d < D; ++d) fx.store(d, xoff, x[d]);
+    }
     if (stale_total) fe.store(Ledger::T, coff, total_q5);
     else ledger.store(fe, coff);
     fw.store(0, coff, w);
-    measure_chain<R, NR, NC, true, true, NT, NTM>(ma, c, x, fmean, fobs, fcov, ffac, nullptr,
-                                                  [&](R &w_real, R &w_cplx) { w_real = w_cplx = w; }, bad_pivot);
+    }
+    if constexpr (LINE) LineTile<R, D, 0>::store(fx.f.rsrc, fx.offset(c & ~63ll), x, __ballot(moved));
+    if (live)
+      measure_chain<R, NR, NC, true, true, NT, NTM>(ma, c, x, fmean, fobs, fcov, ffac, nullptr,
+                                                    [&](R &w_real, R &w_cplx) { w_real = w_cplx = w; }, bad_pivot);
   }
   publish_step(a, blockDim.x >> 6, wave_accepted, bad_energy, bad_width, bad_pivot);
 }
diff --git a/metropolisengine_amd/csrc/me_engine.h b/metropolisengine_amd/csrc/me_engine.h
--- a/metropolisengine_amd/csrc/me_engine.h
+++ b/metropolisengine_amd/csrc/me_engine.h
@@ -142,7 +142,7 @@
   me::DeviceBuffer accept_slots, accept_total;
   long long n_slots = 0;
   unsigned long long proposed = 0;
-  bool x_tiled = false;
+  int x_layout = me::ME_STATE_COMPONENT_MAJOR;
   int width_rows = 1;
   bool widths_synced = true;
   me::DeviceBuffer status;
diff --git a/metropolisengine_amd/csrc/me_generic.hip b/metropolisengine_amd/csrc/me_generic.hip
--- a/metropolisengine_amd/csrc/me_generic.hip
+++ b/metropolisengine_amd/csrc/me_generic.hip
@@ -12,10 +12,13 @@
 }
 
 template <typename R>
-__global__ void __launch_bounds__(kBlockThreads) k_broadcast_tiled(R *dst, const R *entry_values, int entries, long long n_padded) {
+__global__ void __launch_bounds__(kBlockThreads) k_broadcast_tiled(R *dst, const R *entry_values, int entries, long long n_padded, int layout) {
   const long long total = n_padded * entries, stride = (long long)gridDim.x * kBlockThreads;
-  for (long long i = (long long)blockIdx.x * kBlockThreads + threadIdx.x; i < total; i += stride)
-    dst[i] = entry_values[(i >> 6) % entries];
+  for (long long i = (long long)blockIdx.x * kBlockThreads + threadIdx.x; i < total; i += stride) {
+    const long long row_of_tile = i >> 6;
+    const int k = (int)(row_of_tile % entries);
+    dst[state_index(layout, row_of_tile / entries * 64 + (i & 63), k, entries, n_padded)] = entry_values[k];
+  }
 }
 
 __device__ __forceinline__ void pair_of(int p, int &i, int &j) {
@@ -28,7 +31,7 @@
 constexpr int kMaxEntries = 12;
 
 template <typename R, int TILE>
-__global__ void __launch_bounds__(kBlockThreads) k_pool_reduce(const R *x, long long n, int nr, int nc, int entry_base, int tiled, double *partials) {
+__global__ void __launch_bounds__(kBlockThreads) k_pool_reduce(const R *x, long long n, int nr, int nc, int entry_base, int layout, double *partials) {
   extern __shared__ __attribute__((aligned(16))) unsigned char smem_raw[];
   R *tile = reinterpret_cast<R *>(smem_raw);
   constexpr int kTilePitch = TILE + 1;
@@ -37,7 +40,7 @@
   const int n_pair = d * (d + 1) / 2;
   const int n_entries = 1 + n_aug + n_pair;
   const int tid = threadIdx.x;
-  auto at = [&](int r, long long c) -> long long { return tiled ? ((c >> 6) * (long long)d + r) * 64 + (c & 63) : (long long)r * n + c; };
+  auto at = [&](int r, long long c) -> long long { return state_index(layout, c, r, d, n); };
 
   int row_i[kMaxEntries], row_j[kMaxEntries];
   bool active[kMaxEntries];
@@ -182,17 +185,17 @@
 }
 
 hipError_t launch_broadcast_tiled(void *dst, const void *entry_values, int entries, long long n, int dtype,
-                                  hipStream_t stream) {
+                                  hipStream_t stream, int layout) {
   const long long n_padded = (n + 63) / 64 * 64;
   long long blocks = (n_padded * entries + kBlockThreads - 1) / kBlockThreads;
   if (blocks > 8192) blocks = 8192;
   if (blocks < 1) blocks = 1;
   if (dtype == ME_F32)
     hipLaunchKernelGGL(k_broadcast_tiled<float>, dim3((unsigned)blocks), dim3(kBlockThreads), 0, stream, (float *)dst,
-                       (const float *)entry_values, entries, n_padded);
+                       (const float *)entry_values, entries, n_padded, layout);
   else
     hipLaunchKernelGGL(k_broadcast_tiled<double>, dim3((unsigned)blocks), dim3(kBlockThreads), 0, stream, (double *)dst,
-                       (const double *)entry_values, entries, n_padded);
+                       (const double *)entry_values, entries, n_padded, layout);
   return hipGetLastError();
 }
 
@@ -225,12 +228,12 @@
 template <typename R>
 __global__ void __launch_bounds__(kBlockThreads) k_trace(const R *x, const R *energy, const R *width, long long n, int d,
                                                          int n_terms, int width_rows, long long n_traced, long long stride,
-                                                         int tiled, double *out) {
+                                                         int layout, double *out) {
   const long long t = (long long)blockIdx.x * kBlockThreads + threadIdx.x;
   if (t >= n_traced) return;
   const long long c = t * stride;
   for (int k = 0; k < d; ++k)
-    out[(long long)k * n_traced + t] = (double)x[tiled ? ((c >> 6) * (long long)d + k) * 64 + (c & 63) : (long long)k * n + c];
+    out[(long long)k * n_traced + t] = (double)x[state_index(layout, c, k, d, n)];
   for (int k = 0; k < n_terms; ++k) out[(long long)(d + k) * n_traced + t] = (double)energy[(long long)k * n + c];
   for (int r = 0; r < width_rows; ++r)
     out[(long long)(d + n_terms + r) * n_traced + t] = (double)width[(long long)r * n + c];
@@ -238,14 +241,14 @@
 
 hipError_t launch_trace(const void *x, const void *energy, const void *width, long long n, int d, int n_terms,
                         int width_rows, int dtype, long long n_traced, long long stride, double *out, hipStream_t stream,
-                        bool tiled_state) {
+                        int state_layout) {
   const dim3 grid((unsigned)((n_traced + kBlockThreads - 1) / kBlockThreads)), block(kBlockThreads);
   if (dtype == ME_F32)
     hipLaunchKernelGGL(k_trace<float>, grid, block, 0, stream, (const float *)x, (const float *)energy, (const float *)width,
-                       n, d, n_terms, width_rows, n_traced, stride, tiled_state ? 1 : 0, out);
+                       n, d, n_terms, width_rows, n_traced, stride, state_layout, out);
   else
     hipLaunchKernelGGL(k_trace<double>, grid, block, 0, stream, (const double *)x, (const double *)energy,
-                       (const double *)width, n, d, n_terms, width_rows, n_traced, stride, tiled_state ? 1 : 0, out);
+                       (const double *)width, n, d, n_terms, width_rows, n_traced, stride, state_layout, out);
   return hipGetLastError();
 }
 
@@ -279,21 +282,21 @@
 
 namespace {
 template <typename R, int TILE>
-hipError_t launch_pool_stage1(const void *x, long long n, int nr, int nc, int n_entries, int blocks, double *partials, hipStream_t stream, bool tiled) {
+hipError_t launch_pool_stage1(const void *x, long long n, int nr, int nc, int n_entries, int blocks, double *partials, hipStream_t stream, int layout) {
   const size_t lds = (size_t)(nr + 2 * nc + nr + nc) * (size_t)(TILE + 1) * sizeof(R);
   if (lds > 64 * 1024)
     if (hipError_t rc = raise_lds_limit<k_pool_reduce<R, TILE>>(kPoolLdsLimit); rc != hipSuccess) return rc;
   for (int base = 0; base < n_entries; base += kMaxEntries * kBlockThreads)
     hipLaunchKernelGGL((k_pool_reduce<R, TILE>), dim3((unsigned)blocks), dim3(kBlockThreads), lds, stream, (const R *)x, n, nr, nc, base,
-                       tiled ? 1 : 0, partials);
+                       layout, partials);
   return hipGetLastError();
 }
 template <typename R>
-hipError_t launch_pool_stage1_tile(int tile, const void *x, long long n, int nr, int nc, int n_entries, int blocks, double *partials, hipStream_t stream, bool tiled) {
+hipError_t launch_pool_stage1_tile(int tile, const void *x, long long n, int nr, int nc, int n_entries, int blocks, double *partials, hipStream_t stream, int layout) {
   switch (tile) {
-    case 64: return launch_pool_stage1<R, 64>(x, n, nr, nc, n_entries, blocks, partials, stream, tiled);
-    case 32: return launch_pool_stage1<R, 32>(x, n, nr, nc, n_entries, blocks, partials, stream, tiled);
-    case 16: return launch_pool_stage1<R, 16>(x, n, nr, nc, n_entries, blocks, partials, stream, tiled);
+    case 64: return launch_pool_stage1<R, 64>(x, n, nr, nc, n_entries, blocks, partials, stream, layout);
+    case 32: return launch_pool_stage1<R, 32>(x, n, nr, nc, n_entries, blocks, partials, stream, layout);
+    case 16: return launch_pool_stage1<R, 16>(x, n, nr, nc, n_entries, blocks, partials, stream, layout);
     default: return hipErrorInvalidValue;
   }
 }
@@ -302,7 +305,7 @@
 hipError_t launch_pool_reduce(const void *x, long long n, int nr, int nc, int dtype, const unsigned long long *slots,
                               long long n_slots, double proposed, double *partials, double *out_device,
                               hipStream_t stream,
-                              hipError_t (*stage1)(const void *, long long, double *, int, hipStream_t), bool tiled_state) {
+                              hipError_t (*stage1)(const void *, long long, double *, int, hipStream_t), int state_layout) {
   const int d = nr + 2 * nc;
   const int n_aug = d + nr + nc;
   const int n_entries = 1 + n_aug + d * (d + 1) / 2;
@@ -311,8 +314,8 @@
   const int blocks = pool_reduce_blocks(n, nr, nc);
   hipError_t err;
   if (stage1) err = stage1(x, n, partials, blocks, stream);
-  else if (dtype == ME_F32) err = launch_pool_stage1_tile<float>(tile, x, n, nr, nc, n_entries, blocks, partials, stream, tiled_state);
-  else err = launch_pool_stage1_tile<double>(tile, x, n, nr, nc, n_entries, blocks, partials, stream, tiled_state);
+  else if (dtype == ME_F32) err = launch_pool_stage1_tile<float>(tile, x, n, nr, nc, n_entries, blocks, partials, stream, state_layout);
+  else err = launch_pool_stage1_tile<double>(tile, x, n, nr, nc, n_entries, blocks, partials, stream, state_layout);
   if (err != hipSuccess) return err;
   hipLaunchKernelGGL(k_pool_finish, dim3((unsigned)((n_entries + 63) / 64 + 1)), dim3(kFinishThreads), 0, stream,
                      (const double *)partials, blocks, nr, nc, slots, n_slots, proposed, out_device);
diff --git a/metropolisengine_amd/csrc/me_internal.h b/metropolisengine_amd/csrc/me_internal.h
--- a/metropolisengine_amd/csrc/me_internal.h
+++ b/metropolisengine_amd/csrc/me_internal.h
@@ -80,6 +80,19 @@
 
 constexpr int kMaxRegisterDof = 96;
 
+enum StateLayout : int { ME_STATE_COMPONENT_MAJOR = 0, ME_STATE_TILE_MAJOR = 1, ME_STATE_LINE = 2 };
+__host__ __device__ constexpr long long state_index(int layout, long long c, int row, int d, long long n) {
+  return layout == ME_STATE_LINE         ? c * (long long)d + row
+         : layout == ME_STATE_TILE_MAJOR ? ((c >> 6) * (long long)d + row) * 64 + (c & 63)
+                                         : (long long)row * n + c;
+}
+__host__ __device__ constexpr int state_layout_of(int value_bytes, int d, int tiled_dof) {
+  return value_bytes * d == 128 ? ME_STATE_LINE : d >= tiled_dof ? ME_STATE_TILE_MAJOR : ME_STATE_COMPONENT_MAJOR;
+}
+__host__ __device__ constexpr long long state_field_values(int layout, int d, long long n) {
+  return (layout == ME_STATE_COMPONENT_MAJOR ? n : (n + 63) / 64 * 64) * (long long)d;
+}
+
 struct KernelSet {
   const char *user_name;
   int dtype, n_real, n_complex;
@@ -97,7 +110,7 @@
   bool has_user_reject;
   bool streams_packed;
   hipError_t (*cycle)(const StepLaunch &, const MeasureLaunch &, hipStream_t);
-  bool tiled_state;
+  int state_layout;
 };
 
 void register_kernel_set(const KernelSet *set);
@@ -107,18 +120,18 @@
 hipError_t launch_broadcast_rows(void *dst, const void *row_values, int rows, long long n, int dtype,
                                  hipStream_t stream);
 hipError_t launch_broadcast_tiled(void *dst, const void *entry_values, int entries, long long n, int dtype,
-                                  hipStream_t stream);
+                                  hipStream_t stream, int layout = ME_STATE_TILE_MAJOR);
 hipError_t launch_pool_reduce(const void *x, long long n, int n_real, int n_complex, int dtype,
                               const unsigned long long *slots, long long n_slots, double proposed, double *partials,
                               double *out_device, hipStream_t stream,
                               hipError_t (*stage1)(const void *, long long, double *, int, hipStream_t) = nullptr,
-                              bool tiled_state = false);
+                              int state_layout = ME_STATE_COMPONENT_MAJOR);
 int pool_reduce_blocks(long long n, int n_real, int n_complex);
 bool pool_reduce_supported(int n_real, int n_complex, int dtype);
 int pool_tile_chains(int n_real, int n_complex, int dtype);
 hipError_t launch_trace(const void *x, const void *energy, const void *width, long long n, int d, int n_terms,
                         int width_rows, int dtype, long long n_traced, long long stride, double *out, hipStream_t stream,
-                        bool tiled_state = false);
+                        int state_layout = ME_STATE_COMPONENT_MAJOR);
 hipError_t launch_sum_slots(const unsigned long long *slots, long long n_slots, unsigned long long *total,
                             hipStream_t stream);
 
diff --git a/metropolisengine_amd/csrc/me_kernels.hip b/metropolisengine_amd/csrc/me_kernels.hip
--- a/metropolisengine_amd/csrc/me_kernels.hip
+++ b/metropolisengine_amd/csrc/me_kernels.hip
@@ -117,18 +117,18 @@
       constexpr long long state_bytes = (long long)sizeof(R) * (D + 2);
       if constexpr (!INJECT && GROUP == GROUP_ALL && !LADDER) {
         if (state_bytes * l.n > 2 * cache_budget_bytes()) {
-          hipLaunchKernelGGL((k_step<R, NR, NC, Energy, CK_IDENTITY, INJECT, GROUP, true>), grid, block, 0, stream, a, en);
+          hipLaunchKernelGGL((k_step<R, NR, NC, Energy, CK_IDENTITY, INJECT, GROUP, true>), grid, block, (step_lds_bytes<R, D>((int)block.x)), stream, a, en);
           break;
         }
       }
-      hipLaunchKernelGGL((k_step<R, NR, NC, Energy, CK_IDENTITY, INJECT, GROUP, false, LADDER>), grid, block, 0, stream, a, en);
+      hipLaunchKernelGGL((k_step<R, NR, NC, Energy, CK_IDENTITY, INJECT, GROUP, false, LADDER>), grid, block, (step_lds_bytes<R, D>((int)block.x)), stream, a, en);
       break;
     }
-    case CK_SHARED: hipLaunchKernelGGL((k_step<R, NR, NC, Energy, CK_SHARED, INJECT, GROUP, false, LADDER>), grid, block, 0, stream, a, en); break;
+    case CK_SHARED: hipLaunchKernelGGL((k_step<R, NR, NC, Energy, CK_SHARED, INJECT, GROUP, false, LADDER>), grid, block, (step_lds_bytes<R, D>((int)block.x)), stream, a, en); break;
 #if ME_PER_CHAIN == 2
     case CK_PER_CHAIN: {
       if constexpr (INJECT) return hipErrorInvalidValue;
-      else hipLaunchKernelGGL((k_step<R, NR, NC, Energy, CK_PER_CHAIN_NT, INJECT, GROUP, false, LADDER>), grid, block, 0, stream, a, en);
+      else hipLaunchKernelGGL((k_step<R, NR, NC, Energy, CK_PER_CHAIN_NT, INJECT, GROUP, false, LADDER>), grid, block, (step_lds_bytes<R, D>((int)block.x)), stream, a, en);
       break;
     }
 #elif ME_PER_CHAIN
@@ -136,11 +136,11 @@
       constexpr long long per_chain_bytes = (long long)sizeof(R) * (D + 2 + NR * (NR + 1) / 2 + NC * NC);
       if constexpr (!INJECT) {
         if (per_chain_bytes * l.n > cache_budget_bytes()) {
-          hipLaunchKernelGGL((k_step<R, NR, NC, Energy, CK_PER_CHAIN_NT, INJECT, GROUP, false, LADDER>), grid, block, 0, stream, a, en);
+          hipLaunchKernelGGL((k_step<R, NR, NC, Energy, CK_PER_CHAIN_NT, INJECT, GROUP, false, LADDER>), grid, block, (step_lds_bytes<R, D>((int)block.x)), stream, a, en);
           break;
         }
       }
-      hipLaunchKernelGGL((k_step<R, NR, NC, Energy, CK_PER_CHAIN, INJECT, GROUP, false, LADDER>), grid, block, 0, stream, a, en);
+      hipLaunchKernelGGL((k_step<R, NR, NC, Energy, CK_PER_CHAIN, INJECT, GROUP, false, LADDER>), grid, block, (step_lds_bytes<R, D>((int)block.x)), stream, a, en);
       break;
     }
 #endif
@@ -170,7 +170,7 @@
     if (l.inj_normals) {
       if constexpr (std::is_same<R, double>::value) {
         if (l.group != GROUP_ALL || l.cov_kind != CK_IDENTITY) return hipErrorNotSupported;
-        hipLaunchKernelGGL((k_step<R, NR, NC, Energy, CK_IDENTITY, true, GROUP_ALL, false, true>), grid, block, 0, stream, a, en);
+        hipLaunchKernelGGL((k_step<R, NR, NC, Energy, CK_IDENTITY, true, GROUP_ALL, false, true>), grid, block, (step_lds_bytes<R, D>((int)block.x)), stream, a, en);
         return hipGetLastError();
       } else return hipErrorNotSupported;
     }
@@ -357,11 +357,11 @@
       const dim3 grid(grid_for(l.n, l.grid_blocks, threads)), block(threads);
       auto launch = [&](auto ck) {
         constexpr int CK = decltype(ck)::value;
-        if (l.ladder && nt) hipLaunchKernelGGL((k_cycle<R, NR, NC, Energy, CK, true, true, true>), grid, block, 0, stream, a, ma, en);
-        else if (l.ladder) hipLaunchKernelGGL((k_cycle<R, NR, NC, Energy, CK, false, false, true>), grid, block, 0, stream, a, ma, en);
-        else if (ntm) hipLaunchKernelGGL((k_cycle<R, NR, NC, Energy, CK, true, true>), grid, block, 0, stream, a, ma, en);
-        else if (nt) hipLaunchKernelGGL((k_cycle<R, NR, NC, Energy, CK, true, false>), grid, block, 0, stream, a, ma, en);
-        else hipLaunchKernelGGL((k_cycle<R, NR, NC, Energy, CK, false, false>), grid, block, 0, stream, a, ma, en);
+        if (l.ladder && nt) hipLaunchKernelGGL((k_cycle<R, NR, NC, Energy, CK, true, true, true>), grid, block, (step_lds_bytes<R, D>((int)block.x)), stream, a, ma, en);
+        else if (l.ladder) hipLaunchKernelGGL((k_cycle<R, NR, NC, Energy, CK, false, false, true>), grid, block, (step_lds_bytes<R, D>((int)block.x)), stream, a, ma, en);
+        else if (ntm) hipLaunchKernelGGL((k_cycle<R, NR, NC, Energy, CK, true, true>), grid, block, (step_lds_bytes<R, D>((int)block.x)), stream, a, ma, en);
+        else if (nt) hipLaunchKernelGGL((k_cycle<R, NR, NC, Energy, CK, true, false>), grid, block, (step_lds_bytes<R, D>((int)block.x)), stream, a, ma, en);
+        else hipLaunchKernelGGL((k_cycle<R, NR, NC, Energy, CK, false, false>), grid, block, (step_lds_bytes<R, D>((int)block.x)), stream, a, ma, en);
       };
       if (l.cov_kind == CK_PER_CHAIN) launch(std::integral_constant<int, CK_PER_CHAIN>{});
       else launch(std::integral_constant<int, CK_IDENTITY>{});
@@ -460,12 +460,12 @@
 #if ME_ONLY_DTYPE != 64
 const KernelSet kSetF32 = {ME_SET_NAME, ME_F32, NR, NC, ME_PER_CHAIN != 0, (ME_PER_CHAIN != 0 || ME_TRACK_COV != 0), has_energy, energy_terms, step<float>,
                            (NC > 0 && ME_PER_CHAIN == 1) ? magphase<float> : nullptr, measure<float>, init_energy<float>,
-                           ME_PREPARE_MATRIX_F32, kHasUserReject, ME_PER_CHAIN == 2, cycle<float>, D >= kTiledStateDof};
+                           ME_PREPARE_MATRIX_F32, kHasUserReject, ME_PER_CHAIN == 2, cycle<float>, kStateLayout<float, D>};
 #endif
 #if ME_ONLY_DTYPE != 32
 const KernelSet kSetF64 = {ME_SET_NAME, ME_F64, NR, NC, ME_PER_CHAIN != 0, (ME_PER_CHAIN != 0 || ME_TRACK_COV != 0), has_energy, energy_terms, step<double>,
                            (NC > 0 && ME_PER_CHAIN == 1) ? magphase<double> : nullptr, measure<double>, init_energy<double>,
-                           ME_PREPARE_MATRIX_F64, kHasUserReject, ME_PER_CHAIN == 2, cycle<double>, D >= kTiledStateDof};
+                           ME_PREPARE_MATRIX_F64, kHasUserReject, ME_PER_CHAIN == 2, cycle<double>, kStateLayout<double, D>};
 #endif
 
 struct Registrar {
diff --git a/metropolisengine_amd/csrc/me_mbar_obs.hip b/metropolisengine_amd/csrc/me_mbar_obs.hip
--- a/metropolisengine_amd/csrc/me_mbar_obs.hip
+++ b/metropolisengine_amd/csrc/me_mbar_obs.hip
@@ -15,13 +15,13 @@
 
 template <typename R>
 __global__ void __launch_bounds__(kThreads) k_observable_record(const R *__restrict__ x, const R *__restrict__ energy, long long n,
-                                                                 int nr, int nc, int n_terms, int tiled, ObsSelection sel,
+                                                                 int nr, int nc, int n_terms, int layout, ObsSelection sel,
                                                                  int n_sel, double *dst) {
   const long long c = (long long)blockIdx.x * kThreads + threadIdx.x;
   if (c >= n) return;
   const int d = nr + 2 * nc, nobs = 2 * nr + nc;
-  const long long x0 = tiled ? (c >> 6) * (long long)d * 64 + (c & 63) : c;
-  const long long xs = tiled ? 64 : n;
+  const long long x0 = state_index(layout, c, 0, d, n);
+  const long long xs = state_index(layout, c, 1, d, n) - x0;
   for (int j = 0; j < n_sel; ++j) {
     const int q = sel.q[j];
     double v;
@@ -311,10 +311,10 @@
   const dim3 grid((unsigned)((e->n + kThreads - 1) / kThreads));
   if (e->dtype == ME_F32)
     hipLaunchKernelGGL(k_observable_record<float>, grid, dim3(kThreads), 0, e->stream, e->x.get<const float>(), e->energy.get<const float>(),
-                       e->n, e->nr, e->nc, e->n_terms, e->x_tiled ? 1 : 0, sel, s.n_obs, dst);
+                       e->n, e->nr, e->nc, e->n_terms, e->x_layout, sel, s.n_obs, dst);
   else
     hipLaunchKernelGGL(k_observable_record<double>, grid, dim3(kThreads), 0, e->stream, e->x.get<const double>(),
-                       e->energy.get<const double>(), e->n, e->nr, e->nc, e->n_terms, e->x_tiled ? 1 : 0, sel, s.n_obs, dst);
+                       e->energy.get<const double>(), e->n, e->nr, e->nc, e->n_terms, e->x_layout, sel, s.n_obs, dst);
   return hipGetLastError();
 }
 
diff --git a/metropolisengine_amd/csrc/me_population.hip b/metropolisengine_amd/csrc/me_population.hip
--- a/metropolisengine_amd/csrc/me_population.hip
+++ b/metropolisengine_amd/csrc/me_population.hip
@@ -280,14 +280,14 @@
 template <typename R>
 __global__ void __launch_bounds__(kPopThreads) k_pop_gather(const R *x, const R *energy, const long long *fam, R *x_out,
                                                            R *energy_out, long long *fam_out, long long n, int d, int n_terms,
-                                                           int tiled, const unsigned int *ancestors, const PopParams *params) {
+                                                           int layout, const unsigned int *ancestors, const PopParams *params) {
   const long long j = (long long)blockIdx.x * kPopThreads + threadIdx.x;
   if (j >= n) return;
   const long long hi = params->hi;
   const long long a = (long long)ancestors[j < hi ? j : hi - 1];
   const unsigned int a_off = (unsigned int)a * (unsigned int)sizeof(R), j_off = (unsigned int)j * (unsigned int)sizeof(R);
-  if (tiled) copy_rows(TiledField<R>(x, n, d), TiledField<R>(x_out, n, d), tiled_offset<R>(a, d), tiled_offset<R>(j, d), d);
-  else copy_rows(Field<R>(x, n, d), Field<R>(x_out, n, d), a_off, j_off, d);
+  const LayoutField<R> fx(x, n, d, layout), fx_out(x_out, n, d, layout);
+  copy_rows(fx, fx_out, fx.offset(a), fx.offset(j), d);
   copy_rows(Field<R>(energy, n, n_terms), Field<R>(energy_out, n, n_terms), a_off, j_off, n_terms);
   fam_out[j] = fam[a];
 }
@@ -316,7 +316,7 @@
                      (const PopParams *)params, pop.anc.get<unsigned int>());
   hipLaunchKernelGGL(k_pop_gather<R>, dim3(slot_blocks), dim3(kPopThreads), 0, stream, e->x.get<const R>(), e->energy.get<const R>(),
                      pop.fam.get<const long long>(), pop.x.get<R>(), pop.energy.get<R>(), pop.fam_out.get<long long>(), n, e->d,
-                     e->n_terms, e->x_tiled ? 1 : 0, pop.anc.get<const unsigned int>(), (const PopParams *)params);
+                     e->n_terms, e->x_layout, pop.anc.get<const unsigned int>(), (const PopParams *)params);
   return hipGetLastError();
 }
 
diff --git a/metropolisengine_amd/csrc/me_replica.hip b/metropolisengine_amd/csrc/me_replica.hip
--- a/metropolisengine_amd/csrc/me_replica.hip
+++ b/metropolisengine_amd/csrc/me_replica.hip
@@ -20,7 +20,7 @@
   long long n, rung_chains;
   unsigned long long chain_offset, round;
   uint32_t seed_lo, seed_hi;
-  int d, n_terms, first_rung, tiled;
+  int d, n_terms, first_rung, layout;
 };
 
 template <class F>
@@ -59,8 +59,8 @@
   const R delta = dbeta * (ea - eb);
   const bool accept = N_::finite(ea) && N_::finite(eb) && (delta >= R(0) || N_::uphill(u, eb - ea, dbeta, dbeta_log2e));
   if (accept) {
-    if (s.tiled) swap_rows(TiledField<R>(s.x, s.n, s.d), tiled_offset<R>(a, s.d), tiled_offset<R>(b, s.d), s.d);
-    else swap_rows(Field<R>(s.x, s.n, s.d), ea_off, eb_off, s.d);
+    const LayoutField<R> fx(s.x, s.n, s.d, s.layout);
+    swap_rows(fx, fx.offset(a), fx.offset(b), s.d);
     swap_rows(fe, ea_off, eb_off, s.n_terms);
   }
   return accept;
@@ -92,7 +92,7 @@
 }
 
 template <typename R>
-hipError_t launch(void *x, void *energy, long long n, int d, int n_terms, bool tiled_state, const void *ladder, int n_rungs,
+hipError_t launch(void *x, void *energy, long long n, int d, int n_terms, int state_layout, const void *ladder, int n_rungs,
                   unsigned long long round, unsigned long long chain_offset, unsigned long long seed,
                   unsigned long long *pair_counts, hipStream_t stream) {
   SwapArgs<R> s;
@@ -110,7 +110,7 @@
   s.seed_hi = (uint32_t)(seed >> 32);
   s.d = d;
   s.n_terms = n_terms;
-  s.tiled = tiled_state ? 1 : 0;
+  s.layout = state_layout;
   if (n_pairs == 0) return hipSuccess;
   const long long per_pair = std::min<long long>((s.rung_chains + kSwapThreads - 1) / kSwapThreads, std::max(kSwapBlocks / n_pairs, 1));
   hipLaunchKernelGGL(k_replica_swap<R>, dim3((unsigned)per_pair, (unsigned)n_pairs), dim3(kSwapThreads), 0, stream, s);
@@ -183,7 +183,7 @@
   ME_HIP(e, hipSetDevice(e->device));
   const auto swap = e->dtype == ME_F32 ? launch<float> : launch<double>;
   for (int i = 0; i < n_rounds; ++i) {
-    ME_HIP(e, swap(e->x.get(), e->energy.get(), e->n, e->d, e->n_terms, e->x_tiled, e->ladder.table.get(), e->ladder.n_rungs, e->ladder.round,
+    ME_HIP(e, swap(e->x.get(), e->energy.get(), e->n, e->d, e->n_terms, e->x_layout, e->ladder.table.get(), e->ladder.n_rungs, e->ladder.round,
                    e->chain_offset, e->seed, e->ladder.pair_counts.get<unsigned long long>(), e->stream));
     e->ladder.round += 1;
   }
```

After: 18.04 billion. 0.964x the previous value.
